# SamStudio8/gretel

Hardware: NVIDIA B200
Metric: snp_pair_observations_per_sec (higher is better)
Workload: dtype u32

## Files before the change

gretel_b200/_lib.py:

```python
from __future__ import annotations

import ctypes as C
import os

_HERE = os.path.dirname(os.path.abspath(__file__))
LIB_PATH = os.path.join(_HERE, "libhanselx.so")

HX_OK, HX_HOLE = 0, 1
HX_E_CUDA, HX_E_ARG, HX_E_BAND, HX_E_READ, HX_E_NOMEM, HX_E_STATE = -1, -2, -3, -4, -5, -6
HX_F_VSITE_TO, HX_F_KEEP_UNSYMBOLS = 1, 2

_p, _i32, _i64, _int, _dbl, _flt = C.c_void_p, C.c_int32, C.c_int64, C.c_int, C.c_double, C.c_float
_pp = C.POINTER(C.c_void_p)

SIGNATURES = {
    "hx_last_error": (C.c_char_p, []),
    "hx_version": (_int, []),
    "hx_device_count": (_int, [C.POINTER(_int)]),
    "hx_create": (_int, [_i32, _i32, _i32, _pp]),
    "hx_destroy": (_int, [_p]),
    "hx_copy": (_int, [_p, _pp]),
    "hx_info": (_int, [_p, C.POINTER(_i32), C.POINTER(_i32), C.POINTER(_i32)]),
    "hx_stream": (_int, [_p, _pp]),
    "hx_set_stream": (_int, [_p, _p]),
    "hx_sync": (_int, [_p]),
    "hx_ingest_host": (_int, [_p, _p, _p, _p, _i64, _p]),
    "hx_counts_pack": (_int, [_p, _i32, _pp, C.POINTER(_i64)]),
    "hx_counts_unpack": (_int, [_p, C.POINTER(_i32)]),
    "hx_counts_unpack_async": (_int, [_p, _p]),
    "hx_counts_pack_overflowed": (_int, [_p, C.POINTER(_i32)]),
    "hx_counts_max": (_int, [_p, C.POINTER(C.c_uint32)]),
    "hx_ingest_host_compact": (_int, [_p, _p, _p, _p, _i64, _i64, _p]),
    "hx_dense_encode": (_int, [_p, _p, _p, _i64, _int, _p]),
    "hx_dense_free": (None, [_p]),
    "hx_ingest_host_dense": (_int, [_p, _p, _p, _p, _i64, _p, _i32, _p, _p, _i64, _i64, _i64, _p]),
    "hx_ingest_device": (_int, [_p, _p, _p, _p, _i64]),
    "hx_set_ingest_kernel": (_int, [_p, _int]),
    "hx_set_ingest_sms": (_int, [_p, _int]),
    "hx_ingest_totals": (_int, [_p, _p]),
    "hx_counts_buffer": (_int, [_p, _pp, C.POINTER(_i64), _pp, C.POINTER(_i64)]),
    "hx_counts_ipc_export": (_int, [_p, _i32, _p]),
    "hx_counts_ipc_import": (_int, [_p, _p, _i32, _i32]),
    "hx_counts_ipc_close": (_int, [_p]),
    "hx_finalize_counts": (_int, [_p]),
    "hx_reset_counts": (_int, [_p]),
    "hx_add_observation": (_int, [_p, _int, _int, _i32, _i32, _flt]),
    "hx_get_observation": (_int, [_p, _int, _int, _i32, _i32, C.POINTER(_flt)]),
    "hx_reweight_observation": (_int, [_p, _int, _int, _i32, _i32, _dbl, C.POINTER(_dbl)]),
    "hx_reweight_matrix": (_int, [_p, _dbl]),
    "hx_counts_all": (_int, [_p, _p]),
    "hx_marginal_of_at": (_int, [_p, _int, _i32, C.POINTER(_dbl)]),
    "hx_edge_weights_at": (_int, [_p, _i32, _p, _i32, _int, _p, C.POINTER(_dbl), C.POINTER(_int)]),
    "hx_generate_path": (_int, [_p, _p, _i32, _int, _p, _p, C.POINTER(_i32)]),
    "hx_reweight_path": (_int, [_p, _p, _dbl, C.POINTER(_dbl)]),
    "hx_recover": (_int, [_p, _p, _i32, _int, _i32, _dbl, _p, _p, C.POINTER(_i32)]),
    "hx_pack_bam": (_int, [C.c_char_p, C.c_char_p, _i32, _i32, _p, _i32, _int, _int, _p]),
    "hx_pack_bam_ex": (_int, [C.c_char_p, C.c_char_p, _i32, _i32, _p, _i32, _int, _int, _i32, _p, _p]),
    "hx_pack_free": (None, [_p]),
    "hx_count_coverage": (_int, [C.c_char_p, C.c_char_p, _i32, _i32, _int, _p]),
    "hx_count_coverage_gpu": (_int, [C.c_char_p, C.c_char_p, _i32, _i32, _int, _i32, _p]),
    "hx_bam_contig_length": (_int, [C.c_char_p, C.c_char_p, C.POINTER(_i32)]),
    "hx_inflate_raw": (_int, [_p, _i64, _i64, _p, _i64, _i32]),
    "hx_probe_expected_rows": (_int, [_p, _p, _p, _p, _i64, _p]),
    "hx_counts_row_sums": (_int, [_p, _p]),
    "hx_device_math": (_int, [_i32, _int, _p, _p, _i64]),
    "hx_band_to_host": (_int, [_p, _p]),
    "hx_band_from_host": (_int, [_p, _p]),
    "hx_to_dense": (_int, [_p, _p]),
    "hx_last_kernel_ms": (_int, [_p, _int, C.POINTER(_flt)]),
    "hx_launch_count": (_int, [_p, C.POINTER(_i64)]),
}

class HxPacked(C.Structure):
    _fields_ = [("rank", C.POINTER(C.c_int32)), ("off", C.POINTER(C.c_int64)), ("codes", C.POINTER(C.c_uint8)),
                ("n_reads", C.c_int64), ("n_codes", C.c_int64), ("n_records", C.c_int64)]


class HxDense(C.Structure):
    _fields_ = [("blob", C.POINTER(C.c_uint8)), ("blob_bytes", C.c_int64), ("n_reads", C.c_int64),
                ("n_codes", C.c_int64), ("n_exc", C.c_int64), ("n_esc", C.c_int64), ("o_klen", C.c_int64),
                ("o_codes2", C.c_int64), ("o_exc", C.c_int64), ("o_esc_idx", C.c_int64), ("o_esc_delta", C.c_int64),
                ("klen_bytes", C.c_int32)]


_LIB = None


class HanselxError(RuntimeError):
    def __init__(self, code, msg):
        super().__init__("hanselx error %d: %s" % (code, msg))
        self.code = code


def load():
    global _LIB
    if _LIB is not None:
        return _LIB
    if not os.path.exists(LIB_PATH):
        raise RuntimeError(
            "gretel_b200: %s is missing - build it with `python -m gretel_b200.build` "
            "(nvcc, sm_100a).  There is no CPU fallback." % LIB_PATH)
    lib = C.CDLL(LIB_PATH)
    for name, (res, args) in SIGNATURES.items():
        fn = getattr(lib, name)
        fn.restype = res
        fn.argtypes = args
    _LIB = lib
    return lib


def check(rc, allow=()):
    if rc == HX_OK or rc in allow:
        return rc
    raise HanselxError(rc, load().hx_last_error().decode(errors="replace"))
```

gretel_b200/csrc/api.cu:

```cuda
#include <stdarg.h>
#include <stdlib.h>
#include <string.h>

#include <algorithm>
#include <mutex>
#include <vector>

#include <atomic>

#include "hx_internal.cuh"
#include "scan.cuh"

static thread_local char g_err[512] = "";

void hx_set_error(const char *fmt, ...) {
    va_list ap;
    va_start(ap, fmt);
    vsnprintf(g_err, sizeof(g_err), fmt, ap);
    va_end(ap);
}

static void release_counts(hx_matrix *h) {
    for (int g = 0; g < HX_MAX_PEERS; ++g) {
        if (h->ipc_opened[g]) cudaIpcCloseMemHandle(h->ipc_opened[g]);
        h->ipc_opened[g] = nullptr;
        h->peer_host[g] = nullptr;
    }
    h->peer_world = 0;
    if (h->cnt) {
        if (h->cnt_ipc) { cudaStreamSynchronize(h->stream); cudaFree(h->cnt); }
        else cudaFreeAsync(h->cnt, h->stream);
    }
    h->cnt = nullptr;
    h->cnt_ipc = false;
    h->cnt_elems = 0;
}

HxCnt hx_cnt_ref(const hx_matrix *h) {
    HxCnt c;
    c.local = h->cnt;
    c.peer = h->d_peer_tbl;
    c.world = h->peer_world > 1 ? h->peer_world : 1;
    c.rows_per = h->peer_world > 1 ? h->peer_rows_per : 1;
    return c;
}

namespace {

__global__ void k_fold_counts(const uint32_t *__restrict__ cnt, float *__restrict__ band, int64_t n) {
    const int64_t i = (int64_t)blockIdx.x * blockDim.x + threadIdx.x;
    if (i < n) {
        const uint32_t c = cnt[i];
        if (c) band[i] += (float)c;
    }
}

__global__ void k_add_one(float *p, float amount) { *p += amount; }

__global__ void k_reset_counts(uint4 *__restrict__ cnt, size_t bytes, unsigned long long *__restrict__ totals,
                               int *__restrict__ err) {
    const size_t n16 = bytes / 16;
    const uint4 z = make_uint4(0, 0, 0, 0);
    for (size_t i = (size_t)blockIdx.x * blockDim.x + threadIdx.x; i < n16; i += (size_t)gridDim.x * blockDim.x) cnt[i] = z;
    if (blockIdx.x == 0) {
        uint8_t *tail = reinterpret_cast<uint8_t *>(cnt) + n16 * 16;
        for (size_t i = threadIdx.x; i < bytes - n16 * 16; i += blockDim.x) tail[i] = 0;
        if (threadIdx.x < 8) totals[threadIdx.x] = 0;
        if (threadIdx.x == 8) *err = 0;
    }
}

#define HX_PACK_WORDS 25
__global__ void k_pack_counts(const uint32_t *__restrict__ cnt, int64_t n_pairs, uint32_t lim16,
                              uint32_t *__restrict__ packed, int64_t flag_at) {
    const int64_t i = (int64_t)blockIdx.x * blockDim.x + threadIdx.x;
    if (i >= n_pairs * HX_PACK_WORDS) return;
    const int64_t p = i / HX_PACK_WORDS;
    const int w = (int)(i - p * HX_PACK_WORDS);
    const uint32_t *c = cnt + p * HX_CELL + 2 * w;
    const uint32_t lo = c[0], hi = 2 * w + 1 < HX_CELL ? c[1] : 0u;
    if (lo > lim16 || hi > lim16) packed[flag_at] = 1u;
    packed[i] = (lo & 0xffffu) | (hi << 16);
}

__global__ void k_unpack_counts(const uint32_t *__restrict__ packed, int64_t n_pairs, uint32_t *__restrict__ cnt,
                                int64_t flag_at) {
    if (packed[flag_at] != 0u) return;
    const int64_t i = (int64_t)blockIdx.x * blockDim.x + threadIdx.x;
    if (i >= n_pairs * HX_PACK_WORDS) return;
    const int64_t p = i / HX_PACK_WORDS;
    const int w = (int)(i - p * HX_PACK_WORDS);
    const uint32_t v = packed[i];
    uint32_t *c = cnt + p * HX_CELL + 2 * w;
    c[0] = v & 0xffffu;
    if (2 * w + 1 < HX_CELL) c[1] = v >> 16;
}

__global__ void k_widen_klen(const uint16_t *__restrict__ klen, int64_t n, int64_t *__restrict__ out ) {
    const int64_t i = (int64_t)blockIdx.x * blockDim.x + threadIdx.x;
    if (i <= n) out[i] = i < n ? (int64_t)klen[i] : 0;
}

__global__ void k_unpack_nibbles(const uint32_t *__restrict__ in, int64_t n_words, uint2 *__restrict__ out) {
    const int64_t i = (int64_t)blockIdx.x * blockDim.x + threadIdx.x;
    if (i >= n_words) return;
    const uint32_t w = in[i];
    uint2 o;
    o.x = (w & 0xfu) | ((w >> 4 & 0xfu) << 8) | ((w >> 8 & 0xfu) << 16) | ((w >> 12 & 0xfu) << 24);
    o.y = (w >> 16 & 0xfu) | ((w >> 20 & 0xfu) << 8) | ((w >> 24 & 0xfu) << 16) | ((w >> 28 & 0xfu) << 24);
    out[i] = o;
}

__global__ void k_reweight_one(float *p, double ratio, double *removed) {
    const double old = (double)*p;
    const double nw = old - (ratio * old);
    *p = (float)nw;
    *removed = old - nw;
}

int in_band(const hx_matrix *h, int a, int b, int64_t i, int64_t j) {
    if (a < 0 || a >= HX_NSYM || b < 0 || b >= HX_NSYM) return HX_E_ARG;
    if (i < 0 || j < 0 || i > (int64_t)h->N + 1 || j > (int64_t)h->N + 1) return HX_E_ARG;
    if (j - i < 1 || j - i > h->W) return HX_E_BAND;
    return HX_OK;
}

void free_all(hx_matrix *h) {
    if (!h) return;
    cudaSetDevice(h->device);
    hx_lr_free(h);
    hx_l2_free(h);
    hx_wire_free(h);
    if (h->d_peer_tbl) cudaFree(h->d_peer_tbl);
    cudaStream_t st = h->stream;
    h->band.release(st);
    release_counts(h);
    h->d_totals.release(st); h->d_err.release(st);
    h->s_rank.release(st); h->s_off.release(st); h->s_codes.release(st);
    h->s_klen.release(st); h->s_codes4.release(st); h->s_scan.release(st);
    h->scnt.release(st); h->vseen.release(st); h->d_path.release(st); h->d_stats.release(st); h->d_site.release(st);
    h->d_partials.release(st); h->d_spec.release(st); h->d_terms.release(st); h->d_flags.release(st);
    h->d_run_end.release(st); h->d_run_list.release(st); h->d_jobs.release(st); h->d_misc.release(st);
    h->d_pack.release(st);
    if (st) cudaStreamSynchronize(st);
    free(h->h_pinned);
    if (h->ev0) cudaEventDestroy(h->ev0);
    if (h->ev1) cudaEventDestroy(h->ev1);
    if (h->host_ev) cudaEventDestroy(h->host_ev);
    if (h->sum_stream) { cudaStreamSynchronize(h->sum_stream); cudaStreamDestroy(h->sum_stream); }
    for (int b = 0; b < 2; ++b) if (h->sum_done[b]) cudaEventDestroy(h->sum_done[b]);
    if (h->site_ready) cudaEventDestroy(h->site_ready);
    if (h->own_stream && h->stream) cudaStreamDestroy(h->stream);
    free(h);
}

}

extern "C" {

const char *hx_last_error(void) { return g_err; }
int hx_version(void) { return 100; }

int hx_device_count(int *n) {
    HX_CHECK_ARG(n);
    HX_CUDA(cudaGetDeviceCount(n));
    return HX_OK;
}

}

namespace {
std::mutex &g_park_mu = *new std::mutex;
std::vector<hx_matrix *> &g_parked = *new std::vector<hx_matrix *>;
constexpr size_t HX_PARK_MAX = 4;
constexpr int64_t HX_PARK_MAX_ELEMS = (int64_t)1 << 28;
const bool g_park_on = getenv("HX_NO_MATRIX_CACHE") == nullptr;

hx_matrix *unpark(int32_t n_snps, int32_t band_w, int32_t device) {
    std::lock_guard<std::mutex> lk(g_park_mu);
    for (size_t i = 0; i < g_parked.size(); ++i) {
        hx_matrix *h = g_parked[i];
        if (h->N == n_snps && h->W == band_w && h->device == device) {
            g_parked.erase(g_parked.begin() + (long)i);
            return h;
        }
    }
    return nullptr;
}

bool park(hx_matrix *h) {
    if (!g_park_on || !h->own_stream || h->cnt_ipc || h->peer_world > 1 || h->band_elems > HX_PARK_MAX_ELEMS) return false;
    if (cudaSetDevice(h->device) != cudaSuccess) return false;
    release_counts(h);
    if (cudaStreamSynchronize(h->stream) != cudaSuccess) return false;
    hx_matrix *evict = nullptr;
    {
        std::lock_guard<std::mutex> lk(g_park_mu);
        if (g_parked.size() >= HX_PARK_MAX) { evict = g_parked.front(); g_parked.erase(g_parked.begin()); }
        g_parked.push_back(h);
    }
    if (evict) free_all(evict);
    return true;
}

int reset_parked(hx_matrix *h) {
    HX_CUDA(cudaSetDevice(h->device));
    HX_CUDA(hx_fill_async(h->band.p, 0, sizeof(float) * (size_t)h->band_elems, h->stream));
    HX_CUDA(hx_fill_async(h->d_totals.p, 0, 8 * sizeof(unsigned long long), h->stream));
    HX_CUDA(hx_fill_async(h->d_err.p, 0, sizeof(int), h->stream));
    HX_CUDA(hx_fill_async(h->d_flags.p, 0, 8 * sizeof(int), h->stream));
    h->use = {};
    return HX_OK;
}
}

extern "C" {

int hx_create(int32_t n_snps, int32_t band_w, int32_t device, hx_matrix **out) {
    HX_CHECK_ARG(out && n_snps >= 0 && band_w >= 1);
    *out = nullptr;
    HX_CUDA(cudaSetDevice(device));
    if (hx_matrix *p = unpark(n_snps, band_w, device)) {
        const int rc = reset_parked(p);
        if (rc) { free_all(p); return rc; }
        *out = p;
        return HX_OK;
    }
    hx_matrix *h = (hx_matrix *)calloc(1, sizeof(hx_matrix));
    if (!h) return HX_E_NOMEM;
    h->N = n_snps;
    h->W = band_w;
    h->device = device;
    h->band_elems = ((int64_t)n_snps + 2) * band_w * HX_CELL;
    h->use = {};
#define HX_TRY(call)                                                                     \
    do {                                                                                 \
        cudaError_t e__ = (call);                                                        \
        if (e__ != cudaSuccess) {                                                        \
            hx_set_error("hx_create: %s -> %s", #call, cudaGetErrorString(e__));         \
            free_all(h);                                                                 \
            return e__ == cudaErrorMemoryAllocation ? HX_E_NOMEM : HX_E_CUDA;            \
        }                                                                                \
    } while (0)
    {
        cudaMemPool_t pool;
        if (cudaDeviceGetDefaultMemPool(&pool, device) == cudaSuccess) {
            unsigned long long thr = ~0ull;
            cudaMemPoolSetAttribute(pool, cudaMemPoolAttrReleaseThreshold, &thr);
        }
    }
    HX_TRY(cudaStreamCreateWithFlags(&h->stream, cudaStreamNonBlocking));
    h->own_stream = true;
    HX_TRY(cudaEventCreate(&h->ev0));
    HX_TRY(cudaEventCreate(&h->ev1));
    HX_TRY(h->band.grow(sizeof(float) * (size_t)h->band_elems, h->stream));
    HX_TRY(hx_fill_async(h->band.p, 0, sizeof(float) * (size_t)h->band_elems, h->stream));
    HX_TRY(h->d_totals.grow(8 * sizeof(unsigned long long), h->stream));
    HX_TRY(hx_fill_async(h->d_totals.p, 0, 8 * sizeof(unsigned long long), h->stream));
    HX_TRY(h->d_err.grow(sizeof(int), h->stream));
    HX_TRY(hx_fill_async(h->d_err.p, 0, sizeof(int), h->stream));
    HX_TRY(h->scnt.grow(sizeof(double) * 8 * ((size_t)n_snps + 2), h->stream));
    HX_TRY(h->vseen.grow(sizeof(int32_t) * ((size_t)n_snps + 2), h->stream));
    HX_TRY(h->d_site.grow(sizeof(double) * 6 * ((size_t)n_snps + 2), h->stream));
    HX_TRY(h->d_flags.grow(8 * sizeof(int), h->stream));
    HX_TRY(hx_fill_async(h->d_flags.p, 0, 8 * sizeof(int), h->stream));
    HX_TRY(h->d_misc.grow(32 * sizeof(double), h->stream));
    HX_TRY(h->d_run_end.grow(sizeof(int64_t) * ((size_t)n_snps + 2), h->stream));
    HX_TRY(h->d_run_list.grow(sizeof(int64_t) * (((size_t)n_snps + 3) / 2 + (size_t)n_snps + 2 + 2), h->stream));
    h->h_pinned = calloc(1, 256);
    if (!h->h_pinned) { free_all(h); return HX_E_NOMEM; }
    HX_TRY(cudaStreamSynchronize(h->stream));
#undef HX_TRY
    *out = h;
    return HX_OK;
}

int hx_destroy(hx_matrix *h) {
    if (h && !park(h)) free_all(h);
    return HX_OK;
}

int hx_copy(const hx_matrix *src, hx_matrix **out) {
    HX_CHECK_ARG(src && out);
    if (src->cnt) {
        hx_set_error("hx_copy: integer counts pending; call hx_finalize_counts first");
        return HX_E_STATE;
    }
    int rc = hx_create(src->N, src->W, src->device, out);
    if (rc) return rc;
    hx_matrix *h = *out;
    HX_CUDA(cudaStreamSynchronize(src->stream));
    HX_CUDA(cudaMemcpyAsync(h->band.p, src->band.p, sizeof(float) * (size_t)src->band_elems,
                            cudaMemcpyDeviceToDevice, h->stream));
    HX_CUDA(cudaMemcpyAsync(h->d_totals.p, src->d_totals.p, 8 * sizeof(unsigned long long),
                            cudaMemcpyDeviceToDevice, h->stream));
    HX_CUDA(cudaStreamSynchronize(h->stream));
    h->use.ingest_kernel = src->use.ingest_kernel;
    return HX_OK;
}

int hx_info(const hx_matrix *h, int32_t *n_snps, int32_t *band_w, int32_t *device) {
    HX_CHECK_ARG(h);
    if (n_snps) *n_snps = h->N;
    if (band_w) *band_w = h->W;
    if (device) *device = h->device;
    return HX_OK;
}

int hx_stream(const hx_matrix *h, void **stream) {
    HX_CHECK_ARG(h && stream);
    *stream = (void *)h->stream;
    return HX_OK;
}

int hx_set_stream(hx_matrix *h, void *stream) {
    HX_CHECK_ARG(h);
    HX_CUDA(cudaSetDevice(h->device));
    HX_CUDA(cudaStreamSynchronize(h->stream));
    if (h->own_stream) cudaStreamDestroy(h->stream);
    h->stream = (cudaStream_t)stream;
    h->own_stream = false;
    return HX_OK;
}

int hx_sync(hx_matrix *h) {
    HX_CHECK_ARG(h);
    HX_CUDA(cudaSetDevice(h->device));
    HX_CUDA(cudaStreamSynchronize(h->stream));
    return HX_OK;
}

}
int hx_ensure_counts_buffer(hx_matrix *h) {
    if (h->cnt) return HX_OK;
    h->cnt_elems = h->band_elems;
    HX_CUDA(cudaMallocAsync((void **)&h->cnt, sizeof(uint32_t) * (size_t)h->cnt_elems, h->stream));
    HX_CUDA(hx_fill_async(h->cnt, 0, sizeof(uint32_t) * (size_t)h->cnt_elems, h->stream));
    h->use.cnt_fresh = true;
    return HX_OK;
}
extern "C" {

int hx_set_ingest_kernel(hx_matrix *h, int which) {
    HX_CHECK_ARG(h && which >= 0 && which <= 7);
    h->use.ingest_kernel = which;
    return HX_OK;
}

int hx_set_ingest_sms(hx_matrix *h, int n_sms) {
    HX_CHECK_ARG(h && n_sms >= 0);
    h->use.ingest_sms = n_sms;
    return HX_OK;
}

int hx_ingest_device(hx_matrix *h, const int32_t *d_rank, const int64_t *d_off,
                     const uint8_t *d_codes, int64_t n_reads) {
    HX_CHECK_ARG(h && n_reads >= 0);
    if (n_reads == 0) return HX_OK;
    HX_CHECK_ARG(d_rank && d_off && d_codes);
    HX_CUDA(cudaSetDevice(h->device));
    int rc = hx_ensure_counts_buffer(h);
    if (rc) return rc;
    return hx_launch_ingest(h, d_rank, d_off, d_codes, n_reads);
}

int hx_ingest_totals(hx_matrix *h, int64_t totals[4]) {
    HX_CHECK_ARG(h && totals);
    HX_CUDA(cudaSetDevice(h->device));
    unsigned long long *hp = (unsigned long long *)h->h_pinned;
    int *he = (int *)(hp + 8);
    HX_CUDA(cudaMemcpyAsync(hp, h->d_totals.p, 4 * sizeof(unsigned long long), cudaMemcpyDeviceToHost, h->stream));
    HX_CUDA(cudaMemcpyAsync(he, h->d_err.p, sizeof(int), cudaMemcpyDeviceToHost, h->stream));
    if (h->use.prepass_ran) HX_CUDA(cudaMemcpyAsync(he + 1, h->d_flags.p + 4, sizeof(int), cudaMemcpyDeviceToHost, h->stream));
    HX_CUDA(cudaStreamSynchronize(h->stream));
    if (h->use.prepass_ran && he[1] == 0) hx_note_unsorted();
    hx_wire_trace_dump();
    if (h->use.ev_rec) cudaEventElapsedTime(&h->use.last_ms[0], h->ev0, h->ev1);
    for (int i = 0; i < 4; ++i) totals[i] = (int64_t)hp[i];
    if (*he) {
        hx_set_error("ingest: invalid packed read(s): %s%s",
                     (*he & 1) ? "[read leaves [0,N] or has more SNPs than band_w+1] " : "",
                     (*he & 2) ? "[allele code > 6]" : "");
        return HX_E_READ;
    }
    return HX_OK;
}

int hx_ingest_host(hx_matrix *h, const int32_t *rank, const int64_t *off, const uint8_t *codes,
                   int64_t n_reads, int64_t totals[4]) {
    HX_CHECK_ARG(h && totals && n_reads >= 0);
    HX_CUDA(cudaSetDevice(h->device));
    const char *pipe_env = getenv("HX_HOST_PIPELINE");
    const bool want_dense = pipe_env && !strcmp(pipe_env, "dense");
    const bool want_slim = !pipe_env || !strcmp(pipe_env, "slim");
    if (n_reads >= 200000 && rank && off && codes && (want_dense || want_slim)) {
        int64_t done = 0;
        const int rc = hx_ingest_host_pipelined(h, rank, off, codes, n_reads, !want_dense, &done);
        if (rc == HX_OK) return hx_ingest_totals(h, totals);
        if (rc != HX_E_STATE) return rc;
        hx_note_unsorted();
        rank += done; off += done; n_reads -= done;
    }
    if (n_reads > 0) {
        HX_CHECK_ARG(rank && off && codes);
        const int64_t n_codes = off[n_reads] - off[0];
        HX_CHECK_ARG(n_codes >= 0);
        HX_CUDA(h->s_rank.grow(sizeof(int32_t) * n_reads, h->stream));
        HX_CUDA(h->s_off.grow(sizeof(int64_t) * (n_reads + 1) + 16, h->stream));
        HX_CUDA(h->s_codes.grow(n_codes + 16, h->stream));
        int rc = hx_ensure_counts_buffer(h);
        if (rc) return rc;
        const int n_chunks = n_reads >= 200000 && !(pipe_env && !strcmp(pipe_env, "off")) ? 4 : 1;
        if (n_chunks > 1 && !h->copy_stream) HX_CUDA(cudaStreamCreateWithFlags(&h->copy_stream, cudaStreamNonBlocking));
        cudaStream_t cs = n_chunks > 1 ? h->copy_stream : h->stream;
        if (n_chunks > 1) {
            if (!h->host_ev) HX_CUDA(cudaEventCreateWithFlags(&h->host_ev, cudaEventDisableTiming));
            HX_CUDA(cudaEventRecord(h->host_ev, h->stream));
            HX_CUDA(cudaStreamWaitEvent(cs, h->host_ev, 0));
        }
        int64_t a = 0;
        for (int c = 0; c < n_chunks; ++c) {
            int64_t b = n_reads;
            if (c + 1 < n_chunks) {
                const int64_t target = off[0] + n_codes * (c + 1) / n_chunks;
                b = std::lower_bound(off + a, off + n_reads, target) - off;
                if (b <= a) continue;
            }
            HX_CUDA(cudaMemcpyAsync(h->s_rank.p + a, rank + a, sizeof(int32_t) * (size_t)(b - a), cudaMemcpyHostToDevice, cs));
            HX_CUDA(cudaMemcpyAsync(h->s_off.p + a, off + a, sizeof(int64_t) * (size_t)(b - a + 1), cudaMemcpyHostToDevice, cs));
            HX_CUDA(cudaMemcpyAsync(h->s_codes.p + (off[a] - off[0]), codes + off[a], (size_t)(off[b] - off[a]), cudaMemcpyHostToDevice, cs));
            if (n_chunks > 1) {
                HX_CUDA(cudaEventRecord(h->host_ev, cs));
                HX_CUDA(cudaStreamWaitEvent(h->stream, h->host_ev, 0));
            }
            rc = hx_launch_ingest(h, h->s_rank.p + a, h->s_off.p + a, h->s_codes.p - off[0], b - a);
            if (rc) return rc;
            a = b;
        }
    }
    return hx_ingest_totals(h, totals);
}

int hx_ingest_host_compact(hx_matrix *h, const int32_t *rank, const uint16_t *klen, const uint8_t *codes4,
                           int64_t n_reads, int64_t n_codes, int64_t totals[4]) {
    HX_CHECK_ARG(h && totals && n_reads >= 0 && n_codes >= 0);
    HX_CUDA(cudaSetDevice(h->device));
    if (n_reads > 0) {
        HX_CHECK_ARG(rank && klen && (codes4 || n_codes == 0));
        cudaStream_t st = h->stream;
        const int64_t n_words = (n_codes + 7) / 8;
        constexpr int ITEMS = 16;
        const int64_t n1 = n_reads + 1;
        const int64_t nblk = (n1 + 256 * ITEMS - 1) / (256 * ITEMS);
        HX_CUDA(h->s_rank.grow(sizeof(int32_t) * n_reads, st));
        HX_CUDA(h->s_off.grow(sizeof(int64_t) * n1 + 16, st));
        HX_CUDA(h->s_codes.grow(n_words * 8 + 16, st));
        HX_CUDA(h->s_klen.grow(sizeof(uint16_t) * n_reads, st));
        HX_CUDA(h->s_codes4.grow(sizeof(uint32_t) * n_words, st));
        HX_CUDA(h->s_scan.grow(sizeof(int64_t) * nblk, st));
        HX_CUDA(cudaMemcpyAsync(h->s_rank.p, rank, sizeof(int32_t) * (size_t)n_reads, cudaMemcpyHostToDevice, st));
        HX_CUDA(cudaMemcpyAsync(h->s_klen.p, klen, sizeof(uint16_t) * (size_t)n_reads, cudaMemcpyHostToDevice, st));
        if (n_codes)
            HX_CUDA(cudaMemcpyAsync(h->s_codes4.p, codes4, (size_t)((n_codes + 1) / 2), cudaMemcpyHostToDevice, st));
        k_widen_klen<<<(unsigned)((n1 + 255) / 256), 256, 0, st>>>(h->s_klen.p, n_reads, h->s_off.p);
        k_scan_partials<int64_t, 0, ITEMS><<<(unsigned)nblk, 256, 0, st>>>(h->s_off.p, n1, h->s_scan.p);
        k_scan_spine<int64_t, 0><<<1, 32, 0, st>>>(h->s_scan.p, nblk, nullptr);
        k_scan_apply<int64_t, 0, ITEMS, true><<<(unsigned)nblk, 256, 0, st>>>(h->s_off.p, n1, h->s_scan.p, h->s_off.p);
        if (n_words)
            k_unpack_nibbles<<<(unsigned)((n_words + 255) / 256), 256, 0, st>>>(h->s_codes4.p, n_words, (uint2 *)h->s_codes.p);
        h->use.launches += 5;
        HX_CUDA(cudaGetLastError());
        int rc = hx_ensure_counts_buffer(h);
        if (rc) return rc;
        rc = hx_launch_ingest(h, h->s_rank.p, h->s_off.p, h->s_codes.p, n_reads);
        if (rc) return rc;
    }
    return hx_ingest_totals(h, totals);
}

int hx_counts_buffer(hx_matrix *h, void **d_counts, int64_t *n_u32, void **d_totals, int64_t *n_i64) {
    HX_CHECK_ARG(h && d_counts && n_u32 && d_totals && n_i64);
    HX_CUDA(cudaSetDevice(h->device));
    int rc = hx_ensure_counts_buffer(h);
    if (rc) return rc;
    *d_counts = h->cnt;
    h->use.cnt_fresh = false;
    *n_u32 = h->cnt_elems;
    *d_totals = h->d_totals.p;
    *n_i64 = 4;
    return HX_OK;
}

int hx_counts_pack(hx_matrix *h, int32_t world, void **d_packed, int64_t *n_u32) {
    HX_CHECK_ARG(h && d_packed && n_u32 && world >= 1 && world <= 65535);
    HX_CUDA(cudaSetDevice(h->device));
    int rc = hx_ensure_counts_buffer(h);
    if (rc) return rc;
    const int64_t n_pairs = h->band_elems / HX_CELL;
    const int64_t flag_at = (n_pairs * HX_PACK_WORDS + 3) & ~(int64_t)3;
    const int64_t words = flag_at + 4;
    HX_CUDA(h->d_pack.grow(sizeof(uint32_t) * words, h->stream));
    HX_CUDA(hx_fill_async(h->d_pack.p + n_pairs * HX_PACK_WORDS, 0, (size_t)(words - n_pairs * HX_PACK_WORDS) * 4, h->stream));
    const int64_t n_w = n_pairs * HX_PACK_WORDS;
    k_pack_counts<<<(unsigned)((n_w + 255) / 256), 256, 0, h->stream>>>(h->cnt, n_pairs, 65535u / (uint32_t)world,
                                                                        h->d_pack.p, flag_at);
    h->use.launches++;
    HX_CUDA(cudaGetLastError());
    *d_packed = h->d_pack.p;
    *n_u32 = words;
    return HX_OK;
}

int hx_counts_unpack(hx_matrix *h, int32_t *overflowed) {
    HX_CHECK_ARG(h && overflowed && h->d_pack.p && h->cnt);
    HX_CUDA(cudaSetDevice(h->device));
    const int64_t n_pairs = h->band_elems / HX_CELL;
    const int64_t flag_at = (n_pairs * HX_PACK_WORDS + 3) & ~(int64_t)3;
    const int64_t n_w = n_pairs * HX_PACK_WORDS;
    h->use.cnt_fresh = false;
    k_unpack_counts<<<(unsigned)((n_w + 255) / 256), 256, 0, h->stream>>>(h->d_pack.p, n_pairs, h->cnt, flag_at);
    h->use.launches++;
    HX_CUDA(cudaGetLastError());
    uint32_t *hp = (uint32_t *)h->h_pinned + 40;
    HX_CUDA(cudaMemcpyAsync(hp, h->d_pack.p + flag_at, sizeof(uint32_t), cudaMemcpyDeviceToHost, h->stream));
    HX_CUDA(cudaStreamSynchronize(h->stream));
    *overflowed = *hp != 0;
    return HX_OK;
}

int hx_counts_unpack_async(hx_matrix *h, void *stream) {
    HX_CHECK_ARG(h && h->d_pack.p && h->cnt);
    HX_CUDA(cudaSetDevice(h->device));
    const int64_t n_pairs = h->band_elems / HX_CELL;
    const int64_t flag_at = (n_pairs * HX_PACK_WORDS + 3) & ~(int64_t)3;
    const int64_t n_w = n_pairs * HX_PACK_WORDS;
    h->use.cnt_fresh = false;
    cudaStream_t st = stream ? (cudaStream_t)stream : h->stream;
    k_unpack_counts<<<(unsigned)((n_w + 255) / 256), 256, 0, st>>>(h->d_pack.p, n_pairs, h->cnt, flag_at);
    h->use.launches++;
    HX_CUDA(cudaGetLastError());
    return HX_OK;
}

int hx_counts_pack_overflowed(hx_matrix *h, int32_t *overflowed) {
    HX_CHECK_ARG(h && overflowed && h->d_pack.p);
    HX_CUDA(cudaSetDevice(h->device));
    const int64_t n_pairs = h->band_elems / HX_CELL;
    const int64_t flag_at = (n_pairs * HX_PACK_WORDS + 3) & ~(int64_t)3;
    uint32_t *hp = (uint32_t *)h->h_pinned + 40;
    HX_CUDA(cudaMemcpyAsync(hp, h->d_pack.p + flag_at, sizeof(uint32_t), cudaMemcpyDeviceToHost, h->stream));
    HX_CUDA(cudaStreamSynchronize(h->stream));
    *overflowed = *hp != 0;
    return HX_OK;
}

__global__ void k_counts_max(const uint32_t *__restrict__ cnt, int64_t n, uint32_t *__restrict__ out) {
    uint32_t m = 0;
    for (int64_t i = (int64_t)blockIdx.x * blockDim.x + threadIdx.x; i < n; i += (int64_t)gridDim.x * blockDim.x) m = max(m, cnt[i]);
    m = __reduce_max_sync(0xffffffffu, m);
    if ((threadIdx.x & 31) == 0 && m) atomicMax(out, m);
}

int hx_counts_max(hx_matrix *h, uint32_t *max_count) {
    HX_CHECK_ARG(h && max_count);
    HX_CUDA(cudaSetDevice(h->device));
    int rc = hx_ensure_counts_buffer(h);
    if (rc) return rc;
    uint32_t *d_out = reinterpret_cast<uint32_t *>(h->d_flags.p + 6);
    HX_CUDA(hx_fill_async(d_out, 0, sizeof(uint32_t), h->stream));
    k_counts_max<<<592, 256, 0, h->stream>>>(h->cnt, h->cnt_elems, d_out);
    h->use.launches++;
    HX_CUDA(cudaGetLastError());
    uint32_t *hp = (uint32_t *)h->h_pinned + 41;
    HX_CUDA(cudaMemcpyAsync(hp, d_out, sizeof(uint32_t), cudaMemcpyDeviceToHost, h->stream));
    HX_CUDA(cudaStreamSynchronize(h->stream));
    *max_count = *hp;
    return HX_OK;
}

int hx_counts_ipc_export(hx_matrix *h, int32_t world, void *handle_out) {
    HX_CHECK_ARG(h && handle_out && world >= 1 && world <= HX_MAX_PEERS);
    HX_CUDA(cudaSetDevice(h->device));
    release_counts(h);
    const int64_t rows = (int64_t)h->N + 2;
    const int64_t rows_per = (rows + world - 1) / world;
    h->cnt_elems = rows_per * world * h->W * HX_CELL;
    HX_CUDA(cudaMalloc((void **)&h->cnt, sizeof(uint32_t) * (size_t)h->cnt_elems));
    h->cnt_ipc = true;
    h->use.cnt_fresh = false;
    HX_CUDA(hx_fill_async(h->cnt, 0, sizeof(uint32_t) * (size_t)h->cnt_elems, h->stream));
    HX_CUDA(cudaStreamSynchronize(h->stream));
    cudaIpcMemHandle_t hd;
    HX_CUDA(cudaIpcGetMemHandle(&hd, h->cnt));
    memcpy(handle_out, &hd, sizeof(hd));
    h->peer_rows_per = (int)rows_per;
    return HX_OK;
}

int hx_counts_ipc_import(hx_matrix *h, const void *handles, int32_t world, int32_t my_rank) {
    HX_CHECK_ARG(h && handles && world >= 1 && world <= HX_MAX_PEERS && my_rank >= 0 && my_rank < world);
    if (!h->cnt_ipc) { hx_set_error("hx_counts_ipc_import: call hx_counts_ipc_export first"); return HX_E_STATE; }
    HX_CUDA(cudaSetDevice(h->device));
    for (int g = 0; g < world; ++g) {
        if (g == my_rank) { h->peer_host[g] = h->cnt; continue; }
        cudaIpcMemHandle_t hd;
        memcpy(&hd, (const char *)handles + (size_t)g * sizeof(hd), sizeof(hd));
        void *p = nullptr;
        HX_CUDA(cudaIpcOpenMemHandle(&p, hd, cudaIpcMemLazyEnablePeerAccess));
        h->ipc_opened[g] = p;
        h->peer_host[g] = (uint32_t *)p;
    }
    if (!h->d_peer_tbl) HX_CUDA(cudaMalloc((void **)&h->d_peer_tbl, sizeof(uint32_t *) * HX_MAX_PEERS));
    HX_CUDA(cudaMemcpy(h->d_peer_tbl, h->peer_host, sizeof(uint32_t *) * HX_MAX_PEERS, cudaMemcpyHostToDevice));
    h->peer_world = world;
    return HX_OK;
}

int hx_counts_ipc_close(hx_matrix *h) {
    HX_CHECK_ARG(h);
    HX_CUDA(cudaSetDevice(h->device));
    HX_CUDA(cudaStreamSynchronize(h->stream));
    for (int g = 0; g < HX_MAX_PEERS; ++g) {
        if (h->ipc_opened[g]) HX_CUDA(cudaIpcCloseMemHandle(h->ipc_opened[g]));
        h->ipc_opened[g] = nullptr;
        h->peer_host[g] = nullptr;
    }
    h->peer_world = 0;
    return HX_OK;
}

int hx_reset_counts(hx_matrix *h) {
    HX_CHECK_ARG(h);
    HX_CUDA(cudaSetDevice(h->device));
    if (h->cnt) {
        const size_t n16 = (sizeof(uint32_t) * (size_t)h->cnt_elems + 15) / 16;
        const size_t want = (n16 + 255) / 256;
        const unsigned grid = (unsigned)(want < 1 ? 1 : (want > 148 * 16 ? 148 * 16 : want));
        k_reset_counts<<<grid, 256, 0, h->stream>>>(reinterpret_cast<uint4 *>(h->cnt), sizeof(uint32_t) * (size_t)h->cnt_elems,
                                                    h->d_totals.p, h->d_err.p);
        HX_CUDA(cudaGetLastError());
        h->use.cnt_fresh = true;
    } else {
        HX_CUDA(hx_fill_async(h->d_totals.p, 0, 8 * sizeof(unsigned long long), h->stream));
        HX_CUDA(hx_fill_async(h->d_err.p, 0, sizeof(int), h->stream));
    }
    return HX_OK;
}

int hx_finalize_counts(hx_matrix *h) {
    HX_CHECK_ARG(h);
    if (!h->cnt) return HX_OK;
    HX_CUDA(cudaSetDevice(h->device));
    const int64_t n = h->band_elems;
    k_fold_counts<<<(unsigned)((n + 255) / 256), 256, 0, h->stream>>>(h->cnt, h->band.p, n);
    h->use.launches++;
    HX_CUDA(cudaGetLastError());
    if (h->cnt_ipc) HX_CUDA(cudaStreamSynchronize(h->stream));
    release_counts(h);
    h->use.counts_dirty = true;
    return HX_OK;
}

int hx_add_observation(hx_matrix *h, int a, int b, int32_t i, int32_t j, float amount) {
    HX_CHECK_ARG(h);
    int rc = in_band(h, a, b, i, j);
    if (rc) { hx_set_error("add_observation(%d,%d,%d,%d): outside band/arguments", a, b, i, j); return rc; }
    HX_CUDA(cudaSetDevice(h->device));
    k_add_one<<<1, 1, 0, h->stream>>>(h->band.p + hx_cell_off(h->W, i, j) + a * HX_NSYM + b, amount);
    h->use.launches++;
    h->use.counts_dirty = true;
    HX_CUDA(cudaGetLastError());
    return HX_OK;
}

int hx_get_observation(hx_matrix *h, int a, int b, int32_t i, int32_t j, float *out) {
    HX_CHECK_ARG(h && out);
    int rc = in_band(h, a, b, i, j);
    if (rc == HX_E_BAND) { *out = 0.0f; return HX_E_BAND; }
    if (rc) { hx_set_error("get_observation(%d,%d,%d,%d): bad arguments", a, b, i, j); return rc; }
    HX_CUDA(cudaSetDevice(h->device));
    const int64_t o = hx_cell_off(h->W, i, j) + a * HX_NSYM + b;
    float v = 0.0f;
    HX_CUDA(cudaMemcpyAsync(&v, h->band.p + o, sizeof(float), cudaMemcpyDeviceToHost, h->stream));
    HX_CUDA(cudaStreamSynchronize(h->stream));
    if (h->cnt) {
        uint32_t c = 0;
        HX_CUDA(cudaMemcpyAsync(&c, h->cnt + o, sizeof(uint32_t), cudaMemcpyDeviceToHost, h->stream));
        HX_CUDA(cudaStreamSynchronize(h->stream));
        v += (float)c;
    }
    *out = v;
    return HX_OK;
}

int hx_reweight_observation(hx_matrix *h, int a, int b, int32_t i, int32_t j, double ratio,
                            double *removed) {
    HX_CHECK_ARG(h && removed);
    int rc = in_band(h, a, b, i, j);
    if (rc == HX_E_BAND) { *removed = 0.0; return HX_E_BAND; }
    if (rc) { hx_set_error("reweight_observation(%d,%d,%d,%d): bad arguments", a, b, i, j); return rc; }
    if (h->cnt) { hx_set_error("reweight_observation: call hx_finalize_counts first"); return HX_E_STATE; }
    HX_CUDA(cudaSetDevice(h->device));
    k_reweight_one<<<1, 1, 0, h->stream>>>(h->band.p + hx_cell_off(h->W, i, j) + a * HX_NSYM + b, ratio, h->d_misc.p + 16);
    h->use.launches++;
    h->use.counts_dirty = true;
    HX_CUDA(cudaGetLastError());
    HX_CUDA(cudaMemcpyAsync(removed, h->d_misc.p + 16, sizeof(double), cudaMemcpyDeviceToHost, h->stream));
    HX_CUDA(cudaStreamSynchronize(h->stream));
    return HX_OK;
}

int hx_band_to_host(hx_matrix *h, float *out) {
    HX_CHECK_ARG(h && out);
    if (h->cnt) { hx_set_error("band_to_host: call hx_finalize_counts first"); return HX_E_STATE; }
    HX_CUDA(cudaSetDevice(h->device));
    HX_CUDA(cudaMemcpyAsync(out, h->band.p, sizeof(float) * (size_t)h->band_elems, cudaMemcpyDeviceToHost, h->stream));
    HX_CUDA(cudaStreamSynchronize(h->stream));
    return HX_OK;
}

int hx_band_from_host(hx_matrix *h, const float *in) {
    HX_CHECK_ARG(h && in);
    if (h->cnt) { hx_set_error("band_from_host: call hx_finalize_counts first"); return HX_E_STATE; }
    HX_CUDA(cudaSetDevice(h->device));
    HX_CUDA(cudaMemcpyAsync(h->band.p, in, sizeof(float) * (size_t)h->band_elems, cudaMemcpyHostToDevice, h->stream));
    HX_CUDA(cudaStreamSynchronize(h->stream));
    h->use.counts_dirty = true;
    return HX_OK;
}

int hx_to_dense(hx_matrix *h, float *out) {
    HX_CHECK_ARG(h && out);
    const int64_t P = (int64_t)h->N + 2;
    float *tmp = (float *)malloc(sizeof(float) * (size_t)h->band_elems);
    if (!tmp) return HX_E_NOMEM;
    int rc = hx_band_to_host(h, tmp);
    if (rc) { free(tmp); return rc; }
    memset(out, 0, sizeof(float) * (size_t)(HX_CELL * P * P));
    for (int64_t pj = 1; pj < P; ++pj)
        for (int64_t d = 1; d <= h->W && pj - d >= 0; ++d) {
            const float *cell = tmp + hx_cell_off(h->W, pj - d, pj);
            for (int ab = 0; ab < HX_CELL; ++ab) out[(ab * P + (pj - d)) * P + pj] = cell[ab];
        }
    free(tmp);
    return HX_OK;
}

int hx_last_kernel_ms(hx_matrix *h, int which, float *ms) {
    HX_CHECK_ARG(h && ms && which >= 0 && which < 3);
    *ms = h->use.last_ms[which];
    return HX_OK;
}

int hx_launch_count(const hx_matrix *h, int64_t *n) {
    HX_CHECK_ARG(h && n);
    *n = h->use.launches;
    return HX_OK;
}

}
```

gretel_b200/csrc/hx_internal.cuh:

```cuda
#pragma once
#include <cuda_runtime.h>
#include <stdint.h>
#include <stdio.h>

#include "hanselx.h"

#define HX_NSYM 7
#define HX_CELL 49
#define HX_SYM_N 4
#define HX_SYM_DEL 5
#define HX_SYM_GAP 6
#define HX_RING 4096
#define HX_MAX_L (HX_RING - 1)

#define HX_MAX_PEERS 8
struct HxCnt {
    uint32_t *local;
    uint32_t *const *peer;
    int world, rows_per;
#ifdef __CUDACC__
    __device__ __forceinline__ uint32_t *cell(int64_t W, int64_t pi, int64_t pj) const {
        uint32_t *base = local;
        if (world > 1) base = peer[pj / rows_per];
        return base + (pj * W + (pj - pi - 1)) * 49;
    }
#endif
};

template <class T>
struct HxDevBuf {
    T *p;
    int64_t cap;
    cudaError_t grow(int64_t bytes, cudaStream_t st, bool *grew = nullptr) {
        if (bytes <= cap) return cudaSuccess;
        if (grew) *grew = true;
        release(st);
        const cudaError_t e = cudaMallocAsync((void **)&p, (size_t)bytes, st);
        if (e != cudaSuccess) { p = nullptr; return e; }
        cap = bytes;
        return cudaSuccess;
    }
    void release(cudaStream_t st) {
        if (p) cudaFreeAsync(p, st);
        p = nullptr;
        cap = 0;
    }
};

#define HX_WIRE_SETS 3
struct hx_wire_set {
    HxDevBuf<uint8_t> raw; HxDevBuf<int32_t> rank; HxDevBuf<int64_t> off; HxDevBuf<uint8_t> codes;
    HxDevBuf<int64_t> partials, run_end;
    cudaEvent_t copied, decoded, consumed;
};

struct hx_matrix {
    int32_t N, W, device;
    int64_t band_elems;
    cudaStream_t stream;
    bool own_stream;
    HxDevBuf<float> band;
    uint32_t *cnt;
    bool cnt_ipc;
    int64_t cnt_elems;
    uint32_t *peer_host[HX_MAX_PEERS];
    uint32_t **d_peer_tbl;
    int peer_world, peer_rows_per;
    void *ipc_opened[HX_MAX_PEERS];
    HxDevBuf<unsigned long long> d_totals;
    HxDevBuf<int> d_err;
    HxDevBuf<int32_t> s_rank; HxDevBuf<int64_t> s_off; HxDevBuf<uint8_t> s_codes;
    HxDevBuf<uint16_t> s_klen; HxDevBuf<uint32_t> s_codes4; HxDevBuf<int64_t> s_scan;
    hx_wire_set wire[HX_WIRE_SETS];
    cudaStream_t copy_stream, decode_stream;
    uint8_t *pin[2]; int64_t pin_cap[2]; cudaEvent_t pin_ev[2]; bool pin_busy[2];
    HxDevBuf<double> scnt;
    HxDevBuf<int32_t> vseen;
    HxDevBuf<uint8_t> d_path;
    HxDevBuf<double> d_stats;
    HxDevBuf<double> d_site;
    cudaStream_t sum_stream;
    cudaEvent_t sum_done[2], site_ready;
    HxDevBuf<double> d_terms;
    HxDevBuf<uint8_t> d_spec;
    HxDevBuf<double> d_partials;
    HxDevBuf<int> d_flags;
    HxDevBuf<int64_t> d_run_end;
    HxDevBuf<int64_t> d_run_list;
    HxDevBuf<int4> d_jobs;
    HxDevBuf<double> d_misc;
    HxDevBuf<uint32_t> d_pack;
    void *h_pinned;
    void *lr_scratch;
    void *l2_scratch;
    cudaEvent_t ev0, ev1;
    cudaEvent_t host_ev;
    struct Use {
        int64_t launches = 0;
        int ingest_kernel = 0;
        int ingest_sms = 0;
        bool counts_dirty = true;
        bool cnt_fresh = false;
        bool ev_rec = false;
        bool prepass_ran = false;
        int wire_next = 0;
        bool sum_busy[2] = {};
        float last_ms[3] = {};
    } use;
};

void hx_set_error(const char *fmt, ...);

#define HX_CUDA(call)                                                                   \
    do {                                                                                \
        cudaError_t e__ = (call);                                                       \
        if (e__ != cudaSuccess) {                                                       \
            hx_set_error("%s:%d %s -> %s", __FILE__, __LINE__, #call, cudaGetErrorString(e__)); \
            return HX_E_CUDA;                                                           \
        }                                                                               \
    } while (0)

#define HX_CHECK_ARG(cond)                                                              \
    do {                                                                                \
        if (!(cond)) {                                                                  \
            hx_set_error("%s:%d argument check failed: %s", __FILE__, __LINE__, #cond); \
            return HX_E_ARG;                                                            \
        }                                                                               \
    } while (0)

#ifdef __CUDACC__
static __global__ void k_fill_bytes(uint8_t *p, unsigned v, size_t bytes) {
    if (reinterpret_cast<uintptr_t>(p) & 15) {
        for (size_t i = (size_t)blockIdx.x * blockDim.x + threadIdx.x; i < bytes; i += (size_t)gridDim.x * blockDim.x)
            p[i] = (uint8_t)v;
        return;
    }
    const size_t n16 = bytes / 16;
    const uint4 w = make_uint4(v, v, v, v);
    uint4 *p16 = reinterpret_cast<uint4 *>(p);
    for (size_t i = (size_t)blockIdx.x * blockDim.x + threadIdx.x; i < n16; i += (size_t)gridDim.x * blockDim.x) p16[i] = w;
    if (blockIdx.x == 0)
        for (size_t i = n16 * 16 + threadIdx.x; i < bytes; i += blockDim.x) p[i] = (uint8_t)v;
}
static inline cudaError_t hx_fill_async(void *p, int byte, size_t bytes, cudaStream_t st) {
    if (!bytes) return cudaSuccess;
    const unsigned b = (unsigned)byte & 0xffu, v = b * 0x01010101u;
    const size_t want = (bytes / 16 + 255) / 256;
    const unsigned grid = (unsigned)(want < 1 ? 1 : (want > 148 * 16 ? 148 * 16 : want));
    k_fill_bytes<<<grid, 256, 0, st>>>(static_cast<uint8_t *>(p), v, bytes);
    return cudaGetLastError();
}
#endif

__host__ __device__ __forceinline__ int64_t hx_cell_off(int64_t W, int64_t pi, int64_t pj) {
    return (pj * W + (pj - pi - 1)) * HX_CELL;
}

int hx_launch_ingest(hx_matrix *h, const int32_t *d_rank, const int64_t *d_off,
                     const uint8_t *d_codes, int64_t n_reads);
int hx_launch_ingest_presorted(hx_matrix *h, const int32_t *d_rank, const int64_t *d_off,
                               const uint8_t *d_codes, int64_t n_reads, int64_t *run_end, const int *ok);
bool hx_umma_possible(const hx_matrix *h);
int hx_launch_ingest_umma(hx_matrix *h, const int32_t *d_rank, const int64_t *d_off, const uint8_t *d_codes,
                          int64_t n_reads, const int64_t *run_end, const int *sorted_flag);
HxCnt hx_cnt_ref(const hx_matrix *h);
int hx_ensure_counts_buffer(hx_matrix *h);
void hx_wire_free(hx_matrix *h);
void hx_wire_trace_dump();
bool hx_unsorted_seen();
void hx_note_unsorted();
int hx_ingest_host_pipelined(hx_matrix *h, const int32_t *rank, const int64_t *off, const uint8_t *codes, int64_t n_reads,
                             bool slim, int64_t *done_reads);
int hx_launch_ingest_long(hx_matrix *h, const int32_t *d_rank, const int64_t *d_off,
                          const uint8_t *d_codes, int64_t n_reads, const int *sorted_flag);
void hx_lr_free(hx_matrix *h);
int hx_launch_ingest_lumma(hx_matrix *h, const int32_t *d_rank, const int64_t *d_off, const uint8_t *d_codes,
                           int64_t n_reads, const int *go);
int64_t hx_lumma_scratch_bytes(const hx_matrix *h, int64_t n_reads);
void hx_l2_free(hx_matrix *h);
int hx_ensure_counts(hx_matrix *h);
```

gretel_b200/csrc/ingest.cu:

```cuda
#include <atomic>

#include "hx_internal.cuh"
#include "ingest_common.cuh"

namespace {

constexpr int BS_KMAX = 52;
constexpr int BS_GB = 32;

__device__ __forceinline__ void add_pair(const HxCnt cnt, int N, int64_t W, int rk, int i,
                                         int j, unsigned a, unsigned b, unsigned long long &sent) {
    const int pi = rk + i + 1, pj = rk + j + 1;
    atomicAdd(cnt.cell(W, pi, pj) + a * HX_NSYM + b, 1u);
    if (i == 0 && j == 1 && rk == 0) {
        atomicAdd(cnt.cell(W, 0, 1) + HX_SYM_GAP * HX_NSYM + a, 1u);
        sent++;
    } else if (pj == N && j - i == 1) {
        atomicAdd(cnt.cell(W, N, N + 1) + b * HX_NSYM + HX_SYM_GAP, 1u);
        sent++;
    }
}

__device__ __forceinline__ void warp_read_generic(const uint8_t *__restrict__ c, int k, int rk, int N,
                                                  int64_t W, const HxCnt cnt,
                                                  unsigned long long &t_crumbs, unsigned long long &t_cov,
                                                  unsigned long long &t_sent, int *err) {
    const int lane = threadIdx.x & 31;
    for (int t = lane; t < k; t += 32) {
        const unsigned a = c[t];
        if (a > 6) atomicOr(err, 2);
        const bool v = sym_valid_from(a);
        t_cov += v;
        t_crumbs += v ? (unsigned)(k - 1 - t) : 0u;
    }
    const int64_t npairs = (int64_t)k * (k - 1) / 2;
    const int m = 2 * k - 1;
    for (int64_t q = lane; q < npairs; q += 32) {
        const float disc = (float)((int64_t)m * m - 8 * q);
        int i = (int)(((float)m - sqrtf(disc)) * 0.5f);
        i = max(0, min(i, k - 2));
        while ((int64_t)(i + 1) * (m - (i + 1)) / 2 <= q) ++i;
        while ((int64_t)i * (m - i) / 2 > q) --i;
        const int j = i + 1 + (int)(q - (int64_t)i * (m - i) / 2);
        const unsigned a = c[i], b = c[j];
        if (!sym_valid_from(a) || b > 6) continue;
        add_pair(cnt, N, W, rk, i, j, a, b, t_sent);
    }
}

template <int BLOCK>
__global__ void __launch_bounds__(BLOCK)
k1_pairs_red(const int32_t *__restrict__ rank, const int64_t *__restrict__ off,
             const uint8_t *__restrict__ codes, int64_t n_reads, int N, int W,
             const HxCnt cnt, unsigned long long *__restrict__ totals,
             int *__restrict__ err, const int *__restrict__ sorted_flag, int run_if_sorted) {
    if (run_if_sorted == 0 && *sorted_flag) return;
    if (run_if_sorted == 2 && !*sorted_flag) return;
    const int lane = threadIdx.x & 31;
    const int64_t nwarps = (int64_t)gridDim.x * (BLOCK / 32);
    unsigned long long t_slices = 0, t_crumbs = 0, t_cov = 0, t_sent = 0;
    for (int64_t r = (int64_t)blockIdx.x * (BLOCK / 32) + (threadIdx.x >> 5); r < n_reads; r += nwarps) {
        const int64_t o = off[r];
        const int64_t k64 = off[r + 1] - o;
        if (k64 < 2) continue;
        const int rk = rank[r];
        if (rk < 0 || (int64_t)rk + k64 > N || k64 - 1 > W) {
            if (lane == 0) atomicOr(err, 1);
            continue;
        }
        if (lane == 0) t_slices++;
        warp_read_generic(codes + o, (int)k64, rk, N, W, cnt, t_crumbs, t_cov, t_sent, err);
    }
    flush_totals(t_slices, t_crumbs, t_cov, t_sent, totals);
}

__global__ void k_prepass_init(int *__restrict__ flag, int64_t *__restrict__ run_end, int n) {
    const int i = blockIdx.x * blockDim.x + threadIdx.x;
    if (i == 0) *flag = 1;
    if (i < n) run_end[i] = -1;
}

__global__ void k_prepass(const int32_t *__restrict__ rank, int64_t n_reads, int N, int *__restrict__ flag,
                          int64_t *__restrict__ run_end, int *__restrict__ err) {
    const int64_t i = (int64_t)blockIdx.x * blockDim.x + threadIdx.x;
    if (i >= n_reads) return;
    const int r = rank[i];
    if (r < 0 || r > N) atomicOr(err, 1);
    if (i + 1 < n_reads) {
        const int r2 = rank[i + 1];
        if (r > r2) *flag = 0;
        if (r != r2 && r >= 0 && r <= N) run_end[r] = i + 1;
    } else if (r >= 0 && r <= N) {
        run_end[r] = n_reads;
    }
}

struct BsLayout {
    int kmax, gb;
    __host__ __device__ size_t tile_u4() const { return (size_t)(kmax + 1) * (kmax - 1) * 4; }
    __host__ __device__ size_t bytes() const {
        return tile_u4() * 16 + (size_t)2 * gb * kmax * 16 + 64 * sizeof(int) + (size_t)2 * gb * 32 * sizeof(int);
    }
};

__device__ __forceinline__ unsigned long long bs_flush_rows(uint32_t *tile32, int rows, int cells,
                                                            int64_t pj_lo, int64_t pj_hi, int64_t W,
                                                            const HxCnt cnt) {
    unsigned long long sum = 0;
    const int per_row = cells * 16;
    int row = (int)(pj_lo % rows);
    for (int64_t pj = pj_lo; pj <= pj_hi; ++pj) {
        uint32_t *base = tile32 + (size_t)row * per_row;
        for (int w = threadIdx.x; w < per_row; w += blockDim.x) {
            const uint32_t v = base[w];
            if (v) {
                const int d = (w >> 4) + 1, ab = w & 15;
                atomicAdd(cnt.cell(W, pj - d, pj) + (ab >> 2) * HX_NSYM + (ab & 3), v);
                base[w] = 0;
                sum += v;
            }
        }
        if (++row == rows) row = 0;
    }
    return sum;
}

template <int KW>
__device__ __forceinline__ int bs_build_group(const uint8_t *__restrict__ codes, int64_t o, int kb,
                                              uint32_t pg_addr, uint32_t &rare_or, uint32_t &x0) {
    const int lane = threadIdx.x & 31;
    const int kg = __reduce_max_sync(0xffffffffu, kb);
    const uint8_t *__restrict__ c = codes + o;
    const unsigned mis = (unsigned)(reinterpret_cast<uintptr_t>(c) & 3u);
    const uint32_t *__restrict__ cw = reinterpret_cast<const uint32_t *>(c - mis);
    const int nw = kb ? (int)((mis + kb + 3) >> 2) : 0;
    uint32_t wd[KW + 1];
#pragma unroll
    for (int w = 0; w <= KW; ++w) wd[w] = w < nw ? __ldg(cw + w) : 0u;
    const unsigned sh = 8u * mis;
    const int kb8 = 8 * kb;
    uint32_t g12[KW];
    rare_or = 0;
    x0 = 0xffffffffu;
#pragma unroll
    for (int w = 0; w < KW; ++w) {
        g12[w] = 0;
        if (w == 0 || 4 * w < kg) {
            const uint32_t xx = __funnelshift_r(wd[w], wd[w + 1], sh);
            const int c8 = min(max(kb8 - 32 * w, 0), 32);
            uint32_t inval;
            asm("shl.b32 %0, %1, %2;" : "=r"(inval) : "r"(0xffffffffu), "r"(c8));
            rare_or |= xx & 0xfcfcfcfcu & ~inval;
            const uint32_t x = xx | inval;
            if (w == 0) x0 = x;
            const uint32_t u = (x >> 2) & 0x3f3f3f3fu;
            const uint32_t v = (((u + 0x3f3f3f3fu) & 0x40404040u) >> 6) ^ 0x01010101u;
            const uint32_t f = ((x & 0x03030303u) * 2u + 0x01010101u) & (v * 7u);
            g12[w] = (f & 7u) | ((f >> 5) & 0x38u) | ((f >> 10) & 0x1c0u) | ((f >> 15) & 0xe00u);
        }
    }
    const int my_tl = lane / 3, my_plane = lane - 3 * my_tl;
#pragma unroll
    for (int t0 = 0; t0 < 4 * KW; t0 += 10) {
        if (t0 >= kg) break;
        const int c = t0 / 10, wb = 5 * (c >> 1);
        auto G = [&](int i) -> uint32_t { return i < KW ? g12[i] : 0u; };
        uint32_t row = (c & 1) ? ((G(wb + 2) >> 6) | (G(wb + 3) << 6) | (G(wb + 4) << 18))
                               : (G(wb) | (G(wb + 1) << 12) | ((G(wb + 2) & 0x3fu) << 24));
#pragma unroll
        for (int j = 16; j >= 1; j >>= 1) {
            const uint32_t m = j == 16 ? 0x0000ffffu : j == 8 ? 0x00ff00ffu : j == 4 ? 0x0f0f0f0fu
                             : j == 2 ? 0x33333333u : 0x55555555u;
            const bool up = (lane & j) != 0;
            const uint32_t take = up ? m : ~m;
            const uint32_t y = __shfl_xor_sync(0xffffffffu, row, j);
            const uint32_t yr = __funnelshift_l(y, y, up ? 32 - j : j);
            row = (row & ~take) | (yr & take);
        }
        const int t = t0 + my_tl;
        if (lane < 30 && t < kg)
            asm volatile("st.shared.u32 [%0], %1;" ::"r"(pg_addr + (uint32_t)(t * 16 + my_plane * 4)), "r"(row) : "memory");
    }
    return kg;
}

__device__ __forceinline__ void bs_accumulate(uint32_t (&acc)[16], uint32_t buf_saddr, uint32_t gk_addr, int a1, int a2,
                                              int nb, int kmax) {
    uint32_t p1 = buf_saddr + (uint32_t)a1 * 16u, p2 = buf_saddr + (uint32_t)a2 * 16u;
    uint32_t gstep = (uint32_t)kmax * 16u;
    asm volatile("" : "+r"(p1), "+r"(p2), "+r"(gstep), "+r"(gk_addr));
    for (int g = 0; g < nb; ++g, p1 += gstep, p2 += gstep, gk_addr += 4u) {
        int kg;
        asm volatile("ld.shared.s32 %0, [%1];" : "=r"(kg) : "r"(gk_addr));
        if (a2 < kg) {
            uint4 m1, m2;
            asm volatile("ld.shared.v4.u32 {%0, %1, %2, %3}, [%4];" : "=r"(m1.x), "=r"(m1.y), "=r"(m1.z), "=r"(m1.w) : "r"(p1));
            asm volatile("ld.shared.v4.u32 {%0, %1, %2, %3}, [%4];" : "=r"(m2.x), "=r"(m2.y), "=r"(m2.z), "=r"(m2.w) : "r"(p2));
            const unsigned x1[4] = {m1.x & ~(m1.y | m1.z), m1.y & ~m1.z, m1.z & ~m1.y, m1.y & m1.z};
            const unsigned x2[4] = {m2.x & ~(m2.y | m2.z), m2.y & ~m2.z, m2.z & ~m2.y, m2.y & m2.z};
#pragma unroll
            for (int a = 0; a < 4; ++a)
#pragma unroll
                for (int b = 0; b < 4; ++b) acc[a * 4 + b] += __popc(x1[a] & x2[b]);
        }
    }
}

struct BsBatch {
    int64_t start;
    int n;
    int r;
    bool first, last;
};

template <int KW, int NP, int MAXT, int MINB, bool FUSED>
__global__ void __launch_bounds__(MAXT, MINB)
k1_bitsliced(const int32_t *__restrict__ rank, const int64_t *__restrict__ off,
             const uint8_t *__restrict__ codes, int64_t n_reads, int N, int W, int kmax, int gb,
             const HxCnt cnt_in, unsigned long long *__restrict__ totals,
             int *__restrict__ err, const int *__restrict__ sorted_flag,
             const int64_t *__restrict__ run_end) {
    extern __shared__ uint4 smem4[];
    HxCnt cnt = cnt_in;
    if (!FUSED) { cnt.world = 1; cnt.rows_per = 1; cnt.peer = nullptr; }
    if (!*sorted_flag) return;
    const int rows = kmax + 1, cells = kmax - 1;
    uint4 *const tile = smem4;
    uint32_t *const tile32 = reinterpret_cast<uint32_t *>(tile);
    uint4 *const planes0 = tile + (size_t)rows * cells * 4;
    int *const gk0 = reinterpret_cast<int *>(planes0 + (size_t)2 * gb * kmax);
    int *const rareq0 = gk0 + 64;
    const uint32_t planes_saddr = (uint32_t)__cvta_generic_to_shared(planes0);
    const uint32_t gk_saddr = (uint32_t)__cvta_generic_to_shared(gk0);
    __shared__ int s_rare_n[3];
    __shared__ int s_claim[3];

    const int lane = threadIdx.x & 31, warp = threadIdx.x >> 5, nwarps = blockDim.x >> 5;
    int64_t lo, hi;
    hx_weighted_slice(rank, off, n_reads, HX_SLICE_READ_W, HX_SLICE_RANK_W, lo, hi);
    if (lo >= hi) return;

    for (size_t w = threadIdx.x; w < (size_t)rows * cells * 4; w += blockDim.x) tile[w] = make_uint4(0, 0, 0, 0);
    if (threadIdx.x == 0) { s_rare_n[0] = s_rare_n[1] = s_rare_n[2] = 0; s_claim[0] = s_claim[1] = s_claim[2] = 0; }
    const uint32_t pf_bytes = (uint32_t)gb * 32u * (uint32_t)(kmax > 40 ? 32 : 18);
    int rc_build = 1, rc_cons = 0, rc_clear = 2;

    int t1[NP], t2[NP];
#pragma unroll
    for (int q = 0; q < NP; ++q) {
        const int p = threadIdx.x + q * blockDim.x;
        int b = (int)((1.0f + sqrtf(1.0f + 8.0f * (float)p)) * 0.5f);
        while (b * (b - 1) / 2 > p) --b;
        while ((b + 1) * b / 2 <= p) ++b;
        t2[q] = b;
        t1[q] = p - b * (b - 1) / 2;
    }
    unsigned long long t_crumbs = 0;
    unsigned n_slices = 0, n_codes = 0, n_notcov = 0, n_sent = 0, n_rcrumbs = 0, errbits = 0;
    int64_t flushed_upto = (int64_t)rank[lo] + 1;
    uint32_t acc[NP][16];
    int run_kmax = 0, rbase = 0;

    int64_t cur = lo, run_hi = lo;
    int run_r = 0;
    BsBatch prev{0, 0, 0, false, false};
    int buf = 0;
    int prev_aw = 0;
    __syncthreads();

    for (;;) {
        BsBatch next{0, 0, 0, false, false};
        if (cur < hi) {
            next.first = cur >= run_hi;
            if (next.first) {
                run_r = rank[cur];
                run_hi = cur + 1;
                if (run_r >= 0 && run_r <= N) {
                    run_hi = run_end[run_r];
                    if (run_hi > hi) run_hi = hi;
                }
            }
            next.start = cur;
            next.r = run_r;
            next.n = (int)min((int64_t)gb * 32, run_hi - cur);
            cur += next.n;
            next.last = cur >= run_hi;
            if (threadIdx.x == 0 && cur < hi) {
                const int64_t ahead = min((int64_t)gb * 32 + 1, hi - cur + 1);
                bs_prefetch_l2(off + cur, (uint32_t)(ahead * 8));
                bs_prefetch_l2(rank + cur, 16);
            }
        }
        if (!prev.n && !next.n) break;

        if (prev.n) {
            const int pb = buf ^ 1;
            const int *gk = gk0 + pb * 32;
            const int nb = (prev.n + 31) >> 5;
            const int r = prev.r;
            if (prev.first) {
                if ((int64_t)r + 1 > flushed_upto) {
                    const int64_t last = min((int64_t)r + 1, flushed_upto + rows - 2);
                    t_crumbs += bs_flush_rows(tile32, rows, cells, flushed_upto + 1, last, W, cnt);
                    flushed_upto = (int64_t)r + 1;
                    __syncthreads();
                }
                rbase = (int)(((int64_t)r + 1) % rows);
                run_kmax = 0;
#pragma unroll
                for (int q = 0; q < NP; ++q)
#pragma unroll
                    for (int x = 0; x < 16; ++x) acc[q][x] = 0;
            }
            const int bkm = __reduce_max_sync(0xffffffffu, lane < nb ? gk[lane] : 0);
            run_kmax = max(run_kmax, bkm);
            prev_aw = (bkm * (bkm - 1) / 2 + 31) >> 5;
#pragma unroll
            for (int q = 0; q < NP; ++q) {
                if (t2[q] < bkm) bs_accumulate(acc[q], planes_saddr + (uint32_t)(pb * gb * kmax) * 16u, gk_saddr + pb * 128u,
                                               t1[q], t2[q], nb, kmax);
            }
            if (prev.last) {
#pragma unroll
                for (int q = 0; q < NP; ++q) {
                    if (t2[q] < run_kmax) {
                        int row = rbase + t2[q];
                        if (row >= rows) row -= rows;
                        const int d = t2[q] - t1[q];
                        uint4 *cell = tile + ((size_t)row * cells + (d - 1)) * 4;
#pragma unroll
                        for (int x = 0; x < 4; ++x) {
                            uint4 v = cell[x];
                            v.x += acc[q][4 * x + 0]; v.y += acc[q][4 * x + 1];
                            v.z += acc[q][4 * x + 2]; v.w += acc[q][4 * x + 3];
                            cell[x] = v;
                        }
                    }
                }
            }
            const int nrare = s_rare_n[rc_cons];
            const int *rareq = rareq0 + (size_t)pb * gb * 32;
            for (int qi = nwarps - 1 - warp; qi < nrare; qi += nwarps) {
                const int64_t idx = prev.start + rareq[qi];
                const int64_t o = off[idx];
                const int kb = (int)(off[idx + 1] - o);
                bs_rare_read(codes + o, kb, r, W, cnt, n_rcrumbs, n_notcov, errbits);
            }
        } else {
            prev_aw = 0;
        }

        if (next.n) {
            int *gk = gk0 + buf * 32;
            int *rareq = rareq0 + (size_t)buf * gb * 32;
            const int nb = (next.n + 31) >> 5;
            const int r = next.r;
            const int64_t run_stop = next.start + next.n;
            for (;;) {
                int g = 0;
                if (lane == 0) g = atomicAdd(&s_claim[rc_build], 1);
                g = __shfl_sync(0xffffffffu, g, 0);
                if (g >= nb) break;
                const int64_t idx = next.start + (int64_t)g * 32 + lane;
                int64_t o = 0;
                int kb = 0;
                if (idx < run_stop) {
                    o = off[idx];
                    const int64_t k64 = off[idx + 1] - o;
                    if (k64 >= 2) {
                        if (r < 0 || (int64_t)r + k64 > N || k64 - 1 > W) errbits |= 1;
                        else kb = (int)k64;
                    }
                    if (idx + 1 == run_stop && idx + 1 < hi) bs_prefetch_l2(codes + o + k64, pf_bytes);
                }
                n_slices += kb >= 2;
                n_codes += kb;
                uint32_t rare_or, x0;
                const uint8_t *__restrict__ c = codes + o;
                const int kg = bs_build_group<KW>(codes, o, kb, planes_saddr + (uint32_t)((buf * gb + g) * kmax) * 16u,
                                                  rare_or, x0);
                if (lane == 0) gk[g] = kg;
                if (kb >= 2) {
                    const unsigned a0 = x0 & 0xffu;
                    if (r == 0 && sym_valid_from(a0)) {
                        atomicAdd(cnt.cell(W, 0, 1) + HX_SYM_GAP * HX_NSYM + a0, 1u);
                        n_sent++;
                    }
                    if (r + kb == N && !(kb == 2 && r == 0)) {
                        const unsigned ap = c[kb - 2], bl = c[kb - 1];
                        if (sym_valid_from(ap) && bl <= 6) {
                            atomicAdd(cnt.cell(W, N, N + 1) + bl * HX_NSYM + HX_SYM_GAP, 1u);
                            n_sent++;
                        }
                    }
                    if (rare_or) rareq[atomicAdd(&s_rare_n[rc_build], 1)] = g * 32 + lane;
                }
            }
        }
        if (threadIdx.x == 0) { s_rare_n[rc_clear] = 0; s_claim[rc_clear] = 0; }
        __syncthreads();
        prev = next;
        buf ^= 1;
        { const int t = rc_clear; rc_clear = rc_cons; rc_cons = rc_build; rc_build = t; }
    }
    __syncthreads();
    t_crumbs += bs_flush_rows(tile32, rows, cells, flushed_upto + 1, flushed_upto + rows - 1, W, cnt);
    if (errbits) atomicOr(err, (int)errbits);
    flush_totals(n_slices, t_crumbs + n_rcrumbs, (unsigned long long)n_codes - n_notcov, n_sent, totals);
}

constexpr int WS_NBUF = 3;

struct WsLayout {
    int kmax, gb;
    __host__ __device__ size_t tile_u4() const { return (size_t)(kmax + 1) * (kmax - 1) * 4; }
    __host__ __device__ size_t bytes() const {
        return tile_u4() * 16 + (size_t)WS_NBUF * gb * kmax * 16 + (size_t)WS_NBUF * 32 * sizeof(int);
    }
};

template <int KW, int NP, int MAXT, int MINB, bool FUSED>
__global__ void __launch_bounds__(MAXT, MINB)
k1_bitsliced_ws(const int32_t *__restrict__ rank, const int64_t *__restrict__ off,
                const uint8_t *__restrict__ codes, int64_t n_reads, int N, int W, int kmax, int gb, int pw,
                const HxCnt cnt_in, unsigned long long *__restrict__ totals,
                int *__restrict__ err, const int *__restrict__ sorted_flag,
                const int64_t *__restrict__ run_end) {
    extern __shared__ uint4 smem4[];
    HxCnt cnt = cnt_in;
    if (!FUSED) { cnt.world = 1; cnt.rows_per = 1; cnt.peer = nullptr; }
    __shared__ __align__(8) unsigned long long s_full[WS_NBUF], s_empty[WS_NBUF];
    if (!*sorted_flag) return;
    const int rows = kmax + 1, cells = kmax - 1;
    uint4 *const tile = smem4;
    uint32_t *const tile32 = reinterpret_cast<uint32_t *>(tile);
    uint4 *const planes0 = tile + (size_t)rows * cells * 4;
    int *const gk0 = reinterpret_cast<int *>(planes0 + (size_t)WS_NBUF * gb * kmax);
    const uint32_t planes_saddr = (uint32_t)__cvta_generic_to_shared(planes0);
    const uint32_t gk_saddr = (uint32_t)__cvta_generic_to_shared(gk0);

    const int lane = threadIdx.x & 31, warp = threadIdx.x >> 5, nwarps = blockDim.x >> 5;
    const int bw = nwarps - pw;
    const bool is_pair = warp < pw;
    const int npt = pw * 32;
    int64_t lo, hi;
    hx_weighted_slice(rank, off, n_reads, HX_SLICE_READ_W, HX_SLICE_RANK_W, lo, hi);
    if (lo >= hi) return;

    for (size_t w = threadIdx.x; w < (size_t)rows * cells * 4; w += blockDim.x) tile[w] = make_uint4(0, 0, 0, 0);
    if (threadIdx.x == 0) {
        for (int b = 0; b < WS_NBUF; ++b) {
            ws_mbar_init(ws_smem_u32(&s_full[b]), bw);
            ws_mbar_init(ws_smem_u32(&s_empty[b]), pw);
        }
        asm volatile("fence.mbarrier_init.release.cluster;" ::: "memory");
    }
    __syncthreads();

    unsigned long long t_crumbs = 0;
    unsigned n_slices = 0, n_codes = 0, n_notcov = 0, n_sent = 0, n_rcrumbs = 0, errbits = 0;
    const uint32_t pf_bytes = (uint32_t)gb * 32u * (uint32_t)(kmax > 40 ? 32 : 18);

    int64_t cur = lo, run_hi = lo;
    int run_r = 0;
    unsigned bi = 0;

    if (!is_pair) {
        const int bwid = warp - pw;
        for (;; ++bi) {
            if (cur >= hi) break;
            if (cur >= run_hi) {
                run_r = rank[cur];
                run_hi = cur + 1;
                if (run_r >= 0 && run_r <= N) {
                    run_hi = run_end[run_r];
                    if (run_hi > hi) run_hi = hi;
                }
            }
            const int64_t bstart = cur;
            const int bn = (int)min((int64_t)gb * 32, run_hi - cur);
            cur += bn;
            if (bwid == 0 && lane == 0 && cur < hi) {
                const int64_t ahead = min((int64_t)gb * 32 + 1, hi - cur + 1);
                bs_prefetch_l2(off + cur, (uint32_t)(ahead * 8));
                bs_prefetch_l2(rank + cur, 16);
            }
            const int r = run_r;
            const int nb = (bn + 31) >> 5;
            const int b = bi % WS_NBUF;
            ws_mbar_wait(ws_smem_u32(&s_empty[b]), ((bi / WS_NBUF) & 1) ^ 1);
            int *gk = gk0 + b * 32;
            const int64_t run_stop = bstart + bn;
            for (int g = bwid; g < nb; g += bw) {
                const int64_t idx = bstart + (int64_t)g * 32 + lane;
                int64_t o = 0;
                int kb = 0;
                if (idx < run_stop) {
                    o = off[idx];
                    const int64_t k64 = off[idx + 1] - o;
                    if (k64 >= 2) {
                        if (r < 0 || (int64_t)r + k64 > N || k64 - 1 > W) errbits |= 1;
                        else kb = (int)k64;
                    }
                    if (idx + 1 == run_stop && idx + 1 < hi) bs_prefetch_l2(codes + o + k64, pf_bytes);
                }
                n_slices += kb >= 2;
                n_codes += kb;
                uint32_t rare_or, x0;
                const uint8_t *__restrict__ c = codes + o;
                const int kg = bs_build_group<KW>(codes, o, kb, planes_saddr + (uint32_t)((b * gb + g) * kmax) * 16u,
                                                  rare_or, x0);
                if (lane == 0) gk[g] = kg;
                if (kb >= 2) {
                    const unsigned a0 = x0 & 0xffu;
                    if (r == 0 && sym_valid_from(a0)) {
                        atomicAdd(cnt.cell(W, 0, 1) + HX_SYM_GAP * HX_NSYM + a0, 1u);
                        n_sent++;
                    }
                    if (r + kb == N && !(kb == 2 && r == 0)) {
                        const unsigned ap = c[kb - 2], bl = c[kb - 1];
                        if (sym_valid_from(ap) && bl <= 6) {
                            atomicAdd(cnt.cell(W, N, N + 1) + bl * HX_NSYM + HX_SYM_GAP, 1u);
                            n_sent++;
                        }
                    }
                }
                unsigned rm = __ballot_sync(0xffffffffu, kb >= 2 && rare_or != 0);
                while (rm) {
                    const int src = __ffs(rm) - 1;
                    rm &= rm - 1;
                    const int64_t o2 = __shfl_sync(0xffffffffu, o, src);
                    const int k2 = __shfl_sync(0xffffffffu, kb, src);
                    bs_rare_read(codes + o2, k2, r, W, cnt, n_rcrumbs, n_notcov, errbits);
                }
            }
            __syncwarp();
            if (lane == 0) ws_mbar_arrive(ws_smem_u32(&s_full[b]));
        }
    } else {
        int t1[NP], t2[NP];
#pragma unroll
        for (int q = 0; q < NP; ++q) {
            const int p = threadIdx.x + q * npt;
            int b = (int)((1.0f + sqrtf(1.0f + 8.0f * (float)p)) * 0.5f);
            while (b * (b - 1) / 2 > p) --b;
            while ((b + 1) * b / 2 <= p) ++b;
            t2[q] = b;
            t1[q] = p - b * (b - 1) / 2;
        }
        int64_t flushed_upto = (int64_t)rank[lo] + 1;
        uint32_t acc[NP][16];
        int run_kmax = 0, rbase = 0;
        for (;; ++bi) {
            if (cur >= hi) break;
            const bool first = cur >= run_hi;
            if (first) {
                run_r = rank[cur];
                run_hi = cur + 1;
                if (run_r >= 0 && run_r <= N) {
                    run_hi = run_end[run_r];
                    if (run_hi > hi) run_hi = hi;
                }
            }
            const int bn = (int)min((int64_t)gb * 32, run_hi - cur);
            cur += bn;
            const bool last = cur >= run_hi;
            const int r = run_r;
            const int nb = (bn + 31) >> 5;
            const int b = bi % WS_NBUF;
            if (first) {
                ws_pair_barrier(npt);
                if ((int64_t)r + 1 > flushed_upto) {
                    const int64_t lastrow = min((int64_t)r + 1, flushed_upto + rows - 2);
                    unsigned long long sum = 0;
                    const int per_row = cells * 16;
                    int row = (int)((flushed_upto + 1) % rows);
                    for (int64_t pj = flushed_upto + 1; pj <= lastrow; ++pj) {
                        uint32_t *base = tile32 + (size_t)row * per_row;
                        for (int w = threadIdx.x; w < per_row; w += npt) {
                            const uint32_t v = base[w];
                            if (v) {
                                const int d = (w >> 4) + 1, ab = w & 15;
                                atomicAdd(cnt.cell(W, pj - d, pj) + (ab >> 2) * HX_NSYM + (ab & 3), v);
                                base[w] = 0;
                                sum += v;
                            }
                        }
                        if (++row == rows) row = 0;
                    }
                    t_crumbs += sum;
                    flushed_upto = (int64_t)r + 1;
                    ws_pair_barrier(npt);
                }
                rbase = (int)(((int64_t)r + 1) % rows);
                run_kmax = 0;
#pragma unroll
                for (int q = 0; q < NP; ++q)
#pragma unroll
                    for (int x = 0; x < 16; ++x) acc[q][x] = 0;
            }
            ws_mbar_wait(ws_smem_u32(&s_full[b]), (bi / WS_NBUF) & 1);
            const int *gk = gk0 + b * 32;
            const int bkm = __reduce_max_sync(0xffffffffu, lane < nb ? gk[lane] : 0);
            run_kmax = max(run_kmax, bkm);
#pragma unroll
            for (int q = 0; q < NP; ++q) {
                if (t2[q] < bkm) bs_accumulate(acc[q], planes_saddr + (uint32_t)(b * gb * kmax) * 16u, gk_saddr + b * 128u,
                                               t1[q], t2[q], nb, kmax);
            }
            __syncwarp();
            if (lane == 0) ws_mbar_arrive(ws_smem_u32(&s_empty[b]));
            if (last) {
#pragma unroll
                for (int q = 0; q < NP; ++q) {
                    if (t2[q] < run_kmax) {
                        int row = rbase + t2[q];
                        if (row >= rows) row -= rows;
                        const int d = t2[q] - t1[q];
                        uint4 *cell = tile + ((size_t)row * cells + (d - 1)) * 4;
#pragma unroll
                        for (int x = 0; x < 4; ++x) {
                            uint4 v = cell[x];
                            v.x += acc[q][4 * x + 0]; v.y += acc[q][4 * x + 1];
                            v.z += acc[q][4 * x + 2]; v.w += acc[q][4 * x + 3];
                            cell[x] = v;
                        }
                    }
                }
            }
        }
        ws_pair_barrier(npt);
        {
            unsigned long long sum = 0;
            const int per_row = cells * 16;
            int row = (int)((flushed_upto + 1) % rows);
            for (int64_t pj = flushed_upto + 1; pj <= flushed_upto + rows - 1; ++pj) {
                uint32_t *base = tile32 + (size_t)row * per_row;
                for (int w = threadIdx.x; w < per_row; w += npt) {
                    const uint32_t v = base[w];
                    if (v) {
                        const int d = (w >> 4) + 1, ab = w & 15;
                        atomicAdd(cnt.cell(W, pj - d, pj) + (ab >> 2) * HX_NSYM + (ab & 3), v);
                        sum += v;
                    }
                }
                if (++row == rows) row = 0;
            }
            t_crumbs += sum;
        }
    }
    if (errbits) atomicOr(err, (int)errbits);
    flush_totals(n_slices, t_crumbs + n_rcrumbs, (unsigned long long)n_codes - n_notcov, n_sent, totals);
}

}

static std::atomic<bool> g_unsorted_seen{false};
bool hx_unsorted_seen() { return g_unsorted_seen.load(std::memory_order_relaxed); }
void hx_note_unsorted() { g_unsorted_seen.store(true, std::memory_order_relaxed); }

__global__ void k_flag_not(const int *__restrict__ in, int *__restrict__ out) {
    if (threadIdx.x == 0) *out = !*in;
}

static int launch_ingest(hx_matrix *h, const int32_t *d_rank, const int64_t *d_off, const uint8_t *d_codes,
                         int64_t n_reads, int64_t *run_end, const int *ok);

int hx_launch_ingest(hx_matrix *h, const int32_t *d_rank, const int64_t *d_off,
                     const uint8_t *d_codes, int64_t n_reads) {
    return launch_ingest(h, d_rank, d_off, d_codes, n_reads, nullptr, nullptr);
}

int hx_launch_ingest_presorted(hx_matrix *h, const int32_t *d_rank, const int64_t *d_off,
                               const uint8_t *d_codes, int64_t n_reads, int64_t *run_end, const int *ok) {
    return launch_ingest(h, d_rank, d_off, d_codes, n_reads, run_end, ok);
}

static int launch_ingest(hx_matrix *h, const int32_t *d_rank, const int64_t *d_off, const uint8_t *d_codes,
                         int64_t n_reads, int64_t *run_end, const int *ok) {
    if (n_reads <= 0) return HX_OK;
    const bool presorted = run_end != nullptr;
    if (!presorted) run_end = h->d_run_end.p;
    int sms = 148;
    cudaDeviceGetAttribute(&sms, cudaDevAttrMultiProcessorCount, h->device);
    if (h->use.ingest_sms > 0 && h->use.ingest_sms < sms) sms = h->use.ingest_sms;
    const int *sorted_flag = presorted ? ok : h->d_flags.p + 4;
    constexpr int GBLOCK = 256;
    const int64_t gwant = (n_reads + (GBLOCK / 32) - 1) / (GBLOCK / 32);
    const int ggrid = (int)(gwant < (int64_t)sms * 8 ? gwant : (int64_t)sms * 8);

    const int kmax = h->W + 1;
    const bool bs_possible = kmax >= 2 && kmax <= BS_KMAX;
    const bool use_bs = (h->use.ingest_kernel == 2 || h->use.ingest_kernel == 4 || h->use.ingest_kernel == 5 || h->use.ingest_kernel == 6)
                            ? bs_possible : (h->use.ingest_kernel == 0 && bs_possible);
    const bool use_umma = use_bs && hx_umma_possible(h) &&
                          (h->use.ingest_kernel == 6 || (h->use.ingest_kernel == 0 && n_reads >= 64 * ((int64_t)h->N + 1)));
    const bool fused = h->peer_world > 1;
    const bool use_long = !use_bs && (h->use.ingest_kernel == 3 || (h->use.ingest_kernel == 0 && kmax >= 2));
    const bool use_lumma = kmax >= 2 && (h->use.ingest_kernel == 7 ||
                                         (h->use.ingest_kernel == 0 && !use_bs &&
                                          hx_lumma_scratch_bytes(h, n_reads) <= ((int64_t)24 << 30)));

    const bool lumma_fallback = !presorted && use_bs && !use_lumma && h->use.ingest_kernel == 0 && hx_unsorted_seen() &&
                                hx_lumma_scratch_bytes(h, n_reads) <= ((int64_t)24 << 30);
    h->use.prepass_ran = !presorted && !use_lumma && (use_long || use_bs);
    HX_CUDA(cudaEventRecord(h->ev0, h->stream));
    if (use_lumma) {
        int rc = hx_launch_ingest_lumma(h, d_rank, d_off, d_codes, n_reads, presorted ? ok : nullptr);
        if (rc) return rc;
    } else if (use_long) {
        if (!presorted) {
            HX_CUDA(hx_fill_async(h->d_flags.p + 4, 1, sizeof(int), h->stream));
            k_prepass<<<(unsigned)((n_reads + 255) / 256), 256, 0, h->stream>>>(d_rank, n_reads, h->N, h->d_flags.p + 4,
                                                                                run_end, h->d_err.p);
            h->use.launches++;
        }
        int rc = hx_launch_ingest_long(h, d_rank, d_off, d_codes, n_reads, sorted_flag);
        if (rc) return rc;
        if (!presorted) {
            k1_pairs_red<GBLOCK><<<ggrid, GBLOCK, 0, h->stream>>>(d_rank, d_off, d_codes, n_reads, h->N, h->W,
                                                                  hx_cnt_ref(h), h->d_totals.p, h->d_err.p, sorted_flag, 0);
            h->use.launches++;
        }
    } else if (!use_bs) {
        k1_pairs_red<GBLOCK><<<ggrid, GBLOCK, 0, h->stream>>>(d_rank, d_off, d_codes, n_reads, h->N, h->W, hx_cnt_ref(h),
                                                              h->d_totals.p, h->d_err.p, sorted_flag, presorted ? 2 : 1);
        h->use.launches++;
    } else {
        if (!presorted) {
            k_prepass_init<<<(unsigned)((h->N + 2 + 255) / 256), 256, 0, h->stream>>>(h->d_flags.p + 4, run_end, use_umma ? h->N + 2 : 0);
            k_prepass<<<(unsigned)((n_reads + 255) / 256), 256, 0, h->stream>>>(d_rank, n_reads, h->N, h->d_flags.p + 4,
                                                                                run_end, h->d_err.p);
            h->use.launches += 2;
        }
        const int npairs = kmax * (kmax - 1) / 2;
        if (use_umma) {
            int rc = hx_launch_ingest_umma(h, d_rank, d_off, d_codes, n_reads, run_end, sorted_flag);
            if (rc) return rc;
        } else
        if (h->use.ingest_kernel == 5 || (h->use.ingest_kernel != 4 && kmax > 32)) {
            const int np = npairs > 512 ? 2 : 1;
            const int pw = ((npairs + np - 1) / np + 31) / 32;
            int bw = np == 1 && kmax <= 32 ? 20 - pw : 8;
            if (pw + bw > 32) bw = 32 - pw;
            const int block = (pw + bw) * 32;
            int gb = BS_GB;
            while (gb > 4 && WsLayout{kmax, gb}.bytes() > (size_t)((np == 1 ? 100 : 200) * 1024)) gb >>= 1;
            const size_t smem = WsLayout{kmax, gb}.bytes();
#define HX_WS_LAUNCH(KW_, NP_, MAXT_, MINB_)                                                                  \
    do {                                                                                                       \
        auto kern = fused ? k1_bitsliced_ws<KW_, NP_, MAXT_, MINB_, true> : k1_bitsliced_ws<KW_, NP_, MAXT_, MINB_, false>; \
        HX_CUDA(cudaFuncSetAttribute(kern, cudaFuncAttributeMaxDynamicSharedMemorySize, (int)smem));           \
        int occ = 1;                                                                                           \
        HX_CUDA(cudaOccupancyMaxActiveBlocksPerMultiprocessor(&occ, kern, block, smem));                       \
        if (occ < 1) occ = 1;                                                                                  \
        int64_t grid = (int64_t)sms * occ;                                                                     \
        const int64_t max_useful = (n_reads + 255) / 256;                                                      \
        if (grid > max_useful) grid = max_useful;                                                              \
        kern<<<(unsigned)grid, block, smem, h->stream>>>(d_rank, d_off, d_codes, n_reads, h->N, h->W, kmax,    \
                                                         gb, pw, hx_cnt_ref(h), h->d_totals.p, h->d_err.p, sorted_flag, \
                                                         run_end);                                        \
    } while (0)
            if (np == 2) HX_WS_LAUNCH(14, 2, 1024, 1);
            else if (kmax > 32) HX_WS_LAUNCH(14, 1, 1024, 1);
            else HX_WS_LAUNCH(8, 1, 640, 2);
#undef HX_WS_LAUNCH
        } else {
        int gb = BS_GB;
        while (gb > 4 && BsLayout{kmax, gb}.bytes() > (size_t)200 * 1024) gb >>= 1;
        const size_t smem = BsLayout{kmax, gb}.bytes();
        const int np = npairs > 1024 ? 2 : 1;
        int block = ((npairs + np - 1) / np + 31) / 32 * 32;
        if (block < 128) block = 128;
        if (block > 1024) block = 1024;
#define HX_BS_LAUNCH(KW_, NP_, MAXT_, MINB_)                                                                  \
    do {                                                                                                       \
        auto kern = fused ? k1_bitsliced<KW_, NP_, MAXT_, MINB_, true> : k1_bitsliced<KW_, NP_, MAXT_, MINB_, false>;       \
        HX_CUDA(cudaFuncSetAttribute(kern, cudaFuncAttributeMaxDynamicSharedMemorySize, (int)smem));           \
        int occ = 1;                                                                                           \
        HX_CUDA(cudaOccupancyMaxActiveBlocksPerMultiprocessor(&occ, kern, block, smem));                       \
        if (occ < 1) occ = 1;                                                                                  \
        int64_t grid = (int64_t)sms * occ;                                                                     \
        const int64_t max_useful = (n_reads + 255) / 256;               \
        if (grid > max_useful) grid = max_useful;                                                              \
        kern<<<(unsigned)grid, block, smem, h->stream>>>(d_rank, d_off, d_codes, n_reads, h->N, h->W, kmax,    \
                                                         gb, hx_cnt_ref(h), h->d_totals.p, h->d_err.p, sorted_flag,   \
                                                         run_end);                                        \
    } while (0)
        if (np == 2) HX_BS_LAUNCH(14, 2, 1024, 1);
        else if (kmax > 32) HX_BS_LAUNCH(14, 1, 1024, 1);
        else HX_BS_LAUNCH(8, 1, 512, 2);
#undef HX_BS_LAUNCH
        }
        h->use.launches++;
        if (lumma_fallback) {
            k_flag_not<<<1, 32, 0, h->stream>>>(h->d_flags.p + 4, h->d_flags.p + 5);
            h->use.launches++;
            int rc = hx_launch_ingest_lumma(h, d_rank, d_off, d_codes, n_reads, h->d_flags.p + 5);
            if (rc) return rc;
        } else if (!presorted) {
            k1_pairs_red<GBLOCK><<<ggrid, GBLOCK, 0, h->stream>>>(d_rank, d_off, d_codes, n_reads, h->N, h->W,
                                                                  hx_cnt_ref(h), h->d_totals.p, h->d_err.p, sorted_flag, 0);
            h->use.launches++;
        }
    }
    h->use.cnt_fresh = false;
    HX_CUDA(cudaGetLastError());
    HX_CUDA(cudaEventRecord(h->ev1, h->stream));
    h->use.ev_rec = true;
    return HX_OK;
}
```

gretel_b200/csrc/ingest_umma.cu:

```cuda
#include <stdlib.h>

#include <algorithm>

#include "hx_internal.cuh"
#include "ingest_common.cuh"

namespace {

#ifndef UM_EXP_WARPS_N
#define UM_EXP_WARPS_N 24
#endif
constexpr int UM_RD_WARPS = 8;
constexpr int UM_EXP_WARPS = UM_EXP_WARPS_N;
constexpr int UM_THREADS = (UM_RD_WARPS + UM_EXP_WARPS) * 32;
#ifndef UM_GATE_NS
#define UM_GATE_NS 200
#endif
constexpr int UM_JB = 256;
constexpr int UM_NACC = 4;
constexpr int UM_TMEM_COLS = 128 * UM_NACC;
constexpr uint32_t UM_ACC_COUNT = 1u << 19;

#ifdef UM_PROFILE
__device__ unsigned long long um_prof[32];
#define UM_T(var) const long long var = clock64()
#define UM_ACC(slot, expr) prof_acc[slot] += (unsigned long long)(expr)
#else
#define UM_T(var)
#define UM_ACC(slot, expr)
#endif

struct UmLayout {
    int kmax;
    __host__ __device__ int ch() const { return kmax <= 16 ? 4 : 8; }
    __host__ __device__ size_t slot_bytes() const { return (size_t)32 * 16 * ch(); }
    __host__ __device__ size_t tile_bytes() const { return (size_t)(kmax + 1) * (kmax - 1) * 64; }
    __host__ __device__ size_t bytes() const {
        return (size_t)UM_EXP_WARPS * slot_bytes() + tile_bytes() + 1024;
    }
};

__device__ __forceinline__ uint32_t um_shl(uint32_t v, uint32_t amt) {
    uint32_t r;
    asm("shl.b32 %0, %1, %2;" : "=r"(r) : "r"(v), "r"(amt));
    return r;
}

__device__ __forceinline__ uint64_t um_desc(uint32_t saddr, uint32_t lbo_bytes) {
    uint64_t d = 0;
    d |= (uint64_t)((saddr >> 4) & 0x3fffu);
    d |= (uint64_t)((lbo_bytes >> 4) & 0x3fffu) << 16;
    d |= (uint64_t)((128u >> 4) & 0x3fffu) << 32;
    d |= (uint64_t)1 << 46;
    return d;
}

__device__ __forceinline__ uint32_t um_idesc(int n_cols) {
    return (2u << 4) | (1u << 15) | (1u << 16) | ((uint32_t)(n_cols >> 3) << 17) | ((128u >> 4) << 24);
}

__device__ __forceinline__ void um_mma(uint32_t tmem_d, uint64_t desc, uint32_t idesc, uint32_t accumulate) {
    asm volatile(
        "{\n\t.reg .pred p;\n\t"
        "setp.ne.b32 p, %3, 0;\n\t"
        "tcgen05.mma.cta_group::1.kind::i8 [%0], %1, %1, %2, p;\n\t}"
        ::"r"(tmem_d), "l"(desc), "r"(idesc), "r"(accumulate)
        : "memory");
}
__device__ __forceinline__ void um_commit(uint32_t bar) {
    asm volatile("tcgen05.commit.cta_group::1.mbarrier::arrive::one.shared::cluster.b64 [%0];" ::"r"(bar) : "memory");
}
__device__ __forceinline__ void um_fence_before() { asm volatile("tcgen05.fence::before_thread_sync;" ::: "memory"); }
__device__ __forceinline__ void um_fence_after() { asm volatile("tcgen05.fence::after_thread_sync;" ::: "memory"); }
__device__ __forceinline__ void um_ld16(uint32_t taddr, uint32_t (&v)[16]) {
    asm volatile(
        "tcgen05.ld.sync.aligned.32x32b.x16.b32 {%0, %1, %2, %3, %4, %5, %6, %7, %8, %9, %10, %11, %12, %13, %14, %15}, [%16];"
        : "=r"(v[0]), "=r"(v[1]), "=r"(v[2]), "=r"(v[3]), "=r"(v[4]), "=r"(v[5]), "=r"(v[6]), "=r"(v[7]), "=r"(v[8]),
          "=r"(v[9]), "=r"(v[10]), "=r"(v[11]), "=r"(v[12]), "=r"(v[13]), "=r"(v[14]), "=r"(v[15])
        : "r"(taddr)
        : "memory");
}
__device__ __forceinline__ unsigned um_ld_acquire(uint32_t addr) {
    unsigned v;
    asm volatile("ld.acquire.cta.shared.u32 %0, [%1];" : "=r"(v) : "r"(addr) : "memory");
    return v;
}
__device__ __forceinline__ void um_st16_zero(uint32_t taddr) {
    const uint32_t z = 0;
    asm volatile(
        "tcgen05.st.sync.aligned.32x32b.x16.b32 [%0], {%1, %1, %1, %1, %1, %1, %1, %1, %1, %1, %1, %1, %1, %1, %1, %1};"
        ::"r"(taddr), "r"(z)
        : "memory");
}
__device__ __forceinline__ void um_wait_st() { asm volatile("tcgen05.wait::st.sync.aligned;" ::: "memory"); }
__device__ __forceinline__ void um_wait_ld() { asm volatile("tcgen05.wait::ld.sync.aligned;" ::: "memory"); }

struct UmWalk {
    const int32_t *run_rank;
    const int64_t *run_stop;
    int64_t hi, cur, p_stop;
    int n_runs, j, p_rank;
    int64_t start, n;
    int r;
    unsigned ri;

    __device__ __forceinline__ void fetch() {
        if (j < n_runs) { p_rank = run_rank[j]; p_stop = run_stop[j]; }
    }
    __device__ __forceinline__ void init(const int32_t *rr, const int64_t *rs, int n_runs_, int64_t lo_, int64_t hi_) {
        run_rank = rr; run_stop = rs; n_runs = n_runs_; hi = hi_; cur = lo_; ri = 0u - 1u; r = 0; start = lo_; n = 0;
        int a = 0, b = n_runs_;
        while (a < b) {
            const int m = (a + b) >> 1;
            if (run_stop[m] > lo_) b = m; else a = m + 1;
        }
        j = a;
        p_rank = 0; p_stop = 0;
        fetch();
    }
    __device__ __forceinline__ bool next_run() {
        while (cur < hi && j < n_runs) {
            const int64_t stop = p_stop;
            r = p_rank;
            ++j;
            fetch();
            if (stop <= cur) continue;
            const int64_t run_hi = stop < hi ? stop : hi;
            start = cur;
            n = run_hi - cur;
            cur = run_hi;
            ++ri;
            return true;
        }
        cur = hi;
        return false;
    }
};

__global__ void __launch_bounds__(1024)
k_run_list(const int64_t *__restrict__ run_end, int N, int32_t *__restrict__ run_rank, int64_t *__restrict__ run_stop,
           int *__restrict__ n_runs) {
    __shared__ int s_warp[32];
    const int lane = threadIdx.x & 31, warp = threadIdx.x >> 5;
    const int per = (N + 1 + 1023) / 1024;
    const int i0 = (int)threadIdx.x * per, i1 = min(i0 + per, N + 1);
    int mine = 0;
    for (int i = i0; i < i1; ++i) mine += run_end[i] >= 0;
    int incl = mine;
#pragma unroll
    for (int o = 1; o < 32; o <<= 1) {
        const int v = __shfl_up_sync(0xffffffffu, incl, o);
        if (lane >= o) incl += v;
    }
    if (lane == 31) s_warp[warp] = incl;
    __syncthreads();
    if (warp == 0) {
        int w = s_warp[lane];
#pragma unroll
        for (int o = 1; o < 32; o <<= 1) {
            const int v = __shfl_up_sync(0xffffffffu, w, o);
            if (lane >= o) w += v;
        }
        s_warp[lane] = w;
    }
    __syncthreads();
    int pos = incl - mine + (warp ? s_warp[warp - 1] : 0);
    for (int i = i0; i < i1; ++i) {
        const int64_t e = run_end[i];
        if (e >= 0) { run_rank[pos] = i; run_stop[pos] = e; ++pos; }
    }
    if (threadIdx.x == 1023) *n_runs = s_warp[31];
}

template <int CH>
__device__ __forceinline__ void um_load_read(const uint8_t *__restrict__ codes, int64_t o, int kg,
                                             uint32_t (&wd)[CH + 1], unsigned &mis) {
    const uint8_t *__restrict__ c = codes + o;
    mis = (unsigned)(reinterpret_cast<uintptr_t>(c) & 3u);
    const uint32_t *__restrict__ cw = reinterpret_cast<const uint32_t *>(c - mis);
    const int nwg = (kg + 6) >> 2;
#pragma unroll
    for (int w = 0; w <= CH; ++w) wd[w] = w < nwg ? __ldg(cw + w) : 0u;
}

template <int CH>
__device__ __forceinline__ void um_expand_read(const uint32_t (&wd)[CH + 1], unsigned mis, int kb, int kg,
                                               uint32_t rowaddr, uint32_t &rare_or, uint32_t &x0) {
    const unsigned sh = 8u * mis;
    const int kb8 = 8 * kb;
    rare_or = 0;
    x0 = 0x04040404u;
#pragma unroll
    for (int ch = 0; ch < CH; ++ch) {
        uint32_t o0 = 0, o1 = 0, o2 = 0, o3 = 0;
        if (4 * ch < kg) {
            const uint32_t xx = __funnelshift_r(wd[ch], wd[ch + 1], sh);
            const int c8 = min(max(kb8 - 32 * ch, 0), 32);
            const uint32_t inval = um_shl(0xffffffffu, (uint32_t)c8);
            rare_or |= xx & 0xfcfcfcfcu & ~inval;
            const uint32_t x = (xx & ~inval) | (0x04040404u & inval);
            if (ch == 0) x0 = x;
            const uint32_t y = x << 3;
            o0 = um_shl(1u, __byte_perm(y, 0u, 0x4440u));
            o1 = um_shl(1u, __byte_perm(y, 0u, 0x4441u));
            o2 = um_shl(1u, __byte_perm(y, 0u, 0x4442u));
            o3 = um_shl(1u, y >> 24);
        }
        asm volatile("st.shared.v4.u32 [%0], {%1, %2, %3, %4};" ::"r"(rowaddr + (uint32_t)ch * 128u), "r"(o0), "r"(o1),
                     "r"(o2), "r"(o3)
                     : "memory");
    }
}

template <int CH, bool FUSED>
__global__ void __launch_bounds__(UM_THREADS, 1)
k1_umma(const int32_t *__restrict__ rank, const int64_t *__restrict__ off, const uint8_t *__restrict__ codes,
        int64_t n_reads, int N, int W, int kmax, const HxCnt cnt_in, unsigned long long *__restrict__ totals,
        int *__restrict__ err, const int *__restrict__ sorted_flag, const int32_t *__restrict__ run_rank,
        const int64_t *__restrict__ run_stop, const int *__restrict__ n_runs_ptr, int4 *__restrict__ jobs_all,
        int jobs_cap, int read_w, int rank_w) {
    extern __shared__ __align__(1024) uint8_t um_smem[];
    UM_T(k_begin);
    HxCnt cnt = cnt_in;
    if (!FUSED) { cnt.world = 1; cnt.rows_per = 1; cnt.peer = nullptr; }
    __shared__ __align__(8) unsigned long long s_slot[UM_EXP_WARPS];
    __shared__ __align__(8) unsigned long long s_acc_full[UM_NACC];
    __shared__ int s_runkg[UM_NACC];
    __shared__ unsigned s_runs_read;
    __shared__ uint32_t s_tmem;
    __shared__ int s_jb_off[UM_JB + 1], s_jb_start[UM_JB], s_jb_n[UM_JB], s_jb_r[UM_JB], s_jb_warp[UM_JB / 32];
    __shared__ int s_njobs;
    if (!*sorted_flag) return;

    constexpr int ROWB = 16 * CH;
    constexpr uint32_t LBO = 128u * CH;
    constexpr uint32_t SLOTB = 32u * ROWB;

    const int lane = threadIdx.x & 31, warp = threadIdx.x >> 5;
    int64_t lo, hi;
    hx_weighted_slice(rank, off, n_reads, read_w, rank_w, lo, hi);
    if (lo >= hi) return;

    const int rows = kmax + 1, cells = kmax - 1;
    const uint32_t x_saddr = ws_smem_u32(um_smem);
    uint4 *const tile = reinterpret_cast<uint4 *>(um_smem + (size_t)UM_EXP_WARPS * SLOTB);
    uint32_t *const tile32 = reinterpret_cast<uint32_t *>(tile);

    for (size_t w = threadIdx.x; w < (size_t)rows * cells * 4; w += blockDim.x) tile[w] = make_uint4(0, 0, 0, 0);
    if (threadIdx.x == 0) {
        s_runs_read = 0;
        for (int s = 0; s < UM_NACC; ++s) s_runkg[s] = 0;
        for (int e = 0; e < UM_EXP_WARPS; ++e) ws_mbar_init(ws_smem_u32(&s_slot[e]), 1);
        for (int s = 0; s < UM_NACC; ++s) ws_mbar_init(ws_smem_u32(&s_acc_full[s]), UM_ACC_COUNT);
        asm volatile("fence.mbarrier_init.release.cluster;" ::: "memory");
    }
    if (warp == 0) {
        asm volatile("tcgen05.alloc.cta_group::1.sync.aligned.shared::cta.b32 [%0], %1;" ::"r"(ws_smem_u32(&s_tmem)),
                     "r"((uint32_t)UM_TMEM_COLS)
                     : "memory");
        asm volatile("tcgen05.relinquish_alloc_permit.cta_group::1.sync.aligned;" ::: "memory");
    }
    um_fence_before();
    __syncthreads();
    um_fence_after();
    const uint32_t tmem_base = s_tmem;
    if (warp < UM_RD_WARPS) {
        for (int st = warp >> 2; st < UM_NACC; st += 2) {
            const uint32_t t0 = tmem_base + (uint32_t)st * 128u + ((uint32_t)((warp & 3) * 32) << 16);
#pragma unroll
            for (int cb = 0; cb < 128; cb += 16) um_st16_zero(t0 + (uint32_t)cb);
        }
        um_wait_st();
    }
    um_fence_before();
    __syncthreads();
    um_fence_after();

    unsigned long long t_crumbs = 0;
    unsigned n_slices = 0, n_codes = 0, n_notcov = 0, n_sent = 0, n_rcrumbs = 0, errbits = 0;
#ifdef UM_PROFILE
    unsigned long long prof_acc[8] = {0, 0, 0, 0, 0, 0, 0, 0};
#endif

    UmWalk wk;
    wk.init(run_rank, run_stop, *n_runs_ptr, lo, hi);

    int4 *const myjobs = jobs_all + (size_t)blockIdx.x * jobs_cap;
    {
        const int n_runs_all = *n_runs_ptr;
        const int j0 = wk.j;
        int job_base = 0;
        for (int jb = j0; jb < n_runs_all; jb += UM_JB) {
            int ng = 0;
            if (threadIdx.x < UM_JB) {
                const int j = jb + (int)threadIdx.x;
                int64_t s0 = hi;
                if (j < n_runs_all) {
                    const int64_t prev = j > 0 ? run_stop[j - 1] : 0;
                    s0 = prev > lo ? prev : lo;
                }
                if (s0 < hi) {
                    const int64_t stop = run_stop[j];
                    const int64_t e0 = stop < hi ? stop : hi;
                    ng = (int)((e0 - s0 + 31) >> 5);
                    s_jb_start[threadIdx.x] = (int)(s0 - lo);
                    s_jb_n[threadIdx.x] = (int)(e0 - s0);
                    s_jb_r[threadIdx.x] = run_rank[j];
                }
                int incl = ng;
#pragma unroll
                for (int o = 1; o < 32; o <<= 1) {
                    const int v = __shfl_up_sync(0xffffffffu, incl, o);
                    if (lane >= o) incl += v;
                }
                if (lane == 31) s_jb_warp[warp] = incl;
                s_jb_off[threadIdx.x + 1] = incl;
            }
            __syncthreads();
            if (threadIdx.x < UM_JB) {
                int before = 0;
                for (int w2 = 0; w2 < warp; ++w2) before += s_jb_warp[w2];
                const int incl = s_jb_off[threadIdx.x + 1] + before;
                __syncwarp();
                s_jb_off[threadIdx.x + 1] = incl;
                if (threadIdx.x == 0) s_jb_off[0] = 0;
            }
            __syncthreads();
            const int batch_jobs = s_jb_off[UM_JB];
            for (int q = threadIdx.x; q < batch_jobs; q += blockDim.x) {
                int a = 0, b = UM_JB - 1;
                while (a < b) {
                    const int m = (a + b) >> 1;
                    if (s_jb_off[m + 1] > q) b = m; else a = m + 1;
                }
                const int g = q - s_jb_off[a];
                const int n_run = s_jb_n[a];
                const int nj = min(32, n_run - 32 * g);
                myjobs[job_base + q] = make_int4(s_jb_start[a] + 32 * g, nj | (g == 0 ? (min(n_run, 2048) << 8) : 0), s_jb_r[a],
                                                 jb - j0 + a);
            }
            job_base += batch_jobs;
            const bool more = s_jb_off[UM_JB] > s_jb_off[UM_JB - 1];
            __syncthreads();
            if (!more) break;
        }
        if (threadIdx.x == 0) s_njobs = job_base;
        __syncthreads();
    }
    UM_T(k_roles);

    if (warp >= UM_RD_WARPS) {
        const int e = warp - UM_RD_WARPS;
        const uint32_t slot_addr = x_saddr + (uint32_t)e * SLOTB;
        const uint32_t slot_bar = ws_smem_u32(&s_slot[e]);
        const uint64_t desc = um_desc(slot_addr, LBO);
        const uint32_t idesc0 = um_idesc(0);
        const uint32_t accfull_addr = ws_smem_u32(&s_acc_full[0]);
        const uint32_t rowaddr = slot_addr + (uint32_t)(lane >> 3) * LBO + (uint32_t)(lane & 7) * 16u;
#ifndef UM_PF_READS
#define UM_PF_READS 2048
#endif
        constexpr int64_t PF_READS = UM_PF_READS;
        unsigned njobs = 0;
        const int n_jobs = s_njobs;
        auto get_job = [&](int idx) -> int4 {
            int4 j = make_int4(0, 0, 0, 0);
            if (idx < n_jobs) j = myjobs[idx];
            return j;
        };
        auto load_off = [&](const int4 &j, int64_t &o, int64_t &o1) {
            o = 0; o1 = 0;
            if (lane < (j.y & 0xff)) { const int64_t *p = off + lo + j.x + lane; o = p[0]; o1 = p[1]; }
        };
        const uint32_t runs_addr = ws_smem_u32(&s_runs_read);
        int ji = e;
        int4 cur = get_job(ji);
        int64_t o, o1;
        load_off(cur, o, o1);
        while (cur.y) {
            UM_T(tA);
            ji += UM_EXP_WARPS;
            const int4 nxt = get_job(ji);
            int64_t on, o1n;
            load_off(nxt, on, o1n);
            if (lane == 0 && (cur.y >> 8)) {
                const int64_t start = lo + cur.x, n_run = cur.y >> 8;
                const int64_t pf0 = start + PF_READS;
                if (pf0 < hi) {
                    const int64_t np = min(n_run, hi - pf0);
                    bs_prefetch_l2(off + pf0, (uint32_t)((np + 1) * 8));
                    const int nj = cur.y & 0xff;
                    const int64_t o_lo = o, o_hi = off[start + nj];
                    const int64_t per_read16 = ((o_hi - o_lo) << 4) / nj;
                    bs_prefetch_l2(codes + o_lo + ((PF_READS * per_read16) >> 4), (uint32_t)(((np * per_read16) >> 4) + 64));
                }
            }
            const int r = cur.z;
            const unsigned cur_ri = (unsigned)cur.w;
            const int s = cur_ri % UM_NACC;
            const uint64_t kd = (uint64_t)(o1 - o);
            const int klim = min(W + 1, N - r);
            int kb = 0;
            if (kd >= 2) {
                if (r < 0 || kd > (uint64_t)(klim < 0 ? 0 : klim)) errbits |= 1;
                else kb = (int)kd;
            }
            n_slices += kb >= 2;
            n_codes += kb;
            const int kg = __reduce_max_sync(0xffffffffu, kb);
            UM_T(tC);
            uint32_t wd[CH + 1];
            unsigned mis;
            um_load_read<CH>(codes, o, kg, wd, mis);
            UM_T(tD);
            if (cur_ri >= (unsigned)UM_NACC) {
                const unsigned need = cur_ri - UM_NACC + 1;
                while (um_ld_acquire(runs_addr) < need) __nanosleep(UM_GATE_NS);
            }
            ws_mbar_wait(slot_bar, (njobs & 1) ^ 1);
            um_fence_after();
            UM_T(tE);
            uint32_t rare_or, x0;
            um_expand_read<CH>(wd, mis, kb, kg, rowaddr, rare_or, x0);
            asm volatile("fence.proxy.async.shared::cta;" ::: "memory");
            __syncwarp();
            if (lane == 0) {
                if (kg >= 2) {
                    const int c4 = (kg + 3) >> 2;
                    atomicMax(&s_runkg[s], kg);
                    asm volatile("fence.acq_rel.cta;" ::: "memory");
                    um_mma(tmem_base + (uint32_t)s * 128u, desc, idesc0 | ((uint32_t)c4 << 18), 1u);
                }
                um_commit(slot_bar);
                um_commit(accfull_addr + 8u * (uint32_t)s);
            }
            ++njobs;
            UM_T(tG);
            if (r == 0 || r + kg >= N) {
                if (kb >= 2) {
                    const uint8_t *__restrict__ c = codes + o;
                    const unsigned a0 = x0 & 0xffu;
                    if (r == 0 && sym_valid_from(a0)) {
                        atomicAdd(cnt.cell(W, 0, 1) + HX_SYM_GAP * HX_NSYM + a0, 1u);
                        n_sent++;
                    }
                    if (r + kb == N && !(kb == 2 && r == 0)) {
                        const unsigned ap = c[kb - 2], bl = c[kb - 1];
                        if (sym_valid_from(ap) && bl <= 6) {
                            atomicAdd(cnt.cell(W, N, N + 1) + bl * HX_NSYM + HX_SYM_GAP, 1u);
                            n_sent++;
                        }
                    }
                }
            }
            unsigned rm = __ballot_sync(0xffffffffu, kb >= 2 && rare_or != 0);
            while (rm) {
                const int src = __ffs(rm) - 1;
                rm &= rm - 1;
                const int64_t o2 = __shfl_sync(0xffffffffu, o, src);
                const int k2 = __shfl_sync(0xffffffffu, kb, src);
                bs_rare_read<false>(codes + o2, k2, r, W, cnt, n_rcrumbs, n_notcov, errbits);
            }
            UM_T(tH);
            UM_ACC(0, tC - tA); UM_ACC(1, tD - tC); UM_ACC(2, tE - tD); UM_ACC(3, tG - tE); UM_ACC(4, tH - tG); UM_ACC(5, 1);
            cur = nxt; o = on; o1 = o1n;
        }
#ifdef UM_PROFILE
        if (lane == 0) for (int i = 0; i < 6; ++i) atomicAdd(&um_prof[i], prof_acc[i]);
#endif
    } else {
        const int npt = UM_RD_WARPS * 32;
        const int q = warp & 3, half = warp >> 2;
        const int m = q * 32 + lane, t1 = m >> 2, a = m & 3;
        const int per_row = cells * 16;
        auto word_off = [](int w) { return (w >> 4) * HX_CELL + ((w & 15) >> 2) * HX_NSYM + (w & 3); };
        const int goff0 = word_off(threadIdx.x), goff1 = word_off(threadIdx.x + npt);
        static_assert(UM_RD_WARPS * 32 * 2 >= 31 * 16, "two tile words per readout thread cover a band row");
        int64_t flushed_upto = (int64_t)max(rank[lo], 0) + 1;
        while (wk.next_run()) {
            const int r = wk.r;
            const unsigned ri = wk.ri;
            const int s = ri % UM_NACC;
            UM_T(r0);
            if ((int64_t)r + 1 > flushed_upto) {
                const bool slots_reused = (int64_t)r - flushed_upto >= 2;
                const int64_t lastrow = min((int64_t)r + 1, flushed_upto + rows - 2);
                unsigned long long sum = 0;
                int row = (int)((unsigned)(flushed_upto + 1) % (unsigned)rows);
                for (int64_t pj = flushed_upto + 1; pj <= lastrow; ++pj) {
                    uint32_t *base = tile32 + (size_t)row * per_row;
                    uint32_t *grow = cnt.cell(W, pj - 1, pj);
                    for (int w = threadIdx.x, k2 = 0; w < per_row; w += npt, ++k2) {
                        const uint32_t v = base[w];
                        if (v) {
                            atomicAdd(grow + (k2 ? goff1 : goff0), v);
                            base[w] = 0;
                            sum += v;
                        }
                    }
                    if (++row == rows) row = 0;
                }
                t_crumbs += sum;
                flushed_upto = (int64_t)r + 1;
                if (slots_reused) ws_pair_barrier(npt);
            }
            const int rbase = (int)((unsigned)(r + 1) % (unsigned)rows);
            UM_T(r1);
            if (threadIdx.x == 0) {
                const uint32_t ng = (uint32_t)((wk.n + 31) >> 5);
                asm volatile("mbarrier.arrive.release.cta.shared::cta.b64 _, [%0], %1;" ::"r"(ws_smem_u32(&s_acc_full[s])),
                             "r"(UM_ACC_COUNT - ng)
                             : "memory");
            }
            ws_mbar_wait(ws_smem_u32(&s_acc_full[s]), (ri / UM_NACC) & 1);
            um_fence_after();
            UM_T(r2);
            const int kg = *reinterpret_cast<volatile int *>(&s_runkg[s]);
            const int ncols = 4 * kg;
            const uint32_t taddr = tmem_base + (uint32_t)s * 128u + ((uint32_t)(q * 32) << 16);
            if (kg >= 2) {
                if (q * 32 < ncols - 4) {
                    for (int cb = q * 32 + 16 * half; cb < ncols; cb += 32) {
                        uint32_t v[16];
                        um_ld16(taddr + (uint32_t)cb, v);
                        um_wait_ld();
#pragma unroll
                        for (int j = 0; j < 4; ++j) {
                            const int t2 = (cb >> 2) + j;
                            if (t2 > t1 && t2 < kg) {
                                int row = rbase + t2;
                                if (row >= rows) row -= rows;
                                uint4 *cell = tile + ((size_t)row * cells + (t2 - t1 - 1)) * 4 + a;
                                uint4 c = *cell;
                                c.x += v[4 * j + 0]; c.y += v[4 * j + 1]; c.z += v[4 * j + 2]; c.w += v[4 * j + 3];
                                *cell = c;
                            }
                        }
                    }
                }
                const int ncols16 = 16 * ((kg + 3) >> 2);
                for (int cb = 16 * half; cb < ncols16; cb += 32) um_st16_zero(taddr + (uint32_t)cb);
                um_wait_st();
            }
            um_fence_before();
            ws_pair_barrier(npt);
            if (threadIdx.x == 0) {
                s_runkg[s] = 0;
                asm volatile("st.release.cta.shared.u32 [%0], %1;" ::"r"(ws_smem_u32(&s_runs_read)), "r"(ri + 1) : "memory");
            }
            UM_T(r3);
            UM_ACC(0, r1 - r0); UM_ACC(1, r2 - r1); UM_ACC(2, r3 - r2); UM_ACC(3, 1);
        }
        {
            unsigned long long sum = 0;
            int row = (int)((flushed_upto + 1) % rows);
            for (int64_t pj = flushed_upto + 1; pj <= flushed_upto + rows - 1; ++pj) {
                uint32_t *base = tile32 + (size_t)row * per_row;
                for (int w = threadIdx.x; w < per_row; w += npt) {
                    const uint32_t v = base[w];
                    if (v) {
                        const int d = (w >> 4) + 1, ab = w & 15;
                        atomicAdd(cnt.cell(W, pj - d, pj) + (ab >> 2) * HX_NSYM + (ab & 3), v);
                        sum += v;
                    }
                }
                if (++row == rows) row = 0;
            }
            t_crumbs += sum;
        }
#ifdef UM_PROFILE
        if (threadIdx.x == 0) for (int i = 0; i < 4; ++i) atomicAdd(&um_prof[16 + i], prof_acc[i]);
#endif
    }
    UM_T(k_roles_end);
    if (errbits) atomicOr(err, (int)errbits);
    um_fence_before();
    flush_totals(n_slices, t_crumbs + n_rcrumbs, (unsigned long long)n_codes - n_notcov, n_sent, totals);
#ifdef UM_PROFILE
    {
        const long long k_end = clock64();
        if (lane == 0) {
            atomicAdd(&um_prof[24], (unsigned long long)(k_roles - k_begin));
            atomicAdd(&um_prof[25], (unsigned long long)(k_roles_end - k_roles));
            atomicAdd(&um_prof[26], (unsigned long long)(k_end - k_roles_end));
            atomicMax(&um_prof[27], (unsigned long long)(k_end - k_begin));
            if (warp >= UM_RD_WARPS) atomicMax(&um_prof[28], (unsigned long long)(k_roles_end - k_roles));
            else atomicMax(&um_prof[29], (unsigned long long)(k_roles_end - k_roles));
        }
    }
#endif
    if (warp == 0) {
        um_fence_after();
        asm volatile("tcgen05.dealloc.cta_group::1.sync.aligned.b32 %0, %1;" ::"r"(tmem_base), "r"((uint32_t)UM_TMEM_COLS)
                     : "memory");
    }
}

}

#ifdef UM_PROFILE
extern "C" int hx_debug_um_prof(unsigned long long *out, int reset) {
    if (cudaMemcpyFromSymbol(out, um_prof, sizeof(unsigned long long) * 32) != cudaSuccess) return -1;
    if (reset) {
        unsigned long long z[32] = {0};
        cudaMemcpyToSymbol(um_prof, z, sizeof(z));
    }
    return 0;
}
#endif

bool hx_umma_possible(const hx_matrix *h) {
    const int kmax = h->W + 1;
    return kmax >= 2 && kmax <= 32;
}

int hx_launch_ingest_umma(hx_matrix *h, const int32_t *d_rank, const int64_t *d_off, const uint8_t *d_codes,
                          int64_t n_reads, const int64_t *run_end, const int *sorted_flag) {
    int sms = 148;
    cudaDeviceGetAttribute(&sms, cudaDevAttrMultiProcessorCount, h->device);
    if (h->use.ingest_sms > 0 && h->use.ingest_sms < sms) sms = h->use.ingest_sms;
    const int kmax = h->W + 1;
    const bool fused = h->peer_world > 1;
    const size_t smem = UmLayout{kmax}.bytes();
    int64_t grid = sms;
    const int64_t max_useful = (n_reads + 255) / 256;
    if (grid > max_useful) grid = max_useful;
    int32_t *run_rank = reinterpret_cast<int32_t *>(h->d_run_list.p);
    int64_t *run_stop = reinterpret_cast<int64_t *>(h->d_run_list.p) + (((size_t)h->N + 2 + 1) / 2);
    int *n_runs = reinterpret_cast<int *>(run_stop + (size_t)h->N + 2);
    k_run_list<<<1, 1024, 0, h->stream>>>(run_end, h->N, run_rank, run_stop, n_runs);
    h->use.launches++;
    static const int read_w = [] { const char *e = getenv("HX_UM_READ_W"); const int v = e ? atoi(e) : HX_SLICE_READ_W; return v < 1 ? 1 : v; }();
    static const int rank_w = [] { const char *e = getenv("HX_UM_RANK_W"); const int v = e ? atoi(e) : HX_SLICE_RANK_W; return v < 0 ? 0 : v; }();
    const int64_t per = (((n_reads + grid - 1) / grid + 1) * (kmax + read_w) + ((int64_t)rank_w * (h->N + 2) + grid - 1) / grid) / read_w + 2;
    const int64_t jobs_cap = per / 32 + std::min<int64_t>((int64_t)h->N + 2, per) + 2;
    HX_CHECK_ARG(jobs_cap < ((int64_t)1 << 31) && per < ((int64_t)1 << 31));
    const int64_t jobs_bytes = jobs_cap * grid * (int64_t)sizeof(int4);
    if (jobs_bytes > h->d_jobs.cap) HX_CUDA(h->d_jobs.grow(jobs_bytes + jobs_bytes / 8, h->stream));
#define HX_UM_LAUNCH(CH_)                                                                                       \
    do {                                                                                                        \
        auto kern = fused ? k1_umma<CH_, true> : k1_umma<CH_, false>;                                           \
        HX_CUDA(cudaFuncSetAttribute(kern, cudaFuncAttributeMaxDynamicSharedMemorySize, (int)smem));            \
        kern<<<(unsigned)grid, UM_THREADS, smem, h->stream>>>(d_rank, d_off, d_codes, n_reads, h->N, h->W, kmax, \
                                                              hx_cnt_ref(h), h->d_totals.p, h->d_err.p, sorted_flag, \
                                                              run_rank, run_stop, n_runs,                       \
                                                              h->d_jobs.p, (int)jobs_cap, read_w, rank_w); \
    } while (0)
    if (kmax <= 16) HX_UM_LAUNCH(4);
    else HX_UM_LAUNCH(8);
#undef HX_UM_LAUNCH
    h->use.launches++;
    HX_CUDA(cudaGetLastError());
    return HX_OK;
}
```

gretel_b200/csrc/wire.cu:

```cuda
#include <algorithm>
#include <stdlib.h>
#include <thread>

#include "dense_enc.h"
#include "hx_internal.cuh"

namespace {

constexpr int WI = 16;
constexpr int WB = 256 * WI;

__device__ __forceinline__ int32_t esc_lookup(const int64_t *__restrict__ idx, const int32_t *__restrict__ delta,
                                              int64_t n_esc, int64_t j) {
    int64_t lo = 0, hi = n_esc;
    while (lo < hi) {
        const int64_t mid = (lo + hi) >> 1;
        if (idx[mid] < j) lo = mid + 1; else hi = mid;
    }
    return lo < n_esc && idx[lo] == j ? delta[lo] : 255;
}

template <int KB>
__device__ __forceinline__ void load_reads(const uint8_t *__restrict__ rd, const void *__restrict__ kl, int64_t j0,
                                           int64_t n, const int64_t *__restrict__ esc_idx,
                                           const int32_t *__restrict__ esc_delta, int64_t n_esc, int32_t (&d)[WI],
                                           int32_t (&k)[WI]) {
    if (j0 + WI <= n) {
        const uint4 a = *reinterpret_cast<const uint4 *>(rd + j0);
        const uint32_t aw[4] = {a.x, a.y, a.z, a.w};
#pragma unroll
        for (int i = 0; i < WI; ++i) d[i] = (int32_t)((aw[i >> 2] >> (8 * (i & 3))) & 0xffu);
        if (KB == 1) {
            const uint4 b = *reinterpret_cast<const uint4 *>(static_cast<const uint8_t *>(kl) + j0);
            const uint32_t bw[4] = {b.x, b.y, b.z, b.w};
#pragma unroll
            for (int i = 0; i < WI; ++i) k[i] = (int32_t)((bw[i >> 2] >> (8 * (i & 3))) & 0xffu);
        } else {
            const uint4 *p = reinterpret_cast<const uint4 *>(static_cast<const uint16_t *>(kl) + j0);
            const uint4 b0 = p[0], b1 = p[1];
            const uint32_t bw[8] = {b0.x, b0.y, b0.z, b0.w, b1.x, b1.y, b1.z, b1.w};
#pragma unroll
            for (int i = 0; i < WI; ++i) k[i] = (int32_t)((bw[i >> 1] >> (16 * (i & 1))) & 0xffffu);
        }
    } else {
#pragma unroll
        for (int i = 0; i < WI; ++i) {
            const int64_t j = j0 + i;
            d[i] = j < n ? (int32_t)rd[j] : 0;
            k[i] = j < n ? (KB == 1 ? (int32_t)static_cast<const uint8_t *>(kl)[j]
                                    : (int32_t)static_cast<const uint16_t *>(kl)[j])
                         : 0;
        }
    }
    if (n_esc) {
#pragma unroll
        for (int i = 0; i < WI; ++i)
            if (d[i] == 255) {
                const int32_t e = esc_lookup(esc_idx, esc_delta, n_esc, j0 + i);
                d[i] = e < 0 ? 0 : e;
            }
    }
}

template <int KB>
__global__ void __launch_bounds__(256)
k_dense_partials(const uint8_t *__restrict__ rd, const void *__restrict__ kl, int64_t n,
                 const int64_t *__restrict__ esc_idx, const int32_t *__restrict__ esc_delta, int64_t n_esc,
                 int64_t *__restrict__ partials ) {
    __shared__ int64_t sh[2][8];
    int32_t d[WI], k[WI];
    load_reads<KB>(rd, kl, (int64_t)blockIdx.x * WB + (int64_t)threadIdx.x * WI, n, esc_idx, esc_delta, n_esc, d, k);
    int64_t sd = 0, sk = 0;
#pragma unroll
    for (int i = 0; i < WI; ++i) { sd += d[i]; sk += k[i]; }
#pragma unroll
    for (int o = 16; o > 0; o >>= 1) {
        sd += __shfl_xor_sync(0xffffffffu, sd, o);
        sk += __shfl_xor_sync(0xffffffffu, sk, o);
    }
    if ((threadIdx.x & 31) == 0) { sh[0][threadIdx.x >> 5] = sd; sh[1][threadIdx.x >> 5] = sk; }
    __syncthreads();
    if (threadIdx.x < 2) {
        int64_t t = 0;
        for (int w = 0; w < 8; ++w) t += sh[threadIdx.x][w];
        partials[2 * (int64_t)blockIdx.x + threadIdx.x] = t;
    }
}

__global__ void __launch_bounds__(1024) k_dense_spine(int64_t *__restrict__ partials, int64_t nblk, int64_t n_codes,
                                                      int *__restrict__ ok, int *__restrict__ err) {
    __shared__ int64_t sh[2][32];
    __shared__ int64_t carry[2];
    const int lane = threadIdx.x & 31, warp = threadIdx.x >> 5;
    if (threadIdx.x < 2) carry[threadIdx.x] = 0;
    __syncthreads();
    for (int64_t b0 = 0; b0 < nblk; b0 += 1024) {
        const int64_t b = b0 + threadIdx.x;
        const int64_t vd = b < nblk ? partials[2 * b] : 0, vk = b < nblk ? partials[2 * b + 1] : 0;
        int64_t sd = vd, sk = vk;
#pragma unroll
        for (int o = 1; o < 32; o <<= 1) {
            const int64_t td = __shfl_up_sync(0xffffffffu, sd, o), tk = __shfl_up_sync(0xffffffffu, sk, o);
            if (lane >= o) { sd += td; sk += tk; }
        }
        if (lane == 31) { sh[0][warp] = sd; sh[1][warp] = sk; }
        __syncthreads();
        if (warp == 0) {
            int64_t wd = sh[0][lane], wk = sh[1][lane];
#pragma unroll
            for (int o = 1; o < 32; o <<= 1) {
                const int64_t td = __shfl_up_sync(0xffffffffu, wd, o), tk = __shfl_up_sync(0xffffffffu, wk, o);
                if (lane >= o) { wd += td; wk += tk; }
            }
            sh[0][lane] = wd;
            sh[1][lane] = wk;
        }
        __syncthreads();
        const int64_t base_d = carry[0] + (warp ? sh[0][warp - 1] : 0), base_k = carry[1] + (warp ? sh[1][warp - 1] : 0);
        if (b < nblk) { partials[2 * b] = base_d + sd - vd; partials[2 * b + 1] = base_k + sk - vk; }
        __syncthreads();
        if (threadIdx.x == 0) { carry[0] += sh[0][31]; carry[1] += sh[1][31]; }
        __syncthreads();
    }
    if (threadIdx.x == 0) {
        const bool good = carry[1] == n_codes;
        *ok = good ? 1 : 0;
        if (!good) atomicOr(err, 1);
    }
}

template <int KB>
__global__ void __launch_bounds__(256)
k_dense_apply(const uint8_t *__restrict__ rd, const void *__restrict__ kl, int64_t n,
              const int64_t *__restrict__ esc_idx, const int32_t *__restrict__ esc_delta, int64_t n_esc,
              const int64_t *__restrict__ partials, int32_t *__restrict__ rank, int64_t *__restrict__ off ,
              int N, int64_t *__restrict__ run_end) {
    __shared__ int64_t sh[2][8];
    const int lane = threadIdx.x & 31, warp = threadIdx.x >> 5;
    const int64_t j0 = (int64_t)blockIdx.x * WB + (int64_t)threadIdx.x * WI;
    int32_t d[WI], k[WI];
    load_reads<KB>(rd, kl, j0, n, esc_idx, esc_delta, n_esc, d, k);
    int64_t sd = 0, sk = 0;
#pragma unroll
    for (int i = 0; i < WI; ++i) { sd += d[i]; sk += k[i]; }
    int64_t id = sd, ik = sk;
#pragma unroll
    for (int o = 1; o < 32; o <<= 1) {
        const int64_t td = __shfl_up_sync(0xffffffffu, id, o), tk = __shfl_up_sync(0xffffffffu, ik, o);
        if (lane >= o) { id += td; ik += tk; }
    }
    if (lane == 31) { sh[0][warp] = id; sh[1][warp] = ik; }
    __syncthreads();
    int64_t run_d = partials[2 * (int64_t)blockIdx.x] + id - sd;
    int64_t run_k = partials[2 * (int64_t)blockIdx.x + 1] + ik - sk;
    for (int w = 0; w < warp; ++w) { run_d += sh[0][w]; run_k += sh[1][w]; }
    int32_t d_next = 0;
    if (j0 + WI < n) {
        d_next = (int32_t)rd[j0 + WI];
        if (n_esc && d_next == 255) {
            d_next = esc_lookup(esc_idx, esc_delta, n_esc, j0 + WI);
            if (d_next < 0) d_next = 0;
        }
    }
#pragma unroll
    for (int i = 0; i < WI; ++i) {
        const int64_t j = j0 + i;
        run_d += d[i];
        if (j < n) {
            rank[j] = (int32_t)(run_d <= (int64_t)N + 1 ? run_d : (int64_t)N + 1);
            const int32_t dn = i + 1 < WI ? d[i + 1] : d_next;
            if ((j + 1 == n || dn != 0) && run_d <= N) run_end[run_d] = j + 1;
        }
        if (j <= n) off[j] = run_k;
        run_k += k[i];
    }
}

__global__ void k_unpack_2bit(const uint32_t *__restrict__ in, int64_t n_words, uint4 *__restrict__ out) {
    const int64_t i = (int64_t)blockIdx.x * blockDim.x + threadIdx.x;
    if (i >= n_words) return;
    const uint32_t w = in[i];
    uint32_t o[4];
#pragma unroll
    for (int b = 0; b < 4; ++b) {
        uint32_t x = (w >> (8 * b)) & 0xffu;
        x = (x | (x << 12)) & 0x000f000fu;
        o[b] = (x | (x << 6)) & 0x03030303u;
    }
    out[i] = make_uint4(o[0], o[1], o[2], o[3]);
}

__global__ void k_patch_exceptions(const uint32_t *__restrict__ pos, int64_t n_exc, int64_t n_codes,
                                   uint8_t *__restrict__ codes, int *__restrict__ err) {
    const int64_t i = (int64_t)blockIdx.x * blockDim.x + threadIdx.x;
    if (i >= n_exc) return;
    const uint32_t p = pos[i];
    if ((int64_t)p >= n_codes) { atomicOr(err, 2); return; }
    codes[p] = (uint8_t)(codes[p] + 4);
}

inline int64_t al16(int64_t x) { return (x + 15) & ~(int64_t)15; }

struct WireTrace {
    static constexpr int MAXC = 32;
    cudaEvent_t ev[MAXC][5];
    int64_t bytes[MAXC];
    int n = 0;
    bool made = false;
};
WireTrace g_trace;
const bool g_trace_on = getenv("HX_WIRE_TRACE") != nullptr;
void trace_mark(int which, cudaStream_t s) {
    if (!g_trace_on || g_trace.n >= WireTrace::MAXC) return;
    if (!g_trace.made) {
        for (auto &row : g_trace.ev) for (auto &e : row) cudaEventCreate(&e);
        g_trace.made = true;
    }
    cudaEventRecord(g_trace.ev[g_trace.n][which], s);
}

}

void hx_wire_trace_dump() {
    if (!g_trace_on || g_trace.n == 0) return;
    cudaEventSynchronize(g_trace.ev[g_trace.n - 1][3]);
    for (int c = 0; c < g_trace.n; ++c) {
        float t[5];
        for (int i = 0; i < 5; ++i) cudaEventElapsedTime(&t[i], g_trace.ev[0][0], g_trace.ev[c][i]);
        fprintf(stderr, "[wire] chunk %d: copy %.3f..%.3f ms (%.1f GB/s)  decode ..%.3f  expand %.3f..%.3f\n", c, t[0], t[1],
                g_trace.bytes[c] / ((t[1] - t[0]) * 1e6), t[2], t[4], t[3]);
    }
    g_trace.n = 0;
}

void hx_wire_free(hx_matrix *h) {
    for (int s = 0; s < HX_WIRE_SETS; ++s) {
        hx_wire_set &w = h->wire[s];
        w.raw.release(h->stream); w.rank.release(h->stream); w.off.release(h->stream);
        w.codes.release(h->stream); w.partials.release(h->stream); w.run_end.release(h->stream);
        if (w.copied) cudaEventDestroy(w.copied);
        if (w.consumed) cudaEventDestroy(w.consumed);
        if (w.decoded) cudaEventDestroy(w.decoded);
        w = hx_wire_set{};
    }
    for (int s = 0; s < 2; ++s) {
        if (h->pin_ev[s]) cudaEventDestroy(h->pin_ev[s]);
        if (h->pin[s]) cudaFreeHost(h->pin[s]);
        h->pin[s] = nullptr; h->pin_cap[s] = 0; h->pin_ev[s] = nullptr; h->pin_busy[s] = false;
    }
    if (h->copy_stream) cudaStreamDestroy(h->copy_stream);
    if (h->decode_stream) cudaStreamDestroy(h->decode_stream);
    h->copy_stream = nullptr;
    h->decode_stream = nullptr;
}

static int ingest_dense_impl(hx_matrix *h, const uint8_t *rank_delta, const int64_t *esc_idx,
                             const int32_t *esc_delta, int64_t n_esc, const void *klen, int32_t klen_bytes,
                             const uint8_t *codes2, const uint32_t *exc_pos, int64_t n_exc, int64_t n_reads,
                             int64_t n_codes, int64_t totals[4], const uint8_t *raw_codes) {
    HX_CHECK_ARG(h && n_reads >= 0 && n_codes >= 0 && n_esc >= 0 && n_exc >= 0);
    HX_CHECK_ARG(klen_bytes == 1 || klen_bytes == 2);
    HX_CHECK_ARG(n_codes < ((int64_t)1 << 32));
    HX_CUDA(cudaSetDevice(h->device));
    if (n_reads > 0) {
        HX_CHECK_ARG(rank_delta && klen && (codes2 || raw_codes || n_codes == 0) && (exc_pos || n_exc == 0));
        HX_CHECK_ARG(n_esc == 0 || (esc_idx && esc_delta));
        cudaStream_t st = h->stream;
        if (!h->copy_stream) HX_CUDA(cudaStreamCreateWithFlags(&h->copy_stream, cudaStreamNonBlocking));
        if (!h->decode_stream) HX_CUDA(cudaStreamCreateWithFlags(&h->decode_stream, cudaStreamNonBlocking));
        cudaStream_t ds = h->decode_stream;
        hx_wire_set &w = h->wire[h->use.wire_next];
        h->use.wire_next = (h->use.wire_next + 1) % HX_WIRE_SETS;
        const int64_t n_words = (n_codes + 15) / 16;
        const int64_t n_words_sent = raw_codes ? 0 : n_words;
        const int64_t o_rd = 0, o_kl = o_rd + al16(n_reads), o_c2 = o_kl + al16(n_reads * klen_bytes);
        const int64_t o_ex = o_c2 + al16(n_words_sent * 4), o_ei = o_ex + al16(n_exc * 4), o_ed = o_ei + al16(n_esc * 8);
        const int64_t raw_bytes = o_ed + al16(n_esc * 4) + 16;
        const int64_t nblk = (n_reads + 1 + WB - 1) / WB;
        for (int s2 = 0; s2 < HX_WIRE_SETS; ++s2) {
            hx_wire_set &ws = h->wire[s2];
            if (!ws.copied) {
                HX_CUDA(cudaEventCreateWithFlags(&ws.copied, cudaEventDisableTiming));
                HX_CUDA(cudaEventCreateWithFlags(&ws.consumed, cudaEventDisableTiming));
                HX_CUDA(cudaEventCreateWithFlags(&ws.decoded, cudaEventDisableTiming));
            }
            bool grew = false;
            auto fit = [&](auto &buf, int64_t need) {
                return need > buf.cap ? buf.grow(need + need / 8 + 256, st, &grew) : cudaSuccess;
            };
            HX_CUDA(fit(ws.raw, raw_bytes));
            HX_CUDA(fit(ws.rank, 4 * n_reads + 16));
            HX_CUDA(fit(ws.off, 8 * (n_reads + 1) + 16));
            HX_CUDA(fit(ws.codes, n_words * 16 + 32));
            HX_CUDA(fit(ws.partials, 16 * nblk + 32));
            HX_CUDA(ws.run_end.grow(8 * ((int64_t)h->N + 2), st, &grew));
            if (grew) HX_CUDA(cudaEventRecord(ws.consumed, st));
        }
        cudaStream_t cs = h->copy_stream;
        HX_CUDA(cudaStreamWaitEvent(cs, w.consumed, 0));
        trace_mark(0, cs);
        uint8_t *raw = w.raw.p;
        const uint8_t *hb = rank_delta;
        if (raw_codes && n_codes) HX_CUDA(cudaMemcpyAsync(w.codes.p, raw_codes, (size_t)n_codes, cudaMemcpyHostToDevice, cs));
        const bool blob = (const uint8_t *)klen == hb + o_kl && (n_codes == 0 || raw_codes || codes2 == hb + o_c2) &&
                          (n_exc == 0 || (const uint8_t *)exc_pos == hb + o_ex) &&
                          (n_esc == 0 || ((const uint8_t *)esc_idx == hb + o_ei && (const uint8_t *)esc_delta == hb + o_ed));
        if (blob) {
            const int64_t used = n_esc ? o_ed + n_esc * 4 : (n_exc ? o_ex + n_exc * 4 : (n_codes && !raw_codes ? o_c2 + (n_codes + 3) / 4
                                                                                        : o_kl + n_reads * klen_bytes));
            HX_CUDA(cudaMemcpyAsync(raw, hb, (size_t)used, cudaMemcpyHostToDevice, cs));
        } else {
        HX_CUDA(cudaMemcpyAsync(raw + o_rd, rank_delta, (size_t)n_reads, cudaMemcpyHostToDevice, cs));
        HX_CUDA(cudaMemcpyAsync(raw + o_kl, klen, (size_t)(n_reads * klen_bytes), cudaMemcpyHostToDevice, cs));
        if (n_esc) {
            HX_CUDA(cudaMemcpyAsync(raw + o_ei, esc_idx, (size_t)(n_esc * 8), cudaMemcpyHostToDevice, cs));
            HX_CUDA(cudaMemcpyAsync(raw + o_ed, esc_delta, (size_t)(n_esc * 4), cudaMemcpyHostToDevice, cs));
        }
        if (n_codes && !raw_codes) HX_CUDA(cudaMemcpyAsync(raw + o_c2, codes2, (size_t)((n_codes + 3) / 4), cudaMemcpyHostToDevice, cs));
        if (n_exc) HX_CUDA(cudaMemcpyAsync(raw + o_ex, exc_pos, (size_t)(n_exc * 4), cudaMemcpyHostToDevice, cs));
        }
        trace_mark(1, cs);
        HX_CUDA(cudaEventRecord(w.copied, cs));
        HX_CUDA(cudaStreamWaitEvent(ds, w.copied, 0));
        int *ok = reinterpret_cast<int *>(w.partials.p + 2 * nblk);
        const int64_t *d_ei = reinterpret_cast<const int64_t *>(raw + o_ei);
        const int32_t *d_ed = reinterpret_cast<const int32_t *>(raw + o_ed);
        HX_CUDA(hx_fill_async(w.run_end.p, 0xff, sizeof(int64_t) * ((size_t)h->N + 2), ds));
        h->use.launches++;
        if (klen_bytes == 1) {
            k_dense_partials<1><<<(unsigned)nblk, 256, 0, ds>>>(raw + o_rd, raw + o_kl, n_reads, d_ei, d_ed, n_esc, w.partials.p);
            k_dense_spine<<<1, 1024, 0, ds>>>(w.partials.p, nblk, n_codes, ok, h->d_err.p);
            k_dense_apply<1><<<(unsigned)nblk, 256, 0, ds>>>(raw + o_rd, raw + o_kl, n_reads, d_ei, d_ed, n_esc, w.partials.p,
                                                            w.rank.p, w.off.p, h->N, w.run_end.p);
        } else {
            k_dense_partials<2><<<(unsigned)nblk, 256, 0, ds>>>(raw + o_rd, raw + o_kl, n_reads, d_ei, d_ed, n_esc, w.partials.p);
            k_dense_spine<<<1, 1024, 0, ds>>>(w.partials.p, nblk, n_codes, ok, h->d_err.p);
            k_dense_apply<2><<<(unsigned)nblk, 256, 0, ds>>>(raw + o_rd, raw + o_kl, n_reads, d_ei, d_ed, n_esc, w.partials.p,
                                                            w.rank.p, w.off.p, h->N, w.run_end.p);
        }
        h->use.launches += 3;
        if (n_words_sent) {
            k_unpack_2bit<<<(unsigned)((n_words + 255) / 256), 256, 0, ds>>>(reinterpret_cast<const uint32_t *>(raw + o_c2),
                                                                            n_words, reinterpret_cast<uint4 *>(w.codes.p));
            h->use.launches++;
        }
        if (n_exc) {
            k_patch_exceptions<<<(unsigned)((n_exc + 255) / 256), 256, 0, ds>>>(
                reinterpret_cast<const uint32_t *>(raw + o_ex), n_exc, n_codes, w.codes.p, h->d_err.p);
            h->use.launches++;
        }
        HX_CUDA(cudaGetLastError());
        trace_mark(2, ds);
        HX_CUDA(cudaEventRecord(w.decoded, ds));
        HX_CUDA(cudaStreamWaitEvent(st, w.decoded, 0));
        int rc = hx_ensure_counts_buffer(h);
        if (rc) return rc;
        trace_mark(4, st);
        rc = hx_launch_ingest_presorted(h, w.rank.p, w.off.p, w.codes.p, n_reads, w.run_end.p, ok);
        if (rc) return rc;
        trace_mark(3, st);
        if (g_trace_on && g_trace.n < WireTrace::MAXC) g_trace.bytes[g_trace.n++] = raw_bytes;
        HX_CUDA(cudaEventRecord(w.consumed, st));
    }
    return totals ? hx_ingest_totals(h, totals) : HX_OK;
}

extern "C" int hx_ingest_host_dense(hx_matrix *h, const uint8_t *rank_delta, const int64_t *esc_idx,
                                    const int32_t *esc_delta, int64_t n_esc, const void *klen, int32_t klen_bytes,
                                    const uint8_t *codes2, const uint32_t *exc_pos, int64_t n_exc, int64_t n_reads,
                                    int64_t n_codes, int64_t totals[4]) {
    return ingest_dense_impl(h, rank_delta, esc_idx, esc_delta, n_esc, klen, klen_bytes, codes2, exc_pos, n_exc, n_reads,
                             n_codes, totals, nullptr);
}


int hx_ingest_host_pipelined(hx_matrix *h, const int32_t *rank, const int64_t *off, const uint8_t *codes, int64_t n_reads,
                             bool slim, int64_t *done_reads) {
    *done_reads = 0;
    int nt = 0;
    if (const char *e = getenv("HX_HOST_THREADS")) nt = atoi(e);
    if (nt <= 0) nt = (int)std::min(32u, std::max(1u, std::thread::hardware_concurrency()));
    const int64_t n_codes = off[n_reads] - off[0];
    constexpr int64_t CHUNK_CODES = (int64_t)32 << 20;
    int n_chunks = (int)std::max<int64_t>(slim ? 6 : 3, (n_codes + CHUNK_CODES - 1) / CHUNK_CODES);
    if (slim && nt > 8) nt = 8;
    if ((int64_t)n_chunks > n_reads) n_chunks = (int)n_reads;
    int64_t a = 0;
    static thread_local HxDensePlan plan;
    for (int c = 0; c < n_chunks; ++c) {
        int64_t b = n_reads;
        if (c + 1 < n_chunks) {
            const int64_t target = off[0] + n_codes * (c + 1) / n_chunks;
            b = std::lower_bound(off + a, off + n_reads, target) - off;
            if (b <= a) continue;
        }
        HxDensePlan &P = plan;
        int rc = hx_dense_begin(off + a, b - a, nt, (int64_t)h->W + 1, &P, slim);
        if (rc) return rc;
        const int slot = c & 1;
        if (h->pin_busy[slot]) { HX_CUDA(cudaEventSynchronize(h->pin_ev[slot])); h->pin_busy[slot] = false; }
        auto ensure_pin = [&](int64_t bytes, int64_t keep) -> int {
            if (bytes <= h->pin_cap[slot]) return HX_OK;
            const int64_t want = bytes + bytes / 8 + ((int64_t)1 << 20);
            uint8_t *np = nullptr;
            HX_CUDA(cudaHostAlloc((void **)&np, (size_t)want, cudaHostAllocPortable));
            if (keep > 0) memcpy(np, h->pin[slot], (size_t)keep);
            if (h->pin[slot]) cudaFreeHost(h->pin[slot]);
            h->pin[slot] = np;
            h->pin_cap[slot] = want;
            return HX_OK;
        };
        rc = ensure_pin(P.head_bytes + 16, 0);
        if (rc) return rc;
        if (!h->pin_ev[slot]) HX_CUDA(cudaEventCreateWithFlags(&h->pin_ev[slot], cudaEventDisableTiming));
        rc = hx_dense_pack(rank + a, off + a, codes, &P, h->pin[slot]);
        if (rc) return rc;
        rc = ensure_pin(P.bytes, P.head_bytes);
        if (rc) return rc;
        uint8_t *blob = h->pin[slot];
        hx_dense_finish(&P, blob);
        rc = ingest_dense_impl(h, blob, reinterpret_cast<const int64_t *>(blob + P.o_esc_idx),
                               reinterpret_cast<const int32_t *>(blob + P.o_esc_delta), P.n_esc, blob + P.o_klen,
                               P.klen_bytes, blob + P.o_codes2, reinterpret_cast<const uint32_t *>(blob + P.o_exc), P.n_exc,
                               b - a, P.n_codes, nullptr, slim ? codes + off[a] : nullptr);
        if (rc) return rc;
        HX_CUDA(cudaEventRecord(h->pin_ev[slot], h->copy_stream));
        h->pin_busy[slot] = true;
        a = b;
        *done_reads = a;
    }
    return HX_OK;
}
```

gretel_b200/hansel.py:

```python
from __future__ import annotations

import ctypes as C
import os

import numpy as np

from . import _lib

REF_SYMBOLS = ['A', 'C', 'G', 'T', 'N', '-', '_']
REF_UNSYMBOLS = ['N', '_']
_DENSE_BAND_LIMIT_BYTES = 2 << 30


def _default_device():
    return int(os.environ.get("GRETEL_B200_DEVICE", os.environ.get("LOCAL_RANK", "0")))


class Hansel:
    def __init__(self, symbols, unsymbols, n_snps, band_w=None, device=None, _handle=None,
                 v_site="from", candidates_skip_unsymbols=True):
        symbols = [str(s) for s in symbols]
        unsymbols = [str(s) for s in unsymbols]
        if len(symbols) != 7 or sorted(unsymbols) != sorted([symbols[4], symbols[6]]):
            raise NotImplementedError(
                "the CUDA kernels are specialised to Gretel's alphabet: 7 symbols with "
                "symbols[4] and symbols[6] as the unsymbols (gretel/util.py:83)")
        self.symbols = symbols
        self.unsymbols = unsymbols
        self.symbols_d = {s: s for s in symbols}
        self.symbols_i = {i: s for i, s in enumerate(symbols)}
        self._code = {s: i for i, s in enumerate(symbols)}
        self.n_snps = int(n_snps)
        self.n_slices = 0
        self.n_crumbs = 0
        self.L = 1
        self.v_site = v_site
        self.candidates_skip_unsymbols = candidates_skip_unsymbols
        self.device = _default_device() if device is None else int(device)
        if band_w is None:
            band_w = self.n_snps + 1
            if (self.n_snps + 2) * band_w * 49 * 4 > _DENSE_BAND_LIMIT_BYTES:
                raise ValueError("n_snps=%d needs an explicit band_w (max SNPs per read - 1); "
                                 "a full upper triangle would not be sensible" % self.n_snps)
        self.band_w = max(1, int(band_w))
        self._lib = _lib.load()
        if _handle is None:
            h = C.c_void_p()
            _lib.check(self._lib.hx_create(self.n_snps, self.band_w, self.device, C.byref(h)))
            _handle = h
        self._h = _handle
        self._spill = {}
        self._counts_cache = None

    @classmethod
    def init_matrix(cls, symbols, unsymbols, n_snps, band_w=None, device=None, **kw):
        return cls(symbols, unsymbols, n_snps, band_w=band_w, device=device, **kw)

    def copy(self):
        self.finalize()
        h = C.c_void_p()
        _lib.check(self._lib.hx_copy(self._h, C.byref(h)))
        o = Hansel(self.symbols, self.unsymbols, self.n_snps, band_w=self.band_w, device=self.device,
                   _handle=h, v_site=self.v_site, candidates_skip_unsymbols=self.candidates_skip_unsymbols)
        o.n_slices, o.n_crumbs, o.L = self.n_slices, self.n_crumbs, self.L
        o._spill = dict(self._spill)
        return o

    def close(self):
        if getattr(self, "_h", None) is not None and self._h:
            self._lib.hx_destroy(self._h)
            self._h = None

    def __del__(self):
        try:
            self.close()
        except Exception:
            pass

    @property
    def flags(self):
        f = 0
        if self.v_site == "to":
            f |= _lib.HX_F_VSITE_TO
        if not self.candidates_skip_unsymbols:
            f |= _lib.HX_F_KEEP_UNSYMBOLS
        return f

    def _touch(self):
        self._counts_cache = None

    def _sym(self, s):
        return self._code[str(s)]

    def encode_path(self, path):
        return np.fromiter((self._code[str(s)] for s in path), dtype=np.uint8, count=len(path))

    def decode_path(self, codes):
        return [self.symbols_d[self.symbols[int(c)]] for c in codes]

    def ingest_packed(self, rank, off, codes):
        rank = np.ascontiguousarray(rank, dtype=np.int32)
        off = np.ascontiguousarray(off, dtype=np.int64)
        codes = np.ascontiguousarray(codes, dtype=np.uint8)
        if len(off) != len(rank) + 1:
            raise ValueError("off must have len(rank)+1 entries")
        totals = np.zeros(4, dtype=np.int64)
        _lib.check(self._lib.hx_ingest_host(self._h, rank.ctypes.data, off.ctypes.data, codes.ctypes.data,
                                            len(rank), totals.ctypes.data))
        self._touch()
        return tuple(int(x) for x in totals)

    def ingest_packed_compact(self, rank, klen, codes4, n_codes):
        rank = np.ascontiguousarray(rank, dtype=np.int32)
        klen = np.ascontiguousarray(klen, dtype=np.uint16)
        codes4 = np.ascontiguousarray(codes4, dtype=np.uint8)
        if len(klen) != len(rank) or len(codes4) < (int(n_codes) + 1) // 2:
            raise ValueError("klen/codes4 do not match rank/n_codes")
        totals = np.zeros(4, dtype=np.int64)
        _lib.check(self._lib.hx_ingest_host_compact(self._h, rank.ctypes.data, klen.ctypes.data, codes4.ctypes.data,
                                                    len(rank), int(n_codes), totals.ctypes.data))
        self._touch()
        return tuple(int(x) for x in totals)

    def ingest_packed_dense(self, dense, wait=True):
        d = dense
        for a in d.arrays():
            if not a.flags["C_CONTIGUOUS"]:
                raise ValueError("dense arrays must be contiguous")
        if len(d.rank_delta) != d.n_reads or len(d.klen) != d.n_reads or len(d.codes2) < (d.n_codes + 3) // 4:
            raise ValueError("dense arrays do not match n_reads/n_codes")
        totals = np.zeros(4, dtype=np.int64)
        if not wait:
            self._dense_keepalive = getattr(self, "_dense_keepalive", []) + [d]
        _lib.check(self._lib.hx_ingest_host_dense(
            self._h, d.rank_delta.ctypes.data, d.esc_idx.ctypes.data, d.esc_delta.ctypes.data, len(d.esc_idx),
            d.klen.ctypes.data, int(d.klen.dtype.itemsize), d.codes2.ctypes.data, d.exc_pos.ctypes.data,
            len(d.exc_pos), d.n_reads, d.n_codes, totals.ctypes.data if wait else None))
        self._touch()
        return tuple(int(x) for x in totals) if wait else None

    def ingest_totals(self):
        totals = np.zeros(4, dtype=np.int64)
        try:
            _lib.check(self._lib.hx_ingest_totals(self._h, totals.ctypes.data))
        finally:
            self._dense_keepalive = []
        return tuple(int(x) for x in totals)

    def set_ingest_kernel(self, which):
        _lib.check(self._lib.hx_set_ingest_kernel(self._h, int(which)))

    def set_ingest_sms(self, n_sms):
        _lib.check(self._lib.hx_set_ingest_sms(self._h, int(n_sms)))

    def set_stream(self, stream_ptr):
        _lib.check(self._lib.hx_set_stream(self._h, stream_ptr))

    def counts_buffer(self):
        a, b = C.c_void_p(), C.c_void_p()
        na, nb = C.c_int64(), C.c_int64()
        _lib.check(self._lib.hx_counts_buffer(self._h, C.byref(a), C.byref(na), C.byref(b), C.byref(nb)))
        return a.value, na.value, b.value, nb.value

    def counts_pack(self, world):
        a, na = C.c_void_p(), C.c_int64()
        _lib.check(self._lib.hx_counts_pack(self._h, int(world), C.byref(a), C.byref(na)))
        return a.value, na.value

    def counts_unpack(self):
        o = C.c_int32()
        _lib.check(self._lib.hx_counts_unpack(self._h, C.byref(o)))
        self._touch()
        return o.value == 0

    def counts_unpack_async(self, stream=None):
        _lib.check(self._lib.hx_counts_unpack_async(self._h, C.c_void_p(stream or 0)))
        self._touch()

    def counts_pack_overflowed(self):
        o = C.c_int32()
        _lib.check(self._lib.hx_counts_pack_overflowed(self._h, C.byref(o)))
        return o.value != 0

    def counts_max(self):
        m = C.c_uint32()
        _lib.check(self._lib.hx_counts_max(self._h, C.byref(m)))
        return int(m.value)

    def ingest_device(self, d_rank_ptr, d_off_ptr, d_codes_ptr, n_reads):
        _lib.check(self._lib.hx_ingest_device(self._h, d_rank_ptr, d_off_ptr, d_codes_ptr, int(n_reads)))
        self._touch()

    def reset_counts(self):
        _lib.check(self._lib.hx_reset_counts(self._h))
        self._touch()

    def probe_expected_rows(self, d_rank_ptr, d_off_ptr, d_codes_ptr, n_reads, d_rows_ptr):
        _lib.check(self._lib.hx_probe_expected_rows(self._h, d_rank_ptr, d_off_ptr, d_codes_ptr, int(n_reads),
                                                    d_rows_ptr))

    def counts_row_sums(self, d_rows_ptr):
        _lib.check(self._lib.hx_counts_row_sums(self._h, d_rows_ptr))

    def counts_ipc_export(self, world):
        buf = C.create_string_buffer(64)
        _lib.check(self._lib.hx_counts_ipc_export(self._h, int(world), buf))
        return bytes(buf.raw)

    def counts_ipc_import(self, handles, my_rank):
        blob = b"".join(handles)
        _lib.check(self._lib.hx_counts_ipc_import(self._h, blob, len(handles), int(my_rank)))

    def counts_ipc_close(self):
        _lib.check(self._lib.hx_counts_ipc_close(self._h))

    def finalize(self):
        _lib.check(self._lib.hx_finalize_counts(self._h))
        self._touch()

    def sync(self):
        _lib.check(self._lib.hx_sync(self._h))

    @property
    def stream(self):
        s = C.c_void_p()
        _lib.check(self._lib.hx_stream(self._h, C.byref(s)))
        return s.value or 0

    def add_observation(self, symbol_from, symbol_to, pos_from, pos_to):
        a, b = self._sym(symbol_from), self._sym(symbol_to)
        rc = self._lib.hx_add_observation(self._h, a, b, int(pos_from), int(pos_to), 1.0)
        if rc == _lib.HX_E_BAND:
            key = (a, b, int(pos_from), int(pos_to))
            self._spill[key] = np.float32(self._spill.get(key, np.float32(0)) + np.float32(1))
        else:
            _lib.check(rc)
        self._touch()

    def get_observation(self, symbol_from, symbol_to, pos_from, pos_to):
        a, b = self._sym(symbol_from), self._sym(symbol_to)
        out = C.c_float()
        rc = self._lib.hx_get_observation(self._h, a, b, int(pos_from), int(pos_to), C.byref(out))
        if rc == _lib.HX_E_BAND:
            return float(self._spill.get((a, b, int(pos_from), int(pos_to)), 0.0))
        _lib.check(rc)
        return float(out.value)

    def reweight_observation(self, symbol_from, symbol_to, pos_from, pos_to, ratio):
        a, b = self._sym(symbol_from), self._sym(symbol_to)
        self.finalize()
        out = C.c_double()
        rc = self._lib.hx_reweight_observation(self._h, a, b, int(pos_from), int(pos_to), float(ratio), C.byref(out))
        if rc == _lib.HX_E_BAND:
            key = (a, b, int(pos_from), int(pos_to))
            old = float(self._spill.get(key, 0.0))
            new = old - float(ratio) * old
            if key in self._spill:
                self._spill[key] = np.float32(new)
            return old - new
        _lib.check(rc)
        self._touch()
        return float(out.value)

    def reweight_matrix(self, ratio):
        self.finalize()
        _lib.check(self._lib.hx_reweight_matrix(self._h, float(ratio)))
        for k in self._spill:
            self._spill[k] = np.float32(float(self._spill[k]) * (1.0 - float(ratio)))
        self._touch()

    def _counts_all(self):
        if self._counts_cache is None:
            self.finalize()
            out = np.zeros((self.n_snps + 1, 8), dtype=np.float64)
            _lib.check(self._lib.hx_counts_all(self._h, out.ctypes.data))
            self._counts_cache = out
        return self._counts_cache

    def get_counts_at(self, at_pos):
        row = self._counts_all()[int(at_pos)]
        d = {self.symbols_d[s]: float(row[i]) for i, s in enumerate(self.symbols) if row[i] > 0}
        d["total"] = float(row[7])
        return d

    def get_marginal_of_at(self, of_symbol, at_pos):
        row = self._counts_all()[int(at_pos)]
        if row[7] == 0:
            return 0.0
        return float(row[self._sym(of_symbol)] / row[7])

    def get_edge_weights_at(self, snp, current_path, debug=False):
        self.finalize()
        path = self.encode_path(current_path[:snp])
        w = np.zeros(7, dtype=np.float64)
        tot, mask = C.c_double(), C.c_int()
        _lib.check(self._lib.hx_edge_weights_at(self._h, int(snp), path.ctypes.data, int(self.L), self.flags,
                                                w.ctypes.data, C.byref(tot), C.byref(mask)))
        out = {self.symbols_d[s]: float(w[i]) for i, s in enumerate(self.symbols) if (mask.value >> i) & 1}
        out["total"] = float(tot.value)
        if debug:
            print(out)
        return out

    def generate_path_codes(self, original, L=None):
        self.finalize()
        original.finalize()
        path = np.zeros(self.n_snps + 1, dtype=np.uint8)
        out = np.zeros(3, dtype=np.float64)
        hole = C.c_int32()
        rc = self._lib.hx_generate_path(self._h, original._h, int(self.L if L is None else L), self.flags,
                                        path.ctypes.data, out.ctypes.data, C.byref(hole))
        if rc == _lib.HX_HOLE:
            return None, int(hole.value)
        _lib.check(rc)
        return path, float(out[0]), float(out[1]), float(out[2])

    def reweight_path_codes(self, path_codes, ratio):
        self.finalize()
        path_codes = np.ascontiguousarray(path_codes, dtype=np.uint8)
        if len(path_codes) != self.n_snps + 1:
            raise ValueError("path must have N+1 entries")
        out = C.c_double()
        _lib.check(self._lib.hx_reweight_path(self._h, path_codes.ctypes.data, float(ratio), C.byref(out)))
        self._touch()
        return float(out.value)

    def recover_codes(self, original, max_paths, min_remove=0.01, L=None):
        self.finalize()
        original.finalize()
        paths = np.zeros((max_paths, self.n_snps + 1), dtype=np.uint8)
        stats = np.zeros((max_paths, 5), dtype=np.float64)
        n = C.c_int32()
        _lib.check(self._lib.hx_recover(self._h, original._h, int(self.L if L is None else L), self.flags,
                                        int(max_paths), float(min_remove), paths.ctypes.data,
                                        stats.ctypes.data, C.byref(n)))
        self._touch()
        return paths[:n.value], stats[:n.value]

    def band(self):
        self.finalize()
        out = np.zeros((self.n_snps + 2, self.band_w, 7, 7), dtype=np.float32)
        _lib.check(self._lib.hx_band_to_host(self._h, out.ctypes.data))
        return out

    def load_band(self, band):
        self.finalize()
        band = np.ascontiguousarray(band, dtype=np.float32)
        if band.shape != (self.n_snps + 2, self.band_w, 7, 7):
            raise ValueError("band shape mismatch")
        _lib.check(self._lib.hx_band_from_host(self._h, band.ctypes.data))
        self._touch()

    def to_dense(self):
        self.finalize()
        P = self.n_snps + 2
        out = np.zeros((7, 7, P, P), dtype=np.float32)
        _lib.check(self._lib.hx_to_dense(self._h, out.ctypes.data))
        for (a, b, i, j), v in self._spill.items():
            out[a, b, i, j] = v
        return out

    def save_hansel_dump(self, path):
        np.savez_compressed(path, band=self.band(), n_snps=self.n_snps, band_w=self.band_w, L=self.L,
                            n_slices=self.n_slices, n_crumbs=self.n_crumbs, symbols=np.array(self.symbols),
                            unsymbols=np.array(self.unsymbols))

    @classmethod
    def load_hansel_dump(cls, path, device=None):
        z = np.load(path if str(path).endswith(".npz") else str(path) + ".npz")
        h = cls([str(s) for s in z["symbols"]], [str(s) for s in z["unsymbols"]], int(z["n_snps"]),
                band_w=int(z["band_w"]), device=device)
        h.load_band(z["band"])
        h.L, h.n_slices, h.n_crumbs = int(z["L"]), int(z["n_slices"]), int(z["n_crumbs"])
        return h

    def kernel_ms(self, which):
        ms = C.c_float()
        _lib.check(self._lib.hx_last_kernel_ms(self._h, {"ingest": 0, "walk": 1, "reweight": 2}[which], C.byref(ms)))
        return float(ms.value)

    def launch_count(self):
        n = C.c_int64()
        _lib.check(self._lib.hx_launch_count(self._h, C.byref(n)))
        return int(n.value)
```

include/hanselx.h:

```cpp
#ifndef HANSELX_H
#define HANSELX_H

#include <stdint.h>

#ifdef __cplusplus
extern "C" {
#endif

typedef struct hx_matrix hx_matrix;

typedef enum {
    HX_OK = 0,
    HX_HOLE = 1,
    HX_E_CUDA = -1,
    HX_E_ARG = -2,
    HX_E_BAND = -3,
    HX_E_READ = -4,
    HX_E_NOMEM = -5,
    HX_E_STATE = -6
} hx_status;

#define HX_F_VSITE_TO        1
#define HX_F_KEEP_UNSYMBOLS  2

const char *hx_last_error(void);
int hx_version(void);
int hx_device_count(int *n);

int hx_create(int32_t n_snps, int32_t band_w, int32_t device, hx_matrix **out);
int hx_destroy(hx_matrix *h);
int hx_copy(const hx_matrix *src, hx_matrix **out);
int hx_info(const hx_matrix *h, int32_t *n_snps, int32_t *band_w, int32_t *device);
int hx_stream(const hx_matrix *h, void **stream);
int hx_set_stream(hx_matrix *h, void *stream);
int hx_sync(hx_matrix *h);

int hx_ingest_host(hx_matrix *h, const int32_t *rank, const int64_t *off, const uint8_t *codes,
                   int64_t n_reads, int64_t totals[4]);
int hx_ingest_host_compact(hx_matrix *h, const int32_t *rank, const uint16_t *klen, const uint8_t *codes4,
                           int64_t n_reads, int64_t n_codes, int64_t totals[4]);
int hx_ingest_host_dense(hx_matrix *h, const uint8_t *rank_delta, const int64_t *esc_idx, const int32_t *esc_delta,
                         int64_t n_esc, const void *klen, int32_t klen_bytes, const uint8_t *codes2,
                         const uint32_t *exc_pos, int64_t n_exc, int64_t n_reads, int64_t n_codes,
                         int64_t totals[4]);
int hx_ingest_device(hx_matrix *h, const int32_t *d_rank, const int64_t *d_off,
                     const uint8_t *d_codes, int64_t n_reads);
int hx_set_ingest_kernel(hx_matrix *h, int which);
int hx_set_ingest_sms(hx_matrix *h, int n_sms);
int hx_ingest_totals(hx_matrix *h, int64_t totals[4]);
int hx_counts_buffer(hx_matrix *h, void **d_counts, int64_t *n_u32, void **d_totals, int64_t *n_i64);
int hx_counts_pack(hx_matrix *h, int32_t world, void **d_packed, int64_t *n_u32);
int hx_counts_unpack(hx_matrix *h, int32_t *overflowed);
int hx_counts_unpack_async(hx_matrix *h, void *stream);
int hx_counts_pack_overflowed(hx_matrix *h, int32_t *overflowed);
int hx_counts_max(hx_matrix *h, uint32_t *max_count);
int hx_counts_ipc_export(hx_matrix *h, int32_t world, void *handle_out);
int hx_counts_ipc_import(hx_matrix *h, const void *handles, int32_t world, int32_t my_rank);
int hx_counts_ipc_close(hx_matrix *h);
int hx_finalize_counts(hx_matrix *h);
int hx_reset_counts(hx_matrix *h);

int hx_add_observation(hx_matrix *h, int a, int b, int32_t i, int32_t j, float amount);
int hx_get_observation(hx_matrix *h, int a, int b, int32_t i, int32_t j, float *out);
int hx_reweight_observation(hx_matrix *h, int a, int b, int32_t i, int32_t j, double ratio,
                            double *removed);
int hx_reweight_matrix(hx_matrix *h, double ratio);
int hx_counts_all(hx_matrix *h, double *out);
int hx_marginal_of_at(hx_matrix *h, int sym, int32_t pos, double *out);
int hx_edge_weights_at(hx_matrix *h, int32_t snp, const uint8_t *path, int32_t L, int flags,
                       double weights[7], double *total, int *mask);

int hx_generate_path(hx_matrix *cur, hx_matrix *orig, int32_t L, int flags, uint8_t *out_path,
                     double out[3], int32_t *hole_site);
int hx_reweight_path(hx_matrix *h, const uint8_t *path, double ratio, double *removed);
int hx_recover(hx_matrix *cur, hx_matrix *orig, int32_t L, int flags, int32_t max_paths,
               double min_remove, uint8_t *paths, double *stats, int32_t *n_found);

typedef struct {
    int32_t *rank;
    int64_t *off;
    uint8_t *codes;
    int64_t n_reads, n_codes, n_records;
} hx_packed;
int hx_pack_bam(const char *bam_path, const char *contig, int32_t start_pos, int32_t end_pos,
                const int32_t *snp_pos, int32_t n_snps, int stepper, int n_threads, hx_packed *out);
int hx_pack_bam_ex(const char *bam_path, const char *contig, int32_t start_pos, int32_t end_pos,
                   const int32_t *snp_pos, int32_t n_snps, int stepper, int n_threads, int32_t max_depth,
                   hx_packed *out, double stage_seconds[6]);
void hx_pack_free(hx_packed *p);
typedef struct hx_dense {
    uint8_t *blob;
    int64_t blob_bytes, n_reads, n_codes, n_exc, n_esc;
    int64_t o_klen, o_codes2, o_exc, o_esc_idx, o_esc_delta;
    int32_t klen_bytes;
} hx_dense;
int hx_dense_encode(const int32_t *rank, const int64_t *off, const uint8_t *codes, int64_t n_reads, int n_threads,
                    hx_dense *out);
void hx_dense_free(hx_dense *d);
int hx_count_coverage(const char *bam_path, const char *contig, int32_t start0, int32_t end0, int n_threads,
                      uint32_t *out);
int hx_count_coverage_gpu(const char *bam_path, const char *contig, int32_t start0, int32_t end0, int n_threads,
                          int32_t device, uint32_t *out);
int hx_bam_contig_length(const char *bam_path, const char *contig, int32_t *length);
int hx_inflate_raw(const uint8_t *src, int64_t n, int64_t n_readable, uint8_t *dst, int64_t m, int32_t use_zlib);

int hx_probe_expected_rows(hx_matrix *h, const int32_t *d_rank, const int64_t *d_off, const uint8_t *d_codes,
                           int64_t n_reads, uint64_t *d_rows);
int hx_counts_row_sums(hx_matrix *h, uint64_t *d_rows);

int hx_device_math(int32_t device, int which, const double *x, double *y, int64_t n);

int hx_band_to_host(hx_matrix *h, float *out );
int hx_band_from_host(hx_matrix *h, const float *in);
int hx_to_dense(hx_matrix *h, float *out );
int hx_last_kernel_ms(hx_matrix *h, int which, float *ms);
int hx_launch_count(const hx_matrix *h, int64_t *n);

#ifdef __cplusplus
}
#endif
#endif
```

Baseline: 3414 billion.

## Replace run list with dense rank_end index built in fused vectorized prepass

Replaces the sparse run_end array with a dense rank_end table in which every rank slot holds its run boundary. It is filled by a single vectorized, grid-strided prepass that also computes the sortedness verdict through a last-block atomic, so the separate init and run-list kernels and a memset go away. The UMMA ingest kernel now looks up run bounds directly instead of binary-searching a compacted run list, and the final tile flush is spread across all threads after the role loop. This trades extra writes over rank gaps, with warp-cooperative filling for long gaps, for fewer launches and simpler run lookup. It also adds an API for querying whether the ingest input was sorted.

```diff
diff --git a/gretel_b200/_lib.py b/gretel_b200/_lib.py
--- a/gretel_b200/_lib.py
+++ b/gretel_b200/_lib.py
@@ -69,6 +69,7 @@
     "hx_to_dense": (_int, [_p, _p]),
     "hx_last_kernel_ms": (_int, [_p, _int, C.POINTER(_flt)]),
     "hx_launch_count": (_int, [_p, C.POINTER(_i64)]),
+    "hx_ingest_sorted": (_int, [_p, C.POINTER(C.c_int32)]),
 }
 
 class HxPacked(C.Structure):
diff --git a/gretel_b200/csrc/api.cu b/gretel_b200/csrc/api.cu
--- a/gretel_b200/csrc/api.cu
+++ b/gretel_b200/csrc/api.cu
@@ -140,7 +140,7 @@
     h->s_klen.release(st); h->s_codes4.release(st); h->s_scan.release(st);
     h->scnt.release(st); h->vseen.release(st); h->d_path.release(st); h->d_stats.release(st); h->d_site.release(st);
     h->d_partials.release(st); h->d_spec.release(st); h->d_terms.release(st); h->d_flags.release(st);
-    h->d_run_end.release(st); h->d_run_list.release(st); h->d_jobs.release(st); h->d_misc.release(st);
+    h->d_run_end.release(st); h->d_jobs.release(st); h->d_misc.release(st);
     h->d_pack.release(st);
     if (st) cudaStreamSynchronize(st);
     free(h->h_pinned);
@@ -208,7 +208,7 @@
     HX_CUDA(hx_fill_async(h->band.p, 0, sizeof(float) * (size_t)h->band_elems, h->stream));
     HX_CUDA(hx_fill_async(h->d_totals.p, 0, 8 * sizeof(unsigned long long), h->stream));
     HX_CUDA(hx_fill_async(h->d_err.p, 0, sizeof(int), h->stream));
-    HX_CUDA(hx_fill_async(h->d_flags.p, 0, 8 * sizeof(int), h->stream));
+    HX_CUDA(hx_fill_async(h->d_flags.p, 0, HX_FLAG_WORDS * sizeof(int), h->stream));
     h->use = {};
     return HX_OK;
 }
@@ -262,11 +262,10 @@
     HX_TRY(h->scnt.grow(sizeof(double) * 8 * ((size_t)n_snps + 2), h->stream));
     HX_TRY(h->vseen.grow(sizeof(int32_t) * ((size_t)n_snps + 2), h->stream));
     HX_TRY(h->d_site.grow(sizeof(double) * 6 * ((size_t)n_snps + 2), h->stream));
-    HX_TRY(h->d_flags.grow(8 * sizeof(int), h->stream));
-    HX_TRY(hx_fill_async(h->d_flags.p, 0, 8 * sizeof(int), h->stream));
+    HX_TRY(h->d_flags.grow(HX_FLAG_WORDS * sizeof(int), h->stream));
+    HX_TRY(hx_fill_async(h->d_flags.p, 0, HX_FLAG_WORDS * sizeof(int), h->stream));
     HX_TRY(h->d_misc.grow(32 * sizeof(double), h->stream));
     HX_TRY(h->d_run_end.grow(sizeof(int64_t) * ((size_t)n_snps + 2), h->stream));
-    HX_TRY(h->d_run_list.grow(sizeof(int64_t) * (((size_t)n_snps + 3) / 2 + (size_t)n_snps + 2 + 2), h->stream));
     h->h_pinned = calloc(1, 256);
     if (!h->h_pinned) { free_all(h); return HX_E_NOMEM; }
     HX_TRY(cudaStreamSynchronize(h->stream));
@@ -374,6 +373,7 @@
     if (h->use.prepass_ran) HX_CUDA(cudaMemcpyAsync(he + 1, h->d_flags.p + 4, sizeof(int), cudaMemcpyDeviceToHost, h->stream));
     HX_CUDA(cudaStreamSynchronize(h->stream));
     if (h->use.prepass_ran && he[1] == 0) hx_note_unsorted();
+    h->use.sorted = h->use.prepass_ran ? (he[1] != 0) : -1;
     hx_wire_trace_dump();
     if (h->use.ev_rec) cudaEventElapsedTime(&h->use.last_ms[0], h->ev0, h->ev1);
     for (int i = 0; i < 4; ++i) totals[i] = (int64_t)hp[i];
@@ -758,4 +758,10 @@
     return HX_OK;
 }
 
-}
+int hx_ingest_sorted(const hx_matrix *h, int32_t *sorted) {
+    HX_CHECK_ARG(h && sorted);
+    *sorted = h->use.sorted;
+    return HX_OK;
+}
+
+}
diff --git a/gretel_b200/csrc/hx_internal.cuh b/gretel_b200/csrc/hx_internal.cuh
--- a/gretel_b200/csrc/hx_internal.cuh
+++ b/gretel_b200/csrc/hx_internal.cuh
@@ -12,6 +12,7 @@
 #define HX_SYM_GAP 6
 #define HX_RING 4096
 #define HX_MAX_L (HX_RING - 1)
+#define HX_FLAG_WORDS 10
 
 #define HX_MAX_PEERS 8
 struct HxCnt {
@@ -86,7 +87,6 @@
     HxDevBuf<double> d_partials;
     HxDevBuf<int> d_flags;
     HxDevBuf<int64_t> d_run_end;
-    HxDevBuf<int64_t> d_run_list;
     HxDevBuf<int4> d_jobs;
     HxDevBuf<double> d_misc;
     HxDevBuf<uint32_t> d_pack;
@@ -103,6 +103,7 @@
         bool cnt_fresh = false;
         bool ev_rec = false;
         bool prepass_ran = false;
+        int sorted = -1;
         int wire_next = 0;
         bool sum_busy[2] = {};
         float last_ms[3] = {};
@@ -150,6 +151,21 @@
     k_fill_bytes<<<grid, 256, 0, st>>>(static_cast<uint8_t *>(p), v, bytes);
     return cudaGetLastError();
 }
+
+constexpr int64_t HX_GAP_SOLO = 32;
+static __device__ __forceinline__ void hx_fill_rank_end(int64_t *rank_end, int64_t q0, int64_t q1, int64_t v) {
+    const bool solo = q1 - q0 <= HX_GAP_SOLO;
+    if (solo)
+        for (int64_t q = q0; q < q1; ++q) rank_end[q] = v;
+    unsigned m = __ballot_sync(0xffffffffu, !solo);
+    while (m) {
+        const int src = __ffs(m) - 1;
+        m &= m - 1;
+        const int64_t a = __shfl_sync(0xffffffffu, q0, src), b = __shfl_sync(0xffffffffu, q1, src);
+        const int64_t vs = __shfl_sync(0xffffffffu, v, src);
+        for (int64_t q = a + (threadIdx.x & 31); q < b; q += 32) rank_end[q] = vs;
+    }
+}
 #endif
 
 __host__ __device__ __forceinline__ int64_t hx_cell_off(int64_t W, int64_t pi, int64_t pj) {
@@ -162,7 +178,7 @@
                                const uint8_t *d_codes, int64_t n_reads, int64_t *run_end, const int *ok);
 bool hx_umma_possible(const hx_matrix *h);
 int hx_launch_ingest_umma(hx_matrix *h, const int32_t *d_rank, const int64_t *d_off, const uint8_t *d_codes,
-                          int64_t n_reads, const int64_t *run_end, const int *sorted_flag);
+                          int64_t n_reads, const int64_t *rank_end, const int *sorted_flag);
 HxCnt hx_cnt_ref(const hx_matrix *h);
 int hx_ensure_counts_buffer(hx_matrix *h);
 void hx_wire_free(hx_matrix *h);
diff --git a/gretel_b200/csrc/ingest.cu b/gretel_b200/csrc/ingest.cu
--- a/gretel_b200/csrc/ingest.cu
+++ b/gretel_b200/csrc/ingest.cu
@@ -1,3 +1,4 @@
+#include <algorithm>
 #include <atomic>
 
 #include "hx_internal.cuh"
@@ -74,24 +75,67 @@
     flush_totals(t_slices, t_crumbs, t_cov, t_sent, totals);
 }
 
-__global__ void k_prepass_init(int *__restrict__ flag, int64_t *__restrict__ run_end, int n) {
-    const int i = blockIdx.x * blockDim.x + threadIdx.x;
-    if (i == 0) *flag = 1;
-    if (i < n) run_end[i] = -1;
-}
-
-__global__ void k_prepass(const int32_t *__restrict__ rank, int64_t n_reads, int N, int *__restrict__ flag,
-                          int64_t *__restrict__ run_end, int *__restrict__ err) {
-    const int64_t i = (int64_t)blockIdx.x * blockDim.x + threadIdx.x;
-    if (i >= n_reads) return;
-    const int r = rank[i];
-    if (r < 0 || r > N) atomicOr(err, 1);
-    if (i + 1 < n_reads) {
-        const int r2 = rank[i + 1];
-        if (r > r2) *flag = 0;
-        if (r != r2 && r >= 0 && r <= N) run_end[r] = i + 1;
-    } else if (r >= 0 && r <= N) {
-        run_end[r] = n_reads;
+constexpr int PP_BLOCK = 256;
+__global__ void __launch_bounds__(PP_BLOCK)
+k_prepass(const int32_t *__restrict__ rank, int64_t n_reads, int N, int *__restrict__ verdict,
+          unsigned *__restrict__ state, int64_t *__restrict__ rank_end, int *__restrict__ err) {
+    const int lane = threadIdx.x & 31;
+    const int64_t nq = (int64_t)N + 2;
+    const int64_t tid = (int64_t)blockIdx.x * PP_BLOCK + threadIdx.x, stride = (int64_t)gridDim.x * PP_BLOCK;
+    {
+        const int64_t lead = min(max((int64_t)rank[0], (int64_t)0), nq);
+        const int64_t tail = min(max((int64_t)rank[n_reads - 1], (int64_t)0), nq);
+        for (int64_t q = tid; q < lead + nq - tail; q += stride) {
+            if (q < lead) rank_end[q] = 0;
+            else rank_end[tail + q - lead] = n_reads;
+        }
+    }
+    const int mis = (int)((reinterpret_cast<uintptr_t>(rank) >> 2) & 3u);
+    const int64_t nv = (mis + n_reads + 3) >> 2;
+    bool unsorted = false, bad = false;
+    for (int64_t v0 = tid - lane; v0 < nv; v0 += stride) {
+        const int64_t v = v0 + lane, i0 = 4 * v - mis;
+        int r[5] = {0, 0, 0, 0, 0};
+        if (v < nv) {
+            if (i0 >= 0 && i0 + 4 <= n_reads) {
+                const int4 x = __ldg(reinterpret_cast<const int4 *>(rank + i0));
+                r[0] = x.x; r[1] = x.y; r[2] = x.z; r[3] = x.w;
+            } else {
+#pragma unroll
+                for (int e = 0; e < 4; ++e)
+                    if (i0 + e >= 0 && i0 + e < n_reads) r[e] = rank[i0 + e];
+            }
+        }
+        r[4] = __shfl_down_sync(0xffffffffu, r[0], 1);
+        if ((lane == 31 || v + 1 >= nv) && i0 + 4 < n_reads) r[4] = rank[i0 + 4];
+        bool edge = false;
+#pragma unroll
+        for (int e = 0; e < 4; ++e) {
+            const bool in = v < nv && i0 + e >= 0 && i0 + e < n_reads;
+            bad |= in && (unsigned)r[e] > (unsigned)N;
+            edge |= in && i0 + e + 1 < n_reads && r[e] != r[e + 1];
+        }
+        if (!__any_sync(0xffffffffu, edge)) continue;
+#pragma unroll
+        for (int e = 0; e < 4; ++e) {
+            int64_t q0 = 0, q1 = 0;
+            if (v < nv && i0 + e >= 0 && i0 + e + 1 < n_reads) {
+                unsorted |= r[e] > r[e + 1];
+                q0 = min(max((int64_t)r[e], (int64_t)0), nq);
+                q1 = min(max((int64_t)r[e + 1], (int64_t)0), nq);
+            }
+            hx_fill_rank_end(rank_end, q0, q1, i0 + e + 1);
+        }
+    }
+    if (bad) atomicOr(err, 1);
+    if (__syncthreads_or(unsorted) && threadIdx.x == 0) atomicOr(&state[0], 1u);
+    if (threadIdx.x == 0) {
+        __threadfence();
+        if (atomicAdd(&state[1], 1u) == gridDim.x - 1) {
+            __threadfence();
+            *verdict = atomicExch(&state[0], 0u) ? 0 : 1;
+            state[1] = 0;
+        }
     }
 }
 
@@ -683,6 +727,14 @@
     if (!presorted) run_end = h->d_run_end.p;
     int sms = 148;
     cudaDeviceGetAttribute(&sms, cudaDevAttrMultiProcessorCount, h->device);
+    const int dev_sms = sms;
+    auto prepass = [&] {
+        const int64_t want = ((n_reads + 6) / 4 + PP_BLOCK - 1) / PP_BLOCK;
+        const int grid = (int)std::min<int64_t>(std::max<int64_t>(want, 1), (int64_t)dev_sms * (2048 / PP_BLOCK));
+        k_prepass<<<grid, PP_BLOCK, 0, h->stream>>>(d_rank, n_reads, h->N, h->d_flags.p + 4,
+                                                     reinterpret_cast<unsigned *>(h->d_flags.p + 8), run_end, h->d_err.p);
+        h->use.launches++;
+    };
     if (h->use.ingest_sms > 0 && h->use.ingest_sms < sms) sms = h->use.ingest_sms;
     const int *sorted_flag = presorted ? ok : h->d_flags.p + 4;
     constexpr int GBLOCK = 256;
@@ -709,12 +761,7 @@
         int rc = hx_launch_ingest_lumma(h, d_rank, d_off, d_codes, n_reads, presorted ? ok : nullptr);
         if (rc) return rc;
     } else if (use_long) {
-        if (!presorted) {
-            HX_CUDA(hx_fill_async(h->d_flags.p + 4, 1, sizeof(int), h->stream));
-            k_prepass<<<(unsigned)((n_reads + 255) / 256), 256, 0, h->stream>>>(d_rank, n_reads, h->N, h->d_flags.p + 4,
-                                                                                run_end, h->d_err.p);
-            h->use.launches++;
-        }
+        if (!presorted) prepass();
         int rc = hx_launch_ingest_long(h, d_rank, d_off, d_codes, n_reads, sorted_flag);
         if (rc) return rc;
         if (!presorted) {
@@ -727,12 +774,7 @@
                                                               h->d_totals.p, h->d_err.p, sorted_flag, presorted ? 2 : 1);
         h->use.launches++;
     } else {
-        if (!presorted) {
-            k_prepass_init<<<(unsigned)((h->N + 2 + 255) / 256), 256, 0, h->stream>>>(h->d_flags.p + 4, run_end, use_umma ? h->N + 2 : 0);
-            k_prepass<<<(unsigned)((n_reads + 255) / 256), 256, 0, h->stream>>>(d_rank, n_reads, h->N, h->d_flags.p + 4,
-                                                                                run_end, h->d_err.p);
-            h->use.launches += 2;
-        }
+        if (!presorted) prepass();
         const int npairs = kmax * (kmax - 1) / 2;
         if (use_umma) {
             int rc = hx_launch_ingest_umma(h, d_rank, d_off, d_codes, n_reads, run_end, sorted_flag);
@@ -765,6 +807,7 @@
             else if (kmax > 32) HX_WS_LAUNCH(14, 1, 1024, 1);
             else HX_WS_LAUNCH(8, 1, 640, 2);
 #undef HX_WS_LAUNCH
+            h->use.launches++;
         } else {
         int gb = BS_GB;
         while (gb > 4 && BsLayout{kmax, gb}.bytes() > (size_t)200 * 1024) gb >>= 1;
@@ -791,8 +834,8 @@
         else if (kmax > 32) HX_BS_LAUNCH(14, 1, 1024, 1);
         else HX_BS_LAUNCH(8, 1, 512, 2);
 #undef HX_BS_LAUNCH
-        }
         h->use.launches++;
+        }
         if (lumma_fallback) {
             k_flag_not<<<1, 32, 0, h->stream>>>(h->d_flags.p + 4, h->d_flags.p + 5);
             h->use.launches++;
diff --git a/gretel_b200/csrc/ingest_umma.cu b/gretel_b200/csrc/ingest_umma.cu
--- a/gretel_b200/csrc/ingest_umma.cu
+++ b/gretel_b200/csrc/ingest_umma.cu
@@ -94,83 +94,6 @@
 }
 __device__ __forceinline__ void um_wait_st() { asm volatile("tcgen05.wait::st.sync.aligned;" ::: "memory"); }
 __device__ __forceinline__ void um_wait_ld() { asm volatile("tcgen05.wait::ld.sync.aligned;" ::: "memory"); }
-
-struct UmWalk {
-    const int32_t *run_rank;
-    const int64_t *run_stop;
-    int64_t hi, cur, p_stop;
-    int n_runs, j, p_rank;
-    int64_t start, n;
-    int r;
-    unsigned ri;
-
-    __device__ __forceinline__ void fetch() {
-        if (j < n_runs) { p_rank = run_rank[j]; p_stop = run_stop[j]; }
-    }
-    __device__ __forceinline__ void init(const int32_t *rr, const int64_t *rs, int n_runs_, int64_t lo_, int64_t hi_) {
-        run_rank = rr; run_stop = rs; n_runs = n_runs_; hi = hi_; cur = lo_; ri = 0u - 1u; r = 0; start = lo_; n = 0;
-        int a = 0, b = n_runs_;
-        while (a < b) {
-            const int m = (a + b) >> 1;
-            if (run_stop[m] > lo_) b = m; else a = m + 1;
-        }
-        j = a;
-        p_rank = 0; p_stop = 0;
-        fetch();
-    }
-    __device__ __forceinline__ bool next_run() {
-        while (cur < hi && j < n_runs) {
-            const int64_t stop = p_stop;
-            r = p_rank;
-            ++j;
-            fetch();
-            if (stop <= cur) continue;
-            const int64_t run_hi = stop < hi ? stop : hi;
-            start = cur;
-            n = run_hi - cur;
-            cur = run_hi;
-            ++ri;
-            return true;
-        }
-        cur = hi;
-        return false;
-    }
-};
-
-__global__ void __launch_bounds__(1024)
-k_run_list(const int64_t *__restrict__ run_end, int N, int32_t *__restrict__ run_rank, int64_t *__restrict__ run_stop,
-           int *__restrict__ n_runs) {
-    __shared__ int s_warp[32];
-    const int lane = threadIdx.x & 31, warp = threadIdx.x >> 5;
-    const int per = (N + 1 + 1023) / 1024;
-    const int i0 = (int)threadIdx.x * per, i1 = min(i0 + per, N + 1);
-    int mine = 0;
-    for (int i = i0; i < i1; ++i) mine += run_end[i] >= 0;
-    int incl = mine;
-#pragma unroll
-    for (int o = 1; o < 32; o <<= 1) {
-        const int v = __shfl_up_sync(0xffffffffu, incl, o);
-        if (lane >= o) incl += v;
-    }
-    if (lane == 31) s_warp[warp] = incl;
-    __syncthreads();
-    if (warp == 0) {
-        int w = s_warp[lane];
-#pragma unroll
-        for (int o = 1; o < 32; o <<= 1) {
-            const int v = __shfl_up_sync(0xffffffffu, w, o);
-            if (lane >= o) w += v;
-        }
-        s_warp[lane] = w;
-    }
-    __syncthreads();
-    int pos = incl - mine + (warp ? s_warp[warp - 1] : 0);
-    for (int i = i0; i < i1; ++i) {
-        const int64_t e = run_end[i];
-        if (e >= 0) { run_rank[pos] = i; run_stop[pos] = e; ++pos; }
-    }
-    if (threadIdx.x == 1023) *n_runs = s_warp[31];
-}
 
 template <int CH>
 __device__ __forceinline__ void um_load_read(const uint8_t *__restrict__ codes, int64_t o, int kg,
@@ -216,9 +139,8 @@
 __global__ void __launch_bounds__(UM_THREADS, 1)
 k1_umma(const int32_t *__restrict__ rank, const int64_t *__restrict__ off, const uint8_t *__restrict__ codes,
         int64_t n_reads, int N, int W, int kmax, const HxCnt cnt_in, unsigned long long *__restrict__ totals,
-        int *__restrict__ err, const int *__restrict__ sorted_flag, const int32_t *__restrict__ run_rank,
-        const int64_t *__restrict__ run_stop, const int *__restrict__ n_runs_ptr, int4 *__restrict__ jobs_all,
-        int jobs_cap, int read_w, int rank_w) {
+        int *__restrict__ err, const int *__restrict__ sorted_flag, const int64_t *__restrict__ rank_end,
+        int4 *__restrict__ jobs_all, int jobs_cap, int2 *__restrict__ runs_all, int runs_cap, int read_w, int rank_w) {
     extern __shared__ __align__(1024) uint8_t um_smem[];
     UM_T(k_begin);
     HxCnt cnt = cnt_in;
@@ -228,8 +150,10 @@
     __shared__ int s_runkg[UM_NACC];
     __shared__ unsigned s_runs_read;
     __shared__ uint32_t s_tmem;
-    __shared__ int s_jb_off[UM_JB + 1], s_jb_start[UM_JB], s_jb_n[UM_JB], s_jb_r[UM_JB], s_jb_warp[UM_JB / 32];
-    __shared__ int s_njobs;
+    __shared__ int s_jb_off[UM_JB + 1], s_jb_b[UM_JB + 1], s_jb_ri[UM_JB];
+    __shared__ long long s_jb_warp[UM_JB / 32];
+    __shared__ int s_njobs, s_nruns;
+    __shared__ long long s_flushed;
     if (!*sorted_flag) return;
 
     constexpr int ROWB = 16 * CH;
@@ -282,69 +206,59 @@
     unsigned long long prof_acc[8] = {0, 0, 0, 0, 0, 0, 0, 0};
 #endif
 
-    UmWalk wk;
-    wk.init(run_rank, run_stop, *n_runs_ptr, lo, hi);
-
     int4 *const myjobs = jobs_all + (size_t)blockIdx.x * jobs_cap;
+    int2 *const myruns = runs_all + (size_t)blockIdx.x * runs_cap;
     {
-        const int n_runs_all = *n_runs_ptr;
-        const int j0 = wk.j;
-        int job_base = 0;
-        for (int jb = j0; jb < n_runs_all; jb += UM_JB) {
-            int ng = 0;
+        const int q_lo = max(rank[lo], 0), q_hi = min(rank[hi - 1], N);
+        int job_base = 0, run_base = 0;
+        for (int qb = q_lo; qb <= q_hi; qb += UM_JB) {
+            long long ps = 0, incl = 0;
             if (threadIdx.x < UM_JB) {
-                const int j = jb + (int)threadIdx.x;
-                int64_t s0 = hi;
-                if (j < n_runs_all) {
-                    const int64_t prev = j > 0 ? run_stop[j - 1] : 0;
-                    s0 = prev > lo ? prev : lo;
-                }
-                if (s0 < hi) {
-                    const int64_t stop = run_stop[j];
-                    const int64_t e0 = stop < hi ? stop : hi;
-                    ng = (int)((e0 - s0 + 31) >> 5);
-                    s_jb_start[threadIdx.x] = (int)(s0 - lo);
-                    s_jb_n[threadIdx.x] = (int)(e0 - s0);
-                    s_jb_r[threadIdx.x] = run_rank[j];
-                }
-                int incl = ng;
+                const int q = qb + (int)threadIdx.x;
+                if (q <= q_hi) {
+                    int64_t s0 = q > 0 ? rank_end[q - 1] : 0, e0 = rank_end[q];
+                    s0 = min(max(s0, lo), hi);
+                    e0 = min(max(e0, lo), hi);
+                    if (threadIdx.x == 0) s_jb_b[0] = (int)(s0 - lo);
+                    s_jb_b[threadIdx.x + 1] = (int)(e0 - lo);
+                    if (e0 > s0) ps = ((e0 - s0 + 31) >> 5 << 9) | 1;
+                }
+                incl = ps;
 #pragma unroll
                 for (int o = 1; o < 32; o <<= 1) {
-                    const int v = __shfl_up_sync(0xffffffffu, incl, o);
+                    const long long v = __shfl_up_sync(0xffffffffu, incl, o);
                     if (lane >= o) incl += v;
                 }
                 if (lane == 31) s_jb_warp[warp] = incl;
-                s_jb_off[threadIdx.x + 1] = incl;
             }
             __syncthreads();
             if (threadIdx.x < UM_JB) {
-                int before = 0;
-                for (int w2 = 0; w2 < warp; ++w2) before += s_jb_warp[w2];
-                const int incl = s_jb_off[threadIdx.x + 1] + before;
-                __syncwarp();
-                s_jb_off[threadIdx.x + 1] = incl;
+                for (int w2 = 0; w2 < warp; ++w2) incl += s_jb_warp[w2];
+                s_jb_off[threadIdx.x + 1] = (int)(incl >> 9);
+                const int ri = run_base + (int)(incl & 511) - (int)(ps & 1);
+                s_jb_ri[threadIdx.x] = ri;
+                if (ps) myruns[ri] = make_int2(qb + (int)threadIdx.x, (int)(ps >> 9));
                 if (threadIdx.x == 0) s_jb_off[0] = 0;
+                if (threadIdx.x == UM_JB - 1) s_nruns = run_base + (int)(incl & 511);
             }
             __syncthreads();
             const int batch_jobs = s_jb_off[UM_JB];
-            for (int q = threadIdx.x; q < batch_jobs; q += blockDim.x) {
+            for (int qj = threadIdx.x; qj < batch_jobs; qj += blockDim.x) {
                 int a = 0, b = UM_JB - 1;
                 while (a < b) {
                     const int m = (a + b) >> 1;
-                    if (s_jb_off[m + 1] > q) b = m; else a = m + 1;
-                }
-                const int g = q - s_jb_off[a];
-                const int n_run = s_jb_n[a];
+                    if (s_jb_off[m + 1] > qj) b = m; else a = m + 1;
+                }
+                const int g = qj - s_jb_off[a];
+                const int start = s_jb_b[a], n_run = s_jb_b[a + 1] - start;
                 const int nj = min(32, n_run - 32 * g);
-                myjobs[job_base + q] = make_int4(s_jb_start[a] + 32 * g, nj | (g == 0 ? (min(n_run, 2048) << 8) : 0), s_jb_r[a],
-                                                 jb - j0 + a);
+                myjobs[job_base + qj] = make_int4(start + 32 * g, nj | (g == 0 ? (min(n_run, 2048) << 8) : 0), qb + a, s_jb_ri[a]);
             }
             job_base += batch_jobs;
-            const bool more = s_jb_off[UM_JB] > s_jb_off[UM_JB - 1];
+            run_base = s_nruns;
             __syncthreads();
-            if (!more) break;
-        }
-        if (threadIdx.x == 0) s_njobs = job_base;
+        }
+        if (threadIdx.x == 0) { s_njobs = job_base; s_nruns = run_base; }
         __syncthreads();
     }
     UM_T(k_roles);
@@ -477,9 +391,12 @@
         const int goff0 = word_off(threadIdx.x), goff1 = word_off(threadIdx.x + npt);
         static_assert(UM_RD_WARPS * 32 * 2 >= 31 * 16, "two tile words per readout thread cover a band row");
         int64_t flushed_upto = (int64_t)max(rank[lo], 0) + 1;
-        while (wk.next_run()) {
-            const int r = wk.r;
-            const unsigned ri = wk.ri;
+        const unsigned n_runs = (unsigned)s_nruns;
+        int2 nxt = n_runs ? myruns[0] : make_int2(0, 0);
+        for (unsigned ri = 0; ri < n_runs; ++ri) {
+            const int r = nxt.x;
+            const uint32_t ng = (uint32_t)nxt.y;
+            if (ri + 1 < n_runs) nxt = myruns[ri + 1];
             const int s = ri % UM_NACC;
             UM_T(r0);
             if ((int64_t)r + 1 > flushed_upto) {
@@ -507,7 +424,6 @@
             const int rbase = (int)((unsigned)(r + 1) % (unsigned)rows);
             UM_T(r1);
             if (threadIdx.x == 0) {
-                const uint32_t ng = (uint32_t)((wk.n + 31) >> 5);
                 asm volatile("mbarrier.arrive.release.cta.shared::cta.b64 _, [%0], %1;" ::"r"(ws_smem_u32(&s_acc_full[s])),
                              "r"(UM_ACC_COUNT - ng)
                              : "memory");
@@ -551,28 +467,35 @@
             UM_T(r3);
             UM_ACC(0, r1 - r0); UM_ACC(1, r2 - r1); UM_ACC(2, r3 - r2); UM_ACC(3, 1);
         }
-        {
-            unsigned long long sum = 0;
-            int row = (int)((flushed_upto + 1) % rows);
-            for (int64_t pj = flushed_upto + 1; pj <= flushed_upto + rows - 1; ++pj) {
-                uint32_t *base = tile32 + (size_t)row * per_row;
-                for (int w = threadIdx.x; w < per_row; w += npt) {
-                    const uint32_t v = base[w];
-                    if (v) {
-                        const int d = (w >> 4) + 1, ab = w & 15;
-                        atomicAdd(cnt.cell(W, pj - d, pj) + (ab >> 2) * HX_NSYM + (ab & 3), v);
-                        sum += v;
-                    }
-                }
-                if (++row == rows) row = 0;
-            }
-            t_crumbs += sum;
-        }
+        if (threadIdx.x == 0) s_flushed = flushed_upto;
 #ifdef UM_PROFILE
         if (threadIdx.x == 0) for (int i = 0; i < 4; ++i) atomicAdd(&um_prof[16 + i], prof_acc[i]);
 #endif
     }
     UM_T(k_roles_end);
+    __syncthreads();
+    {
+        UM_T(f0);
+        const int per_row = cells * 16;
+        const int64_t pj0 = s_flushed + 1;
+        const int row0 = (int)((unsigned)pj0 % (unsigned)rows);
+        unsigned long long sum = 0;
+        for (int idx = threadIdx.x; idx < (rows - 1) * per_row; idx += UM_THREADS) {
+            const int i = idx / per_row, w = idx - i * per_row;
+            const int row = row0 + i < rows ? row0 + i : row0 + i - rows;
+            const uint32_t v = tile32[(size_t)row * per_row + w];
+            if (v) {
+                const int d = (w >> 4) + 1, ab = w & 15;
+                atomicAdd(cnt.cell(W, pj0 + i - d, pj0 + i) + (ab >> 2) * HX_NSYM + (ab & 3), v);
+                sum += v;
+            }
+        }
+        t_crumbs += sum;
+        UM_T(f1);
+#ifdef UM_PROFILE
+        if (threadIdx.x == 0) atomicAdd(&um_prof[20], (unsigned long long)(f1 - f0));
+#endif
+    }
     if (errbits) atomicOr(err, (int)errbits);
     um_fence_before();
     flush_totals(n_slices, t_crumbs + n_rcrumbs, (unsigned long long)n_codes - n_notcov, n_sent, totals);
@@ -615,7 +538,7 @@
 }
 
 int hx_launch_ingest_umma(hx_matrix *h, const int32_t *d_rank, const int64_t *d_off, const uint8_t *d_codes,
-                          int64_t n_reads, const int64_t *run_end, const int *sorted_flag) {
+                          int64_t n_reads, const int64_t *rank_end, const int *sorted_flag) {
     int sms = 148;
     cudaDeviceGetAttribute(&sms, cudaDevAttrMultiProcessorCount, h->device);
     if (h->use.ingest_sms > 0 && h->use.ingest_sms < sms) sms = h->use.ingest_sms;
@@ -625,26 +548,23 @@
     int64_t grid = sms;
     const int64_t max_useful = (n_reads + 255) / 256;
     if (grid > max_useful) grid = max_useful;
-    int32_t *run_rank = reinterpret_cast<int32_t *>(h->d_run_list.p);
-    int64_t *run_stop = reinterpret_cast<int64_t *>(h->d_run_list.p) + (((size_t)h->N + 2 + 1) / 2);
-    int *n_runs = reinterpret_cast<int *>(run_stop + (size_t)h->N + 2);
-    k_run_list<<<1, 1024, 0, h->stream>>>(run_end, h->N, run_rank, run_stop, n_runs);
-    h->use.launches++;
     static const int read_w = [] { const char *e = getenv("HX_UM_READ_W"); const int v = e ? atoi(e) : HX_SLICE_READ_W; return v < 1 ? 1 : v; }();
     static const int rank_w = [] { const char *e = getenv("HX_UM_RANK_W"); const int v = e ? atoi(e) : HX_SLICE_RANK_W; return v < 0 ? 0 : v; }();
     const int64_t per = (((n_reads + grid - 1) / grid + 1) * (kmax + read_w) + ((int64_t)rank_w * (h->N + 2) + grid - 1) / grid) / read_w + 2;
-    const int64_t jobs_cap = per / 32 + std::min<int64_t>((int64_t)h->N + 2, per) + 2;
+    const int64_t runs_cap = std::min<int64_t>((int64_t)h->N + 2, per) + 2;
+    const int64_t jobs_cap = per / 32 + runs_cap;
     HX_CHECK_ARG(jobs_cap < ((int64_t)1 << 31) && per < ((int64_t)1 << 31));
-    const int64_t jobs_bytes = jobs_cap * grid * (int64_t)sizeof(int4);
+    const int64_t jobs_bytes = jobs_cap * grid * (int64_t)sizeof(int4) + runs_cap * grid * (int64_t)sizeof(int2);
     if (jobs_bytes > h->d_jobs.cap) HX_CUDA(h->d_jobs.grow(jobs_bytes + jobs_bytes / 8, h->stream));
+    int2 *const runs = reinterpret_cast<int2 *>(h->d_jobs.p + jobs_cap * grid);
 #define HX_UM_LAUNCH(CH_)                                                                                       \
     do {                                                                                                        \
         auto kern = fused ? k1_umma<CH_, true> : k1_umma<CH_, false>;                                           \
         HX_CUDA(cudaFuncSetAttribute(kern, cudaFuncAttributeMaxDynamicSharedMemorySize, (int)smem));            \
         kern<<<(unsigned)grid, UM_THREADS, smem, h->stream>>>(d_rank, d_off, d_codes, n_reads, h->N, h->W, kmax, \
                                                               hx_cnt_ref(h), h->d_totals.p, h->d_err.p, sorted_flag, \
-                                                              run_rank, run_stop, n_runs,                       \
-                                                              h->d_jobs.p, (int)jobs_cap, read_w, rank_w); \
+                                                              rank_end, h->d_jobs.p, (int)jobs_cap, runs,       \
+                                                              (int)runs_cap, read_w, rank_w);                   \
     } while (0)
     if (kmax <= 16) HX_UM_LAUNCH(4);
     else HX_UM_LAUNCH(8);
diff --git a/gretel_b200/csrc/wire.cu b/gretel_b200/csrc/wire.cu
--- a/gretel_b200/csrc/wire.cu
+++ b/gretel_b200/csrc/wire.cu
@@ -154,23 +154,14 @@
     int64_t run_d = partials[2 * (int64_t)blockIdx.x] + id - sd;
     int64_t run_k = partials[2 * (int64_t)blockIdx.x + 1] + ik - sk;
     for (int w = 0; w < warp; ++w) { run_d += sh[0][w]; run_k += sh[1][w]; }
-    int32_t d_next = 0;
-    if (j0 + WI < n) {
-        d_next = (int32_t)rd[j0 + WI];
-        if (n_esc && d_next == 255) {
-            d_next = esc_lookup(esc_idx, esc_delta, n_esc, j0 + WI);
-            if (d_next < 0) d_next = 0;
-        }
-    }
 #pragma unroll
     for (int i = 0; i < WI; ++i) {
         const int64_t j = j0 + i;
+        const int64_t prev = run_d < (int64_t)N + 1 ? run_d : (int64_t)N + 1;
         run_d += d[i];
-        if (j < n) {
-            rank[j] = (int32_t)(run_d <= (int64_t)N + 1 ? run_d : (int64_t)N + 1);
-            const int32_t dn = i + 1 < WI ? d[i + 1] : d_next;
-            if ((j + 1 == n || dn != 0) && run_d <= N) run_end[run_d] = j + 1;
-        }
+        const int64_t cur = run_d < (int64_t)N + 1 ? run_d : (int64_t)N + 1;
+        if (j < n) rank[j] = (int32_t)cur;
+        hx_fill_rank_end(run_end, prev, j < n ? cur : (j == n ? (int64_t)N + 2 : prev), j);
         if (j <= n) off[j] = run_k;
         run_k += k[i];
     }
@@ -325,8 +316,6 @@
         int *ok = reinterpret_cast<int *>(w.partials.p + 2 * nblk);
         const int64_t *d_ei = reinterpret_cast<const int64_t *>(raw + o_ei);
         const int32_t *d_ed = reinterpret_cast<const int32_t *>(raw + o_ed);
-        HX_CUDA(hx_fill_async(w.run_end.p, 0xff, sizeof(int64_t) * ((size_t)h->N + 2), ds));
-        h->use.launches++;
         if (klen_bytes == 1) {
             k_dense_partials<1><<<(unsigned)nblk, 256, 0, ds>>>(raw + o_rd, raw + o_kl, n_reads, d_ei, d_ed, n_esc, w.partials.p);
             k_dense_spine<<<1, 1024, 0, ds>>>(w.partials.p, nblk, n_codes, ok, h->d_err.p);
diff --git a/gretel_b200/hansel.py b/gretel_b200/hansel.py
--- a/gretel_b200/hansel.py
+++ b/gretel_b200/hansel.py
@@ -383,3 +383,8 @@
         n = C.c_int64()
         _lib.check(self._lib.hx_launch_count(self._h, C.byref(n)))
         return int(n.value)
+
+    def ingest_sorted(self):
+        s = C.c_int32()
+        _lib.check(self._lib.hx_ingest_sorted(self._h, C.byref(s)))
+        return None if s.value < 0 else bool(s.value)
diff --git a/include/hanselx.h b/include/hanselx.h
--- a/include/hanselx.h
+++ b/include/hanselx.h
@@ -115,6 +115,7 @@
 int hx_to_dense(hx_matrix *h, float *out );
 int hx_last_kernel_ms(hx_matrix *h, int which, float *ms);
 int hx_launch_count(const hx_matrix *h, int64_t *n);
+int hx_ingest_sorted(const hx_matrix *h, int32_t *sorted);
 
 #ifdef __cplusplus
 }
```

New measurement: 3797 billion, median of 6. +11.2%, better.
